# michiyasunaga/qagnn

Measured on AMD Instinct MI355X. Metric: QA-subgraphs/sec (batch x num_choice) fwd+bwd, higher is better.
Workload: dtype f32; 1 GPU; configs[1]: CSQA-shaped batch 64 questions x 5 choices = 320 subgraphs per GPU, n=200 node slots, 400..2000 edges/subgraph, 38 relations (run_qagnn__csqa.sh), 5-layer GAT d=200 H=4, QAGNN decoder fwd+bwd (LM encoder excluded: random sent_vecs), dropout 0.2, train-mode BN; subgraphs_per_gpu=320, nodes=64000, edges=396800, edges_with_self_loops=460800, graph_input=load-time int32 blobs (qagnn_graph_from_blobs), 13.3 B/edge on the wire, parallelism=single

## Files before the change

### include/qagnn_hip_tn.h

```cpp
#ifndef QAGNN_HIP_TN_H
#define QAGNN_HIP_TN_H

#include "qagnn_hip.h"

#ifdef __cplusplus
extern "C" {
#endif

int qagnn_gemm_tn_graph_f32(const float* A1, int32_t lda1, int32_t Ka1, const float* A2, int32_t lda2, int32_t Ka2, const float* B, int32_t ldb,
                            float* C, int32_t ldc, int32_t R, int32_t No, const uint32_t* amax_a1, const uint32_t* amax_a2,
                            const uint32_t* amax_b, int32_t pieces, const qagnn_graph* g, float* workspace, qagnn_stream_t stream);
int qagnn_gemm_tn_route_query(int32_t R, int32_t Ka1, int32_t Ka2, int32_t No, int32_t* h_out );
int qagnn_tn_work_table(const qagnn_graph* g, int32_t S, int32_t chunk_tiles, int32_t* out, qagnn_stream_t stream);
int qagnn_tn_live_tiles(int32_t on);

#ifdef __cplusplus
}
#endif
#endif
```

### qagnn_amd/_lib.py

```python
import ctypes as C
import functools
import os

import torch

_HERE = os.path.dirname(os.path.abspath(__file__))
LIB_PATH = os.environ.get('QAGNN_LIB') or os.path.join(_HERE, 'libqagnn_hip.so')

EXPORTS = ['qagnn_last_error', 'qagnn_abi_version', 'qagnn_graph_storage_elems', 'qagnn_graph_prep', 'qagnn_graph_prep_blocked',
           'qagnn_graph_from_blobs', 'qagnn_radam_step_f32', 'qagnn_node_prep_f32', 'qagnn_seed_epoch_advance', 'qagnn_seed_epoch_set',
           'qagnn_gemm_nn_f32', 'qagnn_gemm_nn_split_f32', 'qagnn_gemm_nn_pack_bytes', 'qagnn_gemm_nn_ws_bytes', 'qagnn_gemm_nn_split_ws_f32', 'qagnn_gemm_nn_prepack_bytes', 'qagnn_gemm_nn_prepack_f32',
           'qagnn_gemm_nn_prepack_clear', 'qagnn_gemm_tn_workspace_elems', 'qagnn_gemm_tn_f32', 'qagnn_gemm_tn2_f32', 'qagnn_gemm_tn_colsum_f32',
           'qagnn_colreduce_workspace_elems', 'qagnn_colreduce_f32', 'qagnn_bn_finalize_f32', 'qagnn_bn_stats_finalize_f32', 'qagnn_bn_relu_bwd_f32',
           'qagnn_gelu_dropout_fwd_f32', 'qagnn_gelu_dropout_bwd_f32', 'qagnn_sin_basis_f32',
           'qagnn_bn_relu_bwd_colsum_f32',
           'qagnn_pool_attn_fwd_f32', 'qagnn_pool_attn_bwd_f32', 'qagnn_head_post_fwd_f32', 'qagnn_head_post_bwd_f32', 'qagnn_add_row0_f32', 'qagnn_gather_multi_f32', 'qagnn_gather_multi_sum_f32',
           'qagnn_edge_attn_fwd_f32', 'qagnn_edge_attn_bwd_f32',
           'qagnn_hop_fwd_workspace_elems', 'qagnn_hop_bwd_workspace_elems', 'qagnn_hop_fwd_f32', 'qagnn_hop_bwd_f32',
           'qagnn_stack_fwd_f32', 'qagnn_stack_bwd_f32', 'qagnn_absmax_f32', 'qagnn_zero_words', 'qagnn_gemm_tn_h2_f32', 'qagnn_gelu_dropout_fwd_amax_f32', 'qagnn_gelu_dropout_amax_scratch_elems',
           'qagnn_timing_enable', 'qagnn_timing_read', 'qagnn_gemm_tn_h1_f32', 'qagnn_gelu_dropout_bwd_amax_f32', 'qagnn_packed_min_rows',
           'qagnn_radam_step_scaled_f32', 'qagnn_grad_norm_workspace_elems', 'qagnn_grad_norm_f32', 'qagnn_scale_multi_f32', 'qagnn_graph_prep_cap',
           'qagnn_store_gather', 'qagnn_graph_from_store']
EXPORTS_TN = ['qagnn_gemm_tn_graph_f32', 'qagnn_gemm_tn_route_query', 'qagnn_tn_work_table', 'qagnn_tn_live_tiles']
EXPORTS_INFER = ['qagnn_infer_version', 'qagnn_bn_relu_absmax_scratch_elems', 'qagnn_bn_relu_absmax_f32', 'qagnn_stack_infer_f32',
                 'qagnn_choice_eval_f32']
EXPORTS_LOSS = ['qagnn_loss_version', 'qagnn_choice_loss_f32', 'qagnn_choice_loss_bwd_f32']
LOSS_KINDS = {'cross_entropy': 0, 'margin_rank': 1}
LOSS_THREADS = 256

CLS_SLICES = 4
ABI_VERSION = 25

_i32, _i64, _f32, _u64, _vp = C.c_int32, C.c_int64, C.c_float, C.c_uint64, C.c_void_p


class qagnn_graph(C.Structure):
    _fields_ = ([(n, _i32) for n in ('N', 'E', 'Ep', 'R', 'T', 'C')] +
                [(n, _vp) for n in ('rowptr_s', 'tgt_s', 'src_s', 'cls_s', 'eid_s', 'rowptr_t', 'src_t', 'tgt_t', 'cls_t', 'pos_t',
                                    'cls_count', 'src_c', 'tgt_c', 'pos_c', 'chunk_cls', 'chunk_beg',
                                    'chunk_len', 'n_chunks', 'chunkptr')] +
                [('max_chunks', _i32), ('err', _vp), ('block_n', _i32), ('n_groups', _i32)])


class qagnn_store(C.Structure):
    _fields_ = ([(n, _vp) for n in ('blobs', 'blob_off', 'concept_ids', 'node_type', 'node_scores', 'adj_len')] +
                [('S', _i32), ('n', _i32), ('W', _i64)])


GATHER_MAX = 160


class qagnn_gather_tabs(C.Structure):
    _fields_ = [('p', _vp * GATHER_MAX), ('n', _i32)]


class qagnn_pack_desc(C.Structure):
    _fields_ = [('B1n', _vp), ('ldn1', _i32), ('K1', _i32), ('B2n', _vp), ('ldn2', _i32), ('K2', _i32), ('No', _i32), ('pieces', _i32)]


class qagnn_gemm_nn_args(C.Structure):
    _fields_ = [('A1', _vp), ('lda1', _i32), ('K1', _i32), ('B1', _vp), ('ldb1', _i32),
                ('A2', _vp), ('lda2', _i32), ('K2', _i32), ('B2', _vp), ('ldb2', _i32),
                ('C', _vp), ('ldc', _i32), ('M', _i32), ('No', _i32),
                ('bias', _vp), ('rowtab', _vp), ('ldt', _i32), ('rowidx', _vp),
                ('a_scale', _vp), ('a_shift', _vp), ('accumulate', _i32), ('a_rowidx', _vp), ('xcd_remap', _i32), ('colstat_part', _vp),
                ('a_amax1', _vp), ('a_amax2', _vp), ('a_rows', _i64), ('pieces', _i32)]


class qagnn_hop_args(C.Structure):
    _fields_ = ([('g', C.POINTER(qagnn_graph))] + [(n, _i32) for n in ('N', 'DP', 'SP', 'HP', 'T')] + [('qscale', _f32)] +
                [(n, _vp) for n in ('X', 'S', 'ntype', 'Wx_t', 'Wx', 'Ws_t', 'Ws', 'TT', 'EkEm', 'W1t', 'W1', 'b1', 'gamma', 'beta',
                                    'W2t', 'W2', 'b2')] +
                [('batch_stats', _i32), ('eps', _f32), ('run_mean_p', _vp), ('run_var_p', _vp), ('run_mean', _vp), ('run_var', _vp),
                 ('num_batches_tracked', _vp), ('dense_pos', _vp), ('d', _i32), ('momentum', _f32),
                 ('apply_act', _i32), ('p_drop', _f32), ('seed', _u64)] +
                [(n, _vp) for n in ('KMQ', 'a', 'alpha', 'aggr', 'h1', 'out', 'y', 'stats', 'dy', 'dX', 'dS')] +
                [('accumulate_dS', _i32), ('accumulate_dX', _i32)] +
                [(n, _vp) for n in ('dWx_t', 'dWs_t', 'dTT', 'dEkEm', 'dW1t', 'db1', 'dbn', 'dW2t', 'db2', 'ws')] +
                [('ws_elems', _i64), ('gemm_split', _i32), ('ones_col', _i32), ('tab_col', _i32), ('side_stream', _vp), ('amax', _vp), ('x_amax', _vp), ('s_amax', _vp)])


HOP_AMAX_WORDS = 16


def load_library(path=LIB_PATH):
    if not os.path.exists(path):
        raise OSError(f'{path} not found: build it with `python -m qagnn_amd.build` (hipcc, gfx950)')
    lib = C.CDLL(path)
    lib.qagnn_last_error.restype = C.c_char_p
    lib.qagnn_abi_version.restype = _i32
    lib.qagnn_graph_storage_elems.restype = _i64
    lib.qagnn_graph_storage_elems.argtypes = [_i32, _i32, _i32, _i32]
    lib.qagnn_graph_prep.argtypes = [C.POINTER(qagnn_graph), _vp, _vp, _vp, _vp, _i32, _i32, _i32, _i32, _vp]
    lib.qagnn_graph_prep_blocked.argtypes = [C.POINTER(qagnn_graph), _vp, _vp, _vp, _vp, _i32, _i32, _i32, _i32, _i32, _vp]
    lib.qagnn_graph_prep_cap.argtypes = [C.POINTER(qagnn_graph), _vp, _vp, _i64, _vp, _vp, _i32, _i32, _vp, _i32, _i32, _i32, _vp]
    lib.qagnn_graph_from_blobs.argtypes = [C.POINTER(qagnn_graph), _vp, _vp, _vp, _vp, _vp, _i32, _i32, _i32, _i32, _i32, _vp]
    lib.qagnn_store_gather.argtypes = [C.POINTER(qagnn_store), _vp, _i32, _vp, _vp, _vp, _vp, _vp, _vp, _vp]
    lib.qagnn_graph_from_store.argtypes = [C.POINTER(qagnn_graph), _vp, C.POINTER(qagnn_store), _vp, _vp, _vp, _i32, _i32, _i32, _i32, _vp]
    lib.qagnn_node_prep_f32.argtypes = [_vp, _vp, _vp, _vp, _i32, _i32, _vp, _vp, _vp, _i64, _vp, _vp]
    lib.qagnn_seed_epoch_advance.argtypes = [_u64, _vp]
    lib.qagnn_seed_epoch_set.argtypes = [_u64, _vp]
    lib.qagnn_radam_step_f32.argtypes = [_i32, _vp, _vp, _vp, _vp, _vp] + [C.c_double] * 6 + [_i32, _vp]
    lib.qagnn_radam_step_scaled_f32.argtypes = [_i32, _vp, _vp, _vp, _vp, _vp] + [C.c_double] * 6 + [_i32, _vp, _vp]
    lib.qagnn_grad_norm_workspace_elems.restype = _i64
    lib.qagnn_grad_norm_workspace_elems.argtypes = [_i32, _vp]
    lib.qagnn_grad_norm_f32.argtypes = [_i32, _vp, _vp, C.c_double, _vp, _vp, _vp]
    lib.qagnn_scale_multi_f32.argtypes = [_i32, _vp, _vp, _vp, _vp]
    lib.qagnn_gemm_nn_f32.argtypes = [C.POINTER(qagnn_gemm_nn_args), _vp]
    lib.qagnn_gemm_nn_split_f32.argtypes = [C.POINTER(qagnn_gemm_nn_args), _vp, _i32, _vp, _i32, _vp]
    lib.qagnn_gemm_nn_pack_bytes.restype = _i64
    lib.qagnn_gemm_nn_pack_bytes.argtypes = [_i32, _i32, _i32]
    lib.qagnn_gemm_nn_split_ws_f32.argtypes = [C.POINTER(qagnn_gemm_nn_args), _vp, _i32, _vp, _i32, _vp, _i64, _vp]
    lib.qagnn_gemm_nn_ws_bytes.restype = _i64
    lib.qagnn_gemm_nn_ws_bytes.argtypes = [C.POINTER(qagnn_gemm_nn_args), _vp, _i32, _vp, _i32]
    lib.qagnn_gemm_nn_prepack_bytes.restype = _i64
    lib.qagnn_gemm_nn_prepack_bytes.argtypes = [C.POINTER(qagnn_pack_desc), _i32]
    lib.qagnn_gemm_nn_prepack_f32.argtypes = [C.POINTER(qagnn_pack_desc), _i32, _vp, _i64, _i64, _vp]
    lib.qagnn_gemm_nn_prepack_clear.argtypes = [_i64]
    lib.qagnn_gemm_tn_workspace_elems.restype = _i64
    lib.qagnn_gemm_tn_workspace_elems.argtypes = [_i32, _i32, _i32]
    lib.qagnn_gemm_tn_f32.argtypes = [_vp, _i32, _vp, _i32, _vp, _i32, _i32, _i32, _i32, _vp, _vp, _vp, _i32, _vp, _vp]
    lib.qagnn_gemm_tn2_f32.argtypes = [_vp, _i32, _i32, _vp, _i32, _i32, _vp, _i32, _vp, _i32, _i32, _i32, _vp, _vp]
    lib.qagnn_gemm_tn_h2_f32.argtypes = [_vp, _i32, _i32, _vp, _i32, _i32, _vp, _i32, _vp, _i32, _i32, _i32, _vp, _vp, _vp, _vp, _vp, _vp, _vp]
    lib.qagnn_gemm_tn_h1_f32.argtypes = lib.qagnn_gemm_tn_h2_f32.argtypes
    lib.qagnn_gemm_tn_graph_f32.argtypes = [_vp, _i32, _i32, _vp, _i32, _i32, _vp, _i32, _vp, _i32, _i32, _i32, _vp, _vp, _vp, _i32,
                                            C.POINTER(qagnn_graph), _vp, _vp]
    lib.qagnn_gemm_tn_route_query.argtypes = [_i32, _i32, _i32, _i32, _vp]
    lib.qagnn_tn_work_table.argtypes = [C.POINTER(qagnn_graph), _i32, _i32, _vp, _vp]
    lib.qagnn_tn_live_tiles.argtypes = [_i32]
    lib.qagnn_absmax_f32.argtypes = [_vp, _i64, _vp, _vp]
    lib.qagnn_zero_words.argtypes = [_vp, _i64, _vp]
    lib.qagnn_timing_enable.argtypes = [_i32]
    lib.qagnn_timing_read.argtypes = [_vp, _vp]
    lib.qagnn_packed_min_rows.restype = _i64
    lib.qagnn_packed_min_rows.argtypes = [_i64]
    lib.qagnn_gemm_tn_colsum_f32.argtypes = [_vp, _i32, _vp, _i32, _vp, _i32, _i32, _i32, _i32, _vp, _vp, _vp, _i32, _vp, _vp, _i32,
                                             _vp, _vp]
    lib.qagnn_colreduce_workspace_elems.restype = _i64
    lib.qagnn_colreduce_workspace_elems.argtypes = [_i32, _i32, _i32]
    lib.qagnn_colreduce_f32.argtypes = [_i32, _vp, _i32, _vp, _i32, _i32, _i32, _vp, _i32, _vp, _vp, _vp, _vp, _vp, _f32, _vp, _vp, _vp]
    lib.qagnn_bn_finalize_f32.argtypes = [_vp, _vp, _vp, _vp, _f32, _vp, _vp, _vp, _i32, _vp, _vp, _vp, _vp, _i32, _f32, _f32, _i32, _vp]
    lib.qagnn_bn_stats_finalize_f32.argtypes = [_vp, _i32, _i32, _i32, _vp, _vp, _f32, _vp, _vp, _vp, _vp, _vp, _i32, _f32, _f32, _i32, _vp]
    lib.qagnn_bn_relu_bwd_f32.argtypes = [_vp, _vp, _vp, _i32, _i32, _i32, _vp, _vp, _vp, _vp, _vp, _vp, _vp, _f32, _vp, _vp]
    lib.qagnn_gelu_dropout_fwd_f32.argtypes = [_vp, _vp, _i64, _f32, _u64, _vp]
    lib.qagnn_gelu_dropout_bwd_f32.argtypes = [_vp, _vp, _vp, _i64, _f32, _u64, _vp]
    lib.qagnn_gelu_dropout_fwd_amax_f32.argtypes = [_vp, _vp, _i64, _f32, _u64, _vp, _vp, _vp]
    lib.qagnn_gelu_dropout_bwd_amax_f32.argtypes = [_vp, _vp, _vp, _i64, _f32, _u64, _vp, _vp, _vp]
    lib.qagnn_gelu_dropout_amax_scratch_elems.restype = _i64
    lib.qagnn_gelu_dropout_amax_scratch_elems.argtypes = [_i64]
    lib.qagnn_sin_basis_f32.argtypes = [_vp, _vp, _vp, _i32, _i32, _i32, _vp]
    lib.qagnn_bn_relu_bwd_colsum_f32.argtypes = [_vp, _vp, _vp, _i32, _i32, _i32, _vp, _vp, _vp, _vp, _vp, _vp, _vp, _f32, _vp, _vp, _vp, _vp]
    lib.qagnn_pool_attn_fwd_f32.argtypes = [_vp, _vp, _vp, _i32, _vp, _i32, _i32, _i32, _i32, _f32, _f32, _u64, _vp, _vp, _vp, _vp]
    lib.qagnn_pool_attn_bwd_f32.argtypes = [_vp, _vp, _i32, _i32, _i32, _i32, _i32, _f32, _f32, _u64, _vp, _vp, _vp, _vp, _vp, _i32, _vp, _vp, _vp]
    lib.qagnn_head_post_fwd_f32.argtypes = [_vp, _vp, _vp, _vp, _vp, _vp, _i64, _vp, _vp, _i32, _i32, _i32, _i32, _i32, _i32, _i32, _f32, _f32, _u64, _u64,
                                            _vp, _vp, _vp, _vp]
    lib.qagnn_head_post_bwd_f32.argtypes = [_vp, _vp, _vp, _vp, _vp, _vp, _vp, _i64, _vp, _i32, _i32, _i32, _i32, _i32, _i32, _i32, _f32, _f32, _u64, _u64,
                                            _vp, _vp, _vp, _vp, _vp, _vp, _i32, _vp]
    lib.qagnn_add_row0_f32.argtypes = [_vp, _i64, _vp, _i32, _i32, _vp]
    lib.qagnn_gather_multi_f32.argtypes = [C.POINTER(qagnn_gather_tabs), _vp, _vp, _vp, _i32, _vp]
    lib.qagnn_gather_multi_sum_f32.argtypes = [C.POINTER(qagnn_gather_tabs), _vp, _vp, _i32, _i32, _vp, _vp]
    lib.qagnn_edge_attn_fwd_f32.argtypes = [C.POINTER(qagnn_graph), _vp, _i32, _vp, _i32, _i32, _f32, _vp, _vp, _vp, _vp, _i32, _vp]
    lib.qagnn_edge_attn_bwd_f32.argtypes = [C.POINTER(qagnn_graph), _vp, _i32, _vp, _i32, _i32, _f32, _vp, _vp, _vp, _i32,
                                            _vp, _vp, _vp, _vp, _vp, _vp]
    lib.qagnn_hop_fwd_workspace_elems.restype = _i64
    lib.qagnn_hop_fwd_workspace_elems.argtypes = [_i32, _i32, _i32]
    lib.qagnn_hop_bwd_workspace_elems.restype = _i64
    lib.qagnn_hop_bwd_workspace_elems.argtypes = [_i32, _i32, _i32, _i32, _i32]
    lib.qagnn_hop_fwd_f32.argtypes = [C.POINTER(qagnn_hop_args), _vp]
    lib.qagnn_hop_bwd_f32.argtypes = [C.POINTER(qagnn_hop_args), _vp]
    lib.qagnn_stack_fwd_f32.argtypes = [C.POINTER(qagnn_hop_args), _i32, _vp]
    lib.qagnn_stack_bwd_f32.argtypes = [C.POINTER(qagnn_hop_args), _i32, _vp]
    lib.qagnn_infer_version.argtypes = []
    lib.qagnn_bn_relu_absmax_scratch_elems.restype = _i64
    lib.qagnn_bn_relu_absmax_scratch_elems.argtypes = [_i32, _i32]
    lib.qagnn_bn_relu_absmax_f32.argtypes = [_vp, _i32, _i32, _i32, _vp, _vp, _vp, _vp, _vp]
    lib.qagnn_stack_infer_f32.argtypes = [C.POINTER(qagnn_hop_args), _i32, _vp]
    lib.qagnn_choice_eval_f32.argtypes = [_vp, _i64, _vp, _i32, _i32, _vp, _vp, _vp]
    lib.qagnn_loss_version.argtypes = []
    lib.qagnn_choice_loss_f32.argtypes = [_vp, _i64, _vp, _i32, _i32, _i32, _f32, _vp, _vp, _vp, _i64, _vp, _vp, _vp]
    lib.qagnn_choice_loss_bwd_f32.argtypes = [_vp, _i64, _vp, _vp, _i64, _i32, _i32, _vp]
    for name in EXPORTS + EXPORTS_TN + EXPORTS_INFER + EXPORTS_LOSS:
        fn = getattr(lib, name)
        if fn.restype is C.c_int and name not in ('qagnn_abi_version',):
            fn.restype = _i32
    return lib


def _ptr(t):
    return None if t is None else t.data_ptr()


def choice_loss_bound(kind, nc, Q, max_abs=1.0, margin=0.0, weight=1.0, threads=LOSS_THREADS):
    import math
    u, v = 2.0 ** -24, 2.0 ** -53
    M, L, w = max(1.0, float(max_abs)), math.log(nc), abs(float(weight))
    S = -(-Q // threads) + math.log2(threads) + nc
    if LOSS_KINDS[kind] == 0:
        return w * M * (u * (nc + 8 + 5 * L) + v * S * (2 + L)), w / Q * u * (nc + 8 + L)
    return w * M * (3 * u + v * S) * (2 + abs(float(margin)) / M), w / Q * 2 * u


def _running_fields(running):
    if running is None:
        return None, None, None, None, 0, 0.0, 1.0
    rm, rv, nbt, pos, mom, unb = running
    assert rm.is_contiguous() and rv.is_contiguous() and pos.dtype == torch.long and (nbt is None or nbt.dtype == torch.long)
    return rm.data_ptr(), rv.data_ptr(), _ptr(nbt), pos.data_ptr(), rm.numel(), float(mom), float(unb)


def _chk2d(t, name, dtype=torch.float32):
    assert t.is_cuda and t.dtype == dtype and t.dim() == 2 and t.is_contiguous(), \
        f'{name}: need a contiguous 2-D {dtype} device tensor, got {tuple(t.shape)} {t.dtype} {t.device}'
# ... 426 lines not shown
                n2, ld2 = B2n.data_ptr(), _ld(B2n)
            ws_bytes = self.lib.qagnn_gemm_nn_ws_bytes(C.byref(a), B1n.data_ptr(), ld1, n2, ld2) if M >= self.PACK_MIN_M else 0
            if ws_bytes > 0:
                ws = torch.empty(ws_bytes, dtype=torch.uint8, device=A1.device)
                self._check(self.lib.qagnn_gemm_nn_split_ws_f32(C.byref(a), B1n.data_ptr(), ld1, n2, ld2, ws.data_ptr(), ws_bytes, self._stream()),
                            'qagnn_gemm_nn_split_ws_f32')
            else:
                self._check(self.lib.qagnn_gemm_nn_split_f32(C.byref(a), B1n.data_ptr(), ld1, n2, ld2, self._stream()), 'qagnn_gemm_nn_split_f32')
            return (out, part) if colstats else out
        assert K1 % 16 == 0 and (A2 is None or A2.size(1) % 16 == 0), 'the fp32-MFMA kernel needs K to be a multiple of 16'
        self._check(self.lib.qagnn_gemm_nn_f32(C.byref(a), self._stream()), 'qagnn_gemm_nn_f32')
        return out

    def _tn_out_ws(self, R, Ka, No, out, dev):
        if out is None:
            out = torch.empty((Ka, No), dtype=torch.float32, device=dev)
        else:
            _chkp(out, 'out')
            assert out.shape == (Ka, No)
        return out, torch.empty(self.lib.qagnn_gemm_tn_workspace_elems(R, Ka, No), dtype=torch.float32, device=dev)

    def gemm_tn(self, A, B, a_scale=None, a_shift=None, out=None, accumulate=False, a_rowidx=None, colsum_groups=0,
                b_rowidx=None):
        _chkp(A, 'A'), _chkp(B, 'B')
        Ka = A.size(1)
        R, No = B.shape
        assert (A.size(0) == R) if a_rowidx is None else (a_rowidx.numel() == R and a_rowidx.dtype == torch.long)
        assert out is not None or not accumulate
        out, ws = self._tn_out_ws(R, Ka, No, out, A.device)
        bsum = None
        if colsum_groups:
            assert b_rowidx is None or (b_rowidx.dtype == torch.long and b_rowidx.numel() == R and b_rowidx.is_contiguous())
            bsum = torch.empty((colsum_groups, No), dtype=torch.float32, device=A.device)
        rc = self.lib.qagnn_gemm_tn_colsum_f32(A.data_ptr(), _ld(A), B.data_ptr(), _ld(B), out.data_ptr(), _ld(out), R, Ka, No, _ptr(a_scale),
                                               _ptr(a_shift), _ptr(a_rowidx), 1 if accumulate else 0, _ptr(bsum), _ptr(b_rowidx),
                                               colsum_groups, ws.data_ptr(), self._stream())
        self._check(rc, 'qagnn_gemm_tn_colsum_f32')
        return (out, bsum) if colsum_groups else out

    def absmax(self, x, out=None):
        assert x.is_contiguous() and x.dtype == torch.float32 and x.numel() % 4 == 0
        if out is None:
            out = torch.empty(4, dtype=torch.int32, device=x.device)
            self._check(self.lib.qagnn_zero_words(out.data_ptr(), 4, self._stream()), 'qagnn_zero_words')
        self._check(self.lib.qagnn_absmax_f32(x.data_ptr(), x.numel(), out.data_ptr(), self._stream()), 'qagnn_absmax_f32')
        return out

    def gemm_tn_h2(self, A1, B, amax_a1, amax_b, A2=None, amax_a2=None, a_scale=None, a_shift=None, out=None):
        _chkp(A1, 'A1'), _chkp(B, 'B')
        if A2 is not None:
            _chkp(A2, 'A2')
        Ka1, Ka2 = A1.size(1), (A2.size(1) if A2 is not None else 0)
        R, No = B.shape
        out, ws = self._tn_out_ws(R, Ka1 + Ka2, No, out, B.device)
        fn = self.lib.qagnn_gemm_tn_h1_f32 if self.gemm_split == 3 else self.lib.qagnn_gemm_tn_h2_f32
        rc = fn(A1.data_ptr(), _ld(A1), Ka1, _ptr(A2), _ld(A2) if A2 is not None else 0, Ka2, B.data_ptr(), _ld(B), out.data_ptr(), _ld(out), R, No, _ptr(a_scale),
                                           _ptr(a_shift), amax_a1.data_ptr(), _ptr(amax_a2), amax_b.data_ptr(), ws.data_ptr(), self._stream())
        self._check(rc, 'qagnn_gemm_tn_h2_f32')
        return out

    def gemm_tn_graph(self, A1, A2, B, graph=None, pieces=3, amax=None, out=None):
        _chkp(A1, 'A1'), _chkp(A2, 'A2'), _chkp(B, 'B')
        Ka1, Ka2 = A1.size(1), A2.size(1)
        R, No = B.shape
        assert A1.size(0) == R and A2.size(0) == R and (pieces == 3 or amax is not None)
        out, ws = self._tn_out_ws(R, Ka1 + Ka2, No, out, B.device)
        am = [None, None, None] if amax is None else [t.data_ptr() for t in amax]
        rc = self.lib.qagnn_gemm_tn_graph_f32(A1.data_ptr(), _ld(A1), Ka1, A2.data_ptr(), _ld(A2), Ka2, B.data_ptr(), _ld(B), out.data_ptr(), _ld(out),
                                              R, No, am[0], am[1], am[2], pieces, C.byref(graph.c) if graph is not None else None, ws.data_ptr(),
                                              self._stream())
        self._check(rc, 'qagnn_gemm_tn_graph_f32')
        return out

    def tn_route_query(self, R, Ka1, Ka2, No):
        out = (_i32 * 4)()
        self._check(self.lib.qagnn_gemm_tn_route_query(R, Ka1, Ka2, No, C.cast(out, _vp)), 'qagnn_gemm_tn_route_query')
        return tuple(out)

    def tn_work_table(self, graph, S, chunk_tiles):
        out = torch.empty(4 + 5 * S, dtype=torch.int32, device=graph.storage.device)
        self._check(self.lib.qagnn_tn_work_table(C.byref(graph.c), S, chunk_tiles, out.data_ptr(), self._stream()), 'qagnn_tn_work_table')
        return out

    def tn_live_tiles(self, on):
        return int(self.lib.qagnn_tn_live_tiles(int(on)))

    def gemm_tn2(self, A1, A2, B, out=None):
        _chkp(A1, 'A1'), _chkp(A2, 'A2'), _chkp(B, 'B')
        Ka1, Ka2 = A1.size(1), A2.size(1)
        R, No = B.shape
        assert A1.size(0) == R and A2.size(0) == R
        out, ws = self._tn_out_ws(R, Ka1 + Ka2, No, out, B.device)
        rc = self.lib.qagnn_gemm_tn2_f32(A1.data_ptr(), _ld(A1), Ka1, A2.data_ptr(), _ld(A2), Ka2, B.data_ptr(), _ld(B), out.data_ptr(), _ld(out), R, No,
                                         ws.data_ptr(), self._stream())
        self._check(rc, 'qagnn_gemm_tn2_f32')
        return out

    def _colreduce(self, mode, X, X2, rowidx, groups, mean, invstd, scale, shift, nout, out_scale=1.0, roww=None, out=None):
        _chkp(X, 'X')
        R, Cc = X.shape
        if out is None:
            out = torch.empty((nout, Cc), dtype=torch.float32, device=X.device)
        else:
            assert out.shape == (nout, Cc) and out.is_contiguous() and out.dtype == torch.float32
        ws = torch.empty(self.lib.qagnn_colreduce_workspace_elems(R, Cc, groups), dtype=torch.float32, device=X.device)
        rc = self.lib.qagnn_colreduce_f32(mode, X.data_ptr(), _ld(X), _ptr(X2), _ld(X2) if X2 is not None else Cc, R, Cc, _ptr(rowidx), groups, _ptr(mean),
                                          _ptr(invstd), _ptr(scale), _ptr(shift), _ptr(roww), float(out_scale), out.data_ptr(), ws.data_ptr(), self._stream())
        self._check(rc, 'qagnn_colreduce_f32')
        return out

    def colsum(self, X, rowidx=None, groups=1, scale=1.0, roww=None, out=None):
        return self._colreduce(0, X, None, rowidx, groups, None, None, None, None, groups, scale, roww, out=out)

    def colvar_sum(self, X, mean, scale=1.0, roww=None):
        return self._colreduce(1, X, None, None, 1, mean, None, None, None, 1, scale, roww)[0]

    def bn_finalize(self, mean, var, gamma, beta, eps, running=None, ones_col=-1):
        Cc = mean.numel()
        out = torch.empty((3, Cc), dtype=torch.float32, device=mean.device)
        rc = self.lib.qagnn_bn_finalize_f32(mean.data_ptr(), var.data_ptr(), gamma.data_ptr(), beta.data_ptr(), float(eps),
                                            out[0].data_ptr(), out[1].data_ptr(), out[2].data_ptr(), Cc, *_running_fields(running),
                                            int(ones_col), self._stream())
        self._check(rc, 'qagnn_bn_finalize_f32')
        return out[0], out[1], out[2]

    def bn_stats_finalize(self, part, rows, gamma, beta, eps, running=None, ones_col=-1):
        nt, _, Cc = part.shape
        assert part.is_contiguous() and nt == -(-rows // self.STAT_TILE)
        stats = torch.empty((5, Cc), dtype=torch.float32, device=part.device)
        rc = self.lib.qagnn_bn_stats_finalize_f32(part.data_ptr(), nt, int(rows), Cc, gamma.data_ptr(), beta.data_ptr(), float(eps), stats.data_ptr(),
                                                  *_running_fields(running), int(ones_col), self._stream())
        self._check(rc, 'qagnn_bn_stats_finalize_f32')
        return stats

    def bn_bwd_reduce(self, dR, H, mean, invstd, scale, shift):
        _chkp(H, 'H')
        assert H.shape == dR.shape
        return self._colreduce(2, dR, H, None, 1, mean, invstd, scale, shift, 2)

    @staticmethod
    def _bn_bwd_operands(dR, H, dH):
        _chkp(dR, 'dR'), _chkp(H, 'H')
        if dH is None:
            dH = torch.empty(H.shape, dtype=torch.float32, device=H.device)
        _chkp(dH, 'dH')
        assert dR.shape == H.shape == dH.shape and _ld(dR) == _ld(H) == _ld(dH), \
            f'bn_relu_bwd: dR, H and dH share one row pitch, got {_ld(dR)}, {_ld(H)}, {_ld(dH)}'
        return dH, _ld(H)

    def bn_relu_bwd(self, dR, H, mean, invstd, scale, shift, gamma, red, inv_rows, roww=None, dH=None):
        assert red.is_contiguous() and red.shape == (2, H.size(1))
        dH, ld = self._bn_bwd_operands(dR, H, dH)
        R, Cc = H.shape
        rc = self.lib.qagnn_bn_relu_bwd_f32(dR.data_ptr(), H.data_ptr(), dH.data_ptr(), ld, R, Cc, mean.data_ptr(),
                                            invstd.data_ptr(), scale.data_ptr(), shift.data_ptr(), gamma.data_ptr(),
                                            red[0].data_ptr(), red[1].data_ptr(), float(inv_rows), _ptr(roww), self._stream())
        self._check(rc, 'qagnn_bn_relu_bwd_f32')
        return dH

    POOL_LIMITS = (4, 256, 1024)

    def pool_attn_fwd(self, u, cvec, K, mask, inv_temp, p, seed):
        B, NH, Cc = u.shape
        n = K.size(1)
        assert u.is_contiguous() and cvec.is_contiguous() and mask.is_contiguous() and mask.dtype == torch.bool
        _chkp3(K, 'K')
# ... 473 lines not shown
```

### qagnn_amd/csrc/common.h

```cpp
#pragma once
#include <hip/hip_runtime.h>
#include <stdint.h>
#include <stdio.h>

#include <type_traits>

#include "../../include/qagnn_hip.h"
#include "../../include/qagnn_hip_tn.h"
#include "../../include/qagnn_hip_infer.h"

namespace qagnn {

void set_error(const char* fmt, ...);

struct NnProduct {
  const qagnn_gemm_nn_args* a;
  bool split;
  const float* B1n; int ldn1; const float* B2n; int ldn2;
  void* ws; int64_t ws_bytes;
};
enum class NnFamily { FP32, SPLIT, NN2 };
enum class NnB { IN_KERNEL, PACK, IMAGE };
struct NnRoute {
  NnFamily family;
  int nt, np, wv;
  bool affine, flat, stats;
  NnB b; const void* image;
  int64_t ws_bytes;
  int ntiles, grid;
};
inline int num_cus() {
  static int n = [] {
    int dev = 0, v = 0;
    if (hipGetDevice(&dev) != hipSuccess || hipDeviceGetAttribute(&v, hipDeviceAttributeMultiprocessorCount, dev) != hipSuccess || v <= 0) v = 256;
    return v;
  }();
  return n;
}
static inline int cdiv(int64_t a, int64_t b) { return (int)((a + b - 1) / b); }
inline void nn_grid(NnRoute& r, int M, int No, int rows_per_tile, int per_cu) {
  r.ntiles = cdiv(No, r.nt * 16) * cdiv(M, rows_per_tile);
  const int cap = (num_cus() * per_cu) & ~7;
  r.grid = r.ntiles < cap ? r.ntiles : cap;
}
NnRoute nn_route(const NnProduct& p);
bool nn_rows_packed(int64_t M);
int gemm_nn(const NnProduct& p, hipStream_t stream);
int launch_nn(const NnRoute& r, const qagnn_gemm_nn_args& a, hipStream_t stream);
int launch_nn_split(const NnRoute& r, const qagnn_gemm_nn_args& a, const float* B1n, int ldn1, const float* B2n, int ldn2, hipStream_t stream);
int launch_nn2(const NnRoute& r, const qagnn_gemm_nn_args& a, const float* B1n, int ldn1, const float* B2n, int ldn2, hipStream_t stream);
int launch_pack_b(int np, const qagnn_gemm_nn_args& a, const float* B1n, int ldn1, const float* B2n, int ldn2, void* ws, hipStream_t stream);
namespace nn2 { int walk_tiles(int K1, int K2); }
int64_t nn2_pack_bytes(int No, int K1, int K2, int np);
const void* nn2_prepack_lookup(const float* B1n, int ldn1, int K1, const float* B2n, int ldn2, int K2, int No, int np);

struct TnProduct {
  const float* A1; int lda1, Ka1;
  const float* A2; int lda2, Ka2; bool two;
  const float* B; int ldb;
  float* C; int ldc, R, No;
  const float* a_scale; const float* a_shift; const int64_t* a_rowidx; int accumulate;
  float* bsum; const int64_t* b_rowidx; int groups;
  const uint32_t* amax[3]; int np;
  float* ws;
  const qagnn_graph* g;
};
inline TnProduct tn_product(const float* A1, int lda1, int Ka1, const float* A2, int lda2, int Ka2, const float* B, int ldb, float* C, int ldc, int R,
                            int No, const float* a_scale, const float* a_shift, float* ws, const uint32_t* amax_a1 = nullptr,
                            const uint32_t* amax_a2 = nullptr, const uint32_t* amax_b = nullptr, int np = 3) {
  TnProduct p = {};
  p.A1 = A1; p.lda1 = lda1; p.Ka1 = Ka1;
  if (A2 && Ka2 > 0) { p.A2 = A2; p.lda2 = lda2; p.Ka2 = Ka2; p.two = true; }
  p.B = B; p.ldb = ldb; p.C = C; p.ldc = ldc; p.R = R; p.No = No; p.a_scale = a_scale; p.a_shift = a_shift; p.ws = ws;
  p.amax[0] = amax_a1; p.amax[1] = amax_a2; p.amax[2] = amax_b; p.np = np;
  return p;
}
enum class TnFamily { RUNTIME, STRIP, SPLIT, WS, PAIR };
struct TnRoute {
  TnFamily family;
  int kt, nt, waves, np;
  bool affine, gather, colsum;
  int chunk_rows, nchunks;
  bool sum_by4;
  bool live;
  dim3 grid;
  int64_t ws_elems;
};
TnRoute tn_route(const TnProduct& p);
int gemm_tn(const TnProduct& p, hipStream_t stream);
int launch_tn(const TnRoute& r, const TnProduct& p, float* Pcs, hipStream_t stream);
int launch_tn_strip(const TnRoute& r, const TnProduct& p, float* Pcs, hipStream_t stream);
int launch_tn_split(const TnRoute& r, const TnProduct& p, hipStream_t stream);
int launch_tn_ws(const TnRoute& r, const TnProduct& p, hipStream_t stream);
int launch_sum_chunks(const float* P, float* C, int ldc, int rows, int No, int nchunks, int accumulate, bool by4, hipStream_t stream);

constexpr int TN_LIST_CAP = 1024;
constexpr int TN_LIVE_BC = 208;
struct TnLive { const int* list; const int* n_live; int T, S, chunk_tiles; };
struct TnWork { int cK, cM, lenM, qK, rK; };
struct TnSlot { int cb, list, beg, cnt, pslot; };
__host__ __device__ inline TnWork tn_work(int S, int T, int L, int chunk_tiles) {
  TnWork w;
  L = L < 0 ? 0 : (L > T ? T : L);
  if (L >= T) {
    w.cK = S / 3; w.cM = S - 2 * w.cK; w.lenM = chunk_tiles; w.qK = -1; w.rK = 0;
    return w;
  }
  const long long den = (long long)T + 2ll * L;
  int c = (int)((2ll * S * L + den) / (2 * den));
  const int hi = (S - 1) / 2;
  c = c < 1 ? 1 : (c > hi ? hi : c);
  w.cK = c; w.cM = S - 2 * c; w.lenM = (T + w.cM - 1) / w.cM; w.qK = L / c; w.rK = L % c;
  return w;
}
__host__ __device__ inline TnSlot tn_slot(const TnWork& w, int S, int T, int u) {
  auto start = [&](int j) { return 2 * j + (int)((long long)j * w.cM / w.cK); };
  int j = (int)((long long)u * w.cK / S);
  while (j > 0 && start(j) > u) --j;
  while (j + 1 < w.cK && start(j + 1) <= u) ++j;
  const int off = u - start(j);
  TnSlot s;
  auto range = [&](int i) { s.list = 0; s.beg = i * w.lenM < T ? i * w.lenM : T; s.cnt = T - s.beg < w.lenM ? T - s.beg : w.lenM; };
  if (off < 2) {
    s.cb = off == 0 ? 0 : 2;
    s.pslot = off == 0 ? j : w.cK + j;
    if (w.qK < 0) range(j);
    else { s.list = 1; s.beg = j * w.qK + (j < w.rK ? j : w.rK); s.cnt = w.qK + (j < w.rK ? 1 : 0); }
  } else {
    const int m = (int)((long long)j * w.cM / w.cK) + off - 2;
    s.cb = 1;
    s.pslot = 2 * w.cK + m;
    range(m);
  }
  return s;
}
int launch_sum_chunks_live(const float* P, float* C, int ldc, int rows, const TnLive& lv, int accumulate, hipStream_t stream);
bool tn_live_enabled();
struct LiveTiles { int n_tiles; int32_t *n_live, *live, *list; };
inline LiveTiles live_tiles_of(const qagnn_graph* g) {
  const int T = (int)(((int64_t)g->N + 31) / 32), T4 = (T + 3) & ~3;
  int32_t* const p = g->err + 16;
  return LiveTiles{T, p, p + 4, p + 4 + T4};
}

int launch_gelu_dropout(const float* X, const float* dY, float* out, int64_t n, float p, uint64_t seed, uint32_t* amax, float* amax_part,
                        hipStream_t stream);
int64_t gelu_amax_scratch_elems(int64_t n);
int launch_bn_relu_bwd_colsum(const float* dR, const float* Hh, float* dH, int ld, int R, int Cc, const float* mean, const float* invstd,
                              const float* scale, const float* shift, const float* gamma, const float* sum_dy, const float* sum_dy_hhat,
                              float inv_rows, const float* roww, float* colsum, float* workspace, uint32_t* amax, hipStream_t stream);
int launch_bn_stats_finalize(const float* part, int n_tiles, int R, int Cc, const float* gamma, const float* beta, float eps, float* stats,
                             float* run_mean, float* run_var, int64_t* nbt, int d, float momentum, float unbias, int ones_col, uint32_t* amax_bound,
                             hipStream_t stream);

int launch_edge_attn_fwd(const qagnn_graph* g, const float* KMQ, int32_t ldk, const float* EkEm, int32_t lde, int32_t HP, float qscale,
                         float* score, float* a, float* alpha, float* aggr, int32_t lda, float* amax_part , hipStream_t stream);
int launch_edge_attn_bwd(const qagnn_graph* g, const float* KMQ, int32_t ldk, const float* EkEm, int32_t lde, int32_t HP, float qscale,
                         const float* a, const float* alpha, const float* G, int32_t ldg, float* dKMQ, float* dEkEm, float* ga, float* rs,
                         float* cls_part, float* amax_part , uint32_t* amax_slot, hipStream_t stream);
int launch_amax_reduce(const float* part, int64_t n, uint32_t* slot, hipStream_t stream);
int launch_bn_relu_absmax(const float* H, int ldh, int R, int Cc, const float* scale, const float* shift, uint32_t* slot, float* part, hipStream_t stream);

struct TimedScope {
  int kind;
  hipStream_t s;
  hipEvent_t e0, e1;
  bool counted;
  TimedScope(int kind, hipStream_t s);
  ~TimedScope();
  TimedScope(const TimedScope&) = delete;
  TimedScope& operator=(const TimedScope&) = delete;
};

#define QAGNN_REQUIRE(cond, code, ...) \
  do {                                 \
    if (!(cond)) {                     \
      qagnn::set_error(__VA_ARGS__);   \
      return (code);                   \
    }                                  \
  } while (0)

#define QAGNN_LAUNCH_CHECK(name)                                               \
  do {                                                                         \
    hipError_t e__ = hipGetLastError();                                        \
    if (e__ != hipSuccess) {                                                   \
      qagnn::set_error("%s launch failed: %s", name, hipGetErrorString(e__));  \
      return QAGNN_EHIP;                                                       \
    }                                                                          \
  } while (0)

#ifndef QAGNN_NN_OCC
#define QAGNN_NN_OCC 2
#endif

template <int V0, int... Vs, class F>
inline int dispatch_int(int v, F&& f) {
  if constexpr (sizeof...(Vs) == 0) return f(std::integral_constant<int, V0>{});
  else return v == V0 ? f(std::integral_constant<int, V0>{}) : dispatch_int<Vs...>(v, f);
}
template <class F>
inline int dispatch_bool(bool v, F&& f) { return v ? f(std::true_type{}) : f(std::false_type{}); }

template <auto KERNEL>
inline int raise_lds_limit(int bytes, const char* name) {
  static bool raised[64] = {};
  int dev = 0;
  if (hipGetDevice(&dev) != hipSuccess) dev = 0;
  if (bytes <= 64 * 1024 || raised[dev & 63]) return QAGNN_OK;
  hipError_t e = hipFuncSetAttribute((const void*)KERNEL, hipFuncAttributeMaxDynamicSharedMemorySize, bytes);
  if (e != hipSuccess) { set_error("%s: cannot raise the dynamic LDS limit: %s", name, hipGetErrorString(e)); return QAGNN_EHIP; }
  raised[dev & 63] = true;
  return QAGNN_OK;
}

static inline bool aligned16(const void* p) { return (reinterpret_cast<uintptr_t>(p) & 15u) == 0; }

__device__ __forceinline__ int xcd_remap(int b, int nblocks) {
  const int q = nblocks >> 3, r = nblocks & 7;
  const int xcd = b & 7, slot = b >> 3;
  const int base = xcd < r ? xcd * (q + 1) : r * (q + 1) + (xcd - r) * q;
  return base + slot;
}

__host__ __device__ __forceinline__ int edge_xcd_cap(int N) {
  const int per = (((N + 3) >> 2) + 7) >> 3;
  return (per * 5 + 3) >> 2;
}
// ... 136 lines not shown
```

### qagnn_amd/csrc/elementwise.hip

```cpp
#include "common.h"

namespace qagnn {

constexpr int CR_WR_BIG = 32, CR_WR_SMALL = 8;
static inline int cr_wr(int R) { return R < 32768 ? CR_WR_SMALL : CR_WR_BIG; }

template <int MODE, int CR_WR>
__global__ __launch_bounds__(256) void k_colreduce(const float* __restrict__ X, int ldx, const float* __restrict__ X2, int ldx2,
                                                   int R, int Cc, const int64_t* __restrict__ rowidx, int groups,
                                                   const float* __restrict__ mean, const float* __restrict__ invstd,
                                                   const float* __restrict__ scale, const float* __restrict__ shift,
                                                   const float* __restrict__ roww, float* __restrict__ part) {
  constexpr int NOUT = MODE == 0 ? 4 : (MODE == 2 ? 2 : 1);
  __shared__ __attribute__((aligned(16))) float red[4][NOUT][256];
  const int lane = threadIdx.x & 63, w = threadIdx.x >> 6;
  const int col = blockIdx.x * 256 + lane * 4;
  const bool act = col < Cc;
  constexpr int CR_ROWS = 4 * CR_WR;
  const int r0 = blockIdx.y * CR_ROWS + w * CR_WR;
  float4 acc[NOUT];
#pragma unroll
  for (int o = 0; o < NOUT; ++o) acc[o] = make_float4(0.f, 0.f, 0.f, 0.f);
  float4 mu = make_float4(0.f, 0.f, 0.f, 0.f), is = mu, sc = mu, sh = mu;
  if (act && MODE >= 1) mu = ld4(mean + col);
  if (act && MODE == 2) { is = ld4(invstd + col); sc = ld4(scale + col); sh = ld4(shift + col); }
  if (act) {
    const int rend = min(R, r0 + CR_WR);
    for (int rb = r0; rb < rend; rb += 8) {
      float4 xs[8], hs[8];
#pragma unroll
      for (int u = 0; u < 8; ++u) {
        const int r = min(rb + u, rend - 1);
        xs[u] = ld4(X + (int64_t)r * ldx + col);
        if (MODE == 2) hs[u] = ld4(X2 + (int64_t)r * ldx2 + col);
      }
#pragma unroll
      for (int u = 0; u < 8; ++u) {
        const int r = rb + u;
        if (r >= rend) break;
        float4 x = xs[u];
        const float wr = (MODE != 2 && roww) ? roww[r] : 1.f;
        if (MODE == 0) {
          x = make_float4(x.x * wr, x.y * wr, x.z * wr, x.w * wr);
          const int g = rowidx ? (int)rowidx[r] : 0;
          if (g == 0) acc[0] = add4(acc[0], x);
          else if (g == 1) acc[1] = add4(acc[1], x);
          else if (g == 2) acc[2] = add4(acc[2], x);
          else acc[3] = add4(acc[3], x);
        } else if (MODE == 1) {
          const float4 d = make_float4(x.x - mu.x, x.y - mu.y, x.z - mu.z, x.w - mu.w);
          acc[0] = make_float4(fmaf(d.x * wr, d.x, acc[0].x), fmaf(d.y * wr, d.y, acc[0].y), fmaf(d.z * wr, d.z, acc[0].z),
                               fmaf(d.w * wr, d.w, acc[0].w));
        } else {
          const float4 h = hs[u];
          float4 dy;
          dy.x = fmaf(h.x, sc.x, sh.x) <= 0.f ? 0.f : x.x;
          dy.y = fmaf(h.y, sc.y, sh.y) <= 0.f ? 0.f : x.y;
          dy.z = fmaf(h.z, sc.z, sh.z) <= 0.f ? 0.f : x.z;
          dy.w = fmaf(h.w, sc.w, sh.w) <= 0.f ? 0.f : x.w;
          acc[0] = add4(acc[0], dy);
          acc[1].x = fmaf(dy.x, (h.x - mu.x) * is.x, acc[1].x);
          acc[1].y = fmaf(dy.y, (h.y - mu.y) * is.y, acc[1].y);
          acc[1].z = fmaf(dy.z, (h.z - mu.z) * is.z, acc[1].z);
          acc[1].w = fmaf(dy.w, (h.w - mu.w) * is.w, acc[1].w);
        }
      }
    }
  }
#pragma unroll
  for (int o = 0; o < NOUT; ++o) st4(&red[w][o][lane * 4], acc[o]);
  __syncthreads();
  const int nout = MODE == 0 ? groups : NOUT;
  for (int i = threadIdx.x; i < nout * 256; i += 256) {
    const int o = i >> 8, c = i & 255;
    if (blockIdx.x * 256 + c < Cc) {
      const float s = (red[0][o][c] + red[1][o][c]) + (red[2][o][c] + red[3][o][c]);
      part[((int64_t)blockIdx.y * nout + o) * Cc + blockIdx.x * 256 + c] = s;
    }
  }
}

constexpr int CF_Q = 16;
__global__ __launch_bounds__(64 * CF_Q) void k_colreduce_final(const float* __restrict__ part, float* __restrict__ out, int nchunks,
                                                               int tot, float out_scale) {
  __shared__ float red[CF_Q][64];
  const int lane = threadIdx.x & 63, q = threadIdx.x >> 6;
  const int o = blockIdx.x * 64 + lane;
  float s0 = 0.f, s1 = 0.f;
  if (o < tot) {
    int c = q;
#pragma unroll 4
    for (; c + CF_Q < nchunks; c += 2 * CF_Q) {
      s0 += part[(int64_t)c * tot + o];
      s1 += part[(int64_t)(c + CF_Q) * tot + o];
    }
    if (c < nchunks) s0 += part[(int64_t)c * tot + o];
  }
  red[q][lane] = s0 + s1;
  __syncthreads();
  if (q == 0 && o < tot) {
    float s = red[0][lane];
#pragma unroll
    for (int k = 1; k < CF_Q; ++k) s += red[k][lane];
    out[o] = s * out_scale;
  }
}


__global__ void k_bn_relu_bwd(const float* __restrict__ dR, const float* __restrict__ Hh, float* __restrict__ dH, int ld, int R,
                              int Cc, const float* __restrict__ mean, const float* __restrict__ invstd,
                              const float* __restrict__ scale, const float* __restrict__ shift, const float* __restrict__ gamma,
                              const float* __restrict__ sum_dy, const float* __restrict__ sum_dy_hhat, float inv_rows,
                              const float* __restrict__ roww) {
  const int c4n = Cc >> 2;
  const int64_t i = (int64_t)blockIdx.x * blockDim.x + threadIdx.x;
  if (i >= (int64_t)R * c4n) return;
  const int r = (int)(i / c4n), col = (int)(i % c4n) * 4;
  if (roww) inv_rows = roww[r];
  const int64_t off = (int64_t)r * ld + col;
  const float4 g = ld4(dR + off), h = ld4(Hh + off);
  const float4 mu = ld4(mean + col), is = ld4(invstd + col), sc = ld4(scale + col), sh = ld4(shift + col);
  const float4 ga = ld4(gamma + col), k1 = ld4(sum_dy + col), k2 = ld4(sum_dy_hhat + col);
  float4 o;
#define ONE(f)                                              \
  {                                                         \
// ... 207 lines not shown
        acc = add4(acc, o);
        am = fmaxf(am, absmax4(o));
      }
    }
  }
  st4(&red[w][lane * 4], acc);
  __syncthreads();
  const int c = threadIdx.x;
  if (blockIdx.x * 256 + c < Cc)
    part[(int64_t)blockIdx.y * Cc + blockIdx.x * 256 + c] = (red[0][c] + red[1][c]) + (red[2][c] + red[3][c]);
  if (amax) {
    __shared__ float ared[16];
    block_amax_merge(am, amax, ared);
  }
}

__device__ unsigned long long g_seed_epoch = 0;
__global__ void k_seed_epoch(unsigned long long* w, unsigned long long v, int add) { *w = add ? *w + v : v; }

const unsigned long long* seed_epoch_ptr() {
  static const unsigned long long* cache[64] = {};
  int dev = 0;
  if (hipGetDevice(&dev) != hipSuccess) dev = 0;
  const unsigned long long*& p = cache[dev & 63];
  if (!p) {
    void* a = nullptr;
    if (hipGetSymbolAddress(&a, HIP_SYMBOL(g_seed_epoch)) != hipSuccess) return nullptr;
    p = static_cast<const unsigned long long*>(a);
  }
  return p;
}

__global__ void k_sin_basis(const float* __restrict__ score, const float* __restrict__ js, float* __restrict__ out, int ldo, int R,
                            int J) {
  const int64_t i = (int64_t)blockIdx.x * blockDim.x + threadIdx.x;
  if (i >= (int64_t)R * ldo) return;
  const int r = (int)(i / ldo), j = (int)(i % ldo);
  out[i] = j < J ? sinf(js[j] * score[r]) : 0.f;
}

}

using namespace qagnn;

extern "C" int64_t qagnn_colreduce_workspace_elems(int32_t R, int32_t Cc, int32_t groups) {
  return (int64_t)cdiv(R, 4 * cr_wr(R)) * (groups < 2 ? 2 : groups) * Cc;
}

extern "C" int qagnn_colreduce_f32(int32_t mode, const float* X, int32_t ldx, const float* X2, int32_t ldx2, int32_t R, int32_t Cc,
                                   const int64_t* rowidx, int32_t groups, const float* mean, const float* invstd,
                                   const float* scale, const float* shift, const float* roww, float out_scale, float* out, float* workspace, qagnn_stream_t stream_) {
  hipStream_t stream = (hipStream_t)stream_;
  QAGNN_REQUIRE(X && out && workspace, QAGNN_EINVAL, "colreduce: null pointer");
  QAGNN_REQUIRE(R > 0 && Cc > 0 && Cc % 4 == 0 && ldx % 4 == 0 && aligned16(X), QAGNN_EINVAL, "colreduce: bad sizes/alignment");
  QAGNN_REQUIRE(mode >= 0 && mode <= 2, QAGNN_EINVAL, "colreduce: bad mode %d", mode);
  QAGNN_REQUIRE(ldx >= Cc && (mode != 2 || ldx2 >= Cc), QAGNN_EINVAL, "colreduce: ldx=%d / ldx2=%d below Cc=%d", ldx, ldx2, Cc);
  const bool small = cr_wr(R) == CR_WR_SMALL;
  dim3 grid(cdiv(Cc, 256), cdiv(R, 4 * cr_wr(R)));
  int nout;
  if (mode == 0) {
    QAGNN_REQUIRE(groups >= 1 && groups <= 4 && (groups == 1 || rowidx), QAGNN_EINVAL, "colreduce: groups=%d (1..4)", groups);
    nout = groups;
    if (small) k_colreduce<0, CR_WR_SMALL><<<grid, 256, 0, stream>>>(X, ldx, X2, ldx2, R, Cc, rowidx, groups, mean, invstd, scale, shift, roww, workspace);
    else k_colreduce<0, CR_WR_BIG><<<grid, 256, 0, stream>>>(X, ldx, X2, ldx2, R, Cc, rowidx, groups, mean, invstd, scale, shift, roww, workspace);
  } else if (mode == 1) {
    QAGNN_REQUIRE(mean && aligned16(mean), QAGNN_EINVAL, "colreduce: mode 1 needs mean");
    nout = 1;
    if (small) k_colreduce<1, CR_WR_SMALL><<<grid, 256, 0, stream>>>(X, ldx, X2, ldx2, R, Cc, rowidx, groups, mean, invstd, scale, shift, roww, workspace);
    else k_colreduce<1, CR_WR_BIG><<<grid, 256, 0, stream>>>(X, ldx, X2, ldx2, R, Cc, rowidx, groups, mean, invstd, scale, shift, roww, workspace);
  } else {
    QAGNN_REQUIRE(X2 && mean && invstd && scale && shift && ldx2 % 4 == 0 && aligned16(X2), QAGNN_EINVAL,
                  "colreduce: mode 2 needs X2, mean, invstd, scale, shift");
    nout = 2;
    if (small) k_colreduce<2, CR_WR_SMALL><<<grid, 256, 0, stream>>>(X, ldx, X2, ldx2, R, Cc, rowidx, groups, mean, invstd, scale, shift, roww, workspace);
    else k_colreduce<2, CR_WR_BIG><<<grid, 256, 0, stream>>>(X, ldx, X2, ldx2, R, Cc, rowidx, groups, mean, invstd, scale, shift, roww, workspace);
  }
  QAGNN_LAUNCH_CHECK("k_colreduce");
  const int tot = nout * Cc;
  k_colreduce_final<<<cdiv(tot, 64), 64 * CF_Q, 0, stream>>>(workspace, out, grid.y, tot, out_scale);
  QAGNN_LAUNCH_CHECK("k_colreduce_final");
  return QAGNN_OK;
}

extern "C" int qagnn_bn_relu_bwd_f32(const float* dR, const float* Hh, float* dH, int32_t ld, int32_t R, int32_t Cc,
                                     const float* mean, const float* invstd, const float* scale, const float* shift,
                                     const float* gamma, const float* sum_dy, const float* sum_dy_hhat, float inv_rows,
                                     const float* roww, qagnn_stream_t stream_) {
  hipStream_t stream = (hipStream_t)stream_;
  QAGNN_REQUIRE(dR && Hh && dH && mean && invstd && scale && shift && gamma && sum_dy && sum_dy_hhat, QAGNN_EINVAL,
                "bn_relu_bwd: null pointer");
  QAGNN_REQUIRE(R > 0 && Cc > 0 && Cc % 4 == 0 && ld % 4 == 0, QAGNN_EINVAL, "bn_relu_bwd: bad sizes");
  QAGNN_REQUIRE(ld >= Cc, QAGNN_EINVAL, "bn_relu_bwd: ld=%d below Cc=%d", ld, Cc);
  const int64_t tot = (int64_t)R * (Cc / 4);
  k_bn_relu_bwd<<<cdiv(tot, 256), 256, 0, stream>>>(dR, Hh, dH, ld, R, Cc, mean, invstd, scale, shift, gamma, sum_dy, sum_dy_hhat,
                                                    inv_rows, roww);
  QAGNN_LAUNCH_CHECK("k_bn_relu_bwd");
  return QAGNN_OK;
}

extern "C" int qagnn_bn_finalize_f32(const float* mean, const float* var, const float* gamma, const float* beta, float eps, float* invstd,
                                     float* scale, float* shift, int32_t Cc, float* run_mean, float* run_var, int64_t* num_batches_tracked,
                                     const int64_t* dense_pos, int32_t d, float momentum, float unbias, int32_t ones_col,
                                     qagnn_stream_t stream_) {
  hipStream_t stream = (hipStream_t)stream_;
  QAGNN_REQUIRE(mean && var && gamma && beta && invstd && scale && shift && Cc > 0, QAGNN_EINVAL, "bn_finalize: null pointer");
  QAGNN_REQUIRE(!run_mean || (run_var && dense_pos && d > 0 && d <= Cc), QAGNN_EINVAL, "bn_finalize: running-stat arguments");
  k_bn_finalize<<<cdiv(Cc, 256), 256, 0, stream>>>(mean, var, gamma, beta, eps, invstd, scale, shift, Cc, run_mean, run_var,
                                                   num_batches_tracked, dense_pos, d, momentum, unbias, ones_col);
  QAGNN_LAUNCH_CHECK("k_bn_finalize");
  return QAGNN_OK;
}

namespace qagnn {
int launch_bn_stats_finalize(const float* part, int n_tiles, int R, int Cc, const float* gamma, const float* beta, float eps, float* stats,
                             float* run_mean, float* run_var, int64_t* nbt, int d, float momentum, float unbias, int ones_col, uint32_t* amax_bound,
                             hipStream_t stream) {
  k_bn_stats_finalize<<<cdiv(Cc, BF_COLS), BF_COLS * BF_PARTS, 0, stream>>>(part, n_tiles, R, Cc, gamma, beta, eps, stats, run_mean, run_var, nbt, d,
                                                                            momentum, unbias, ones_col, amax_bound);
  QAGNN_LAUNCH_CHECK("k_bn_stats_finalize");
  return QAGNN_OK;
}
}

extern "C" int qagnn_bn_stats_finalize_f32(const float* part, int32_t n_tiles, int32_t R, int32_t Cc, const float* gamma, const float* beta,
                                           float eps, float* stats, float* run_mean, float* run_var, int64_t* num_batches_tracked,
                                           const int64_t* dense_pos, int32_t d, float momentum, float unbias, int32_t ones_col,
                                           qagnn_stream_t stream_) {
  hipStream_t stream = (hipStream_t)stream_;
  QAGNN_REQUIRE(part && gamma && beta && stats && R > 0 && Cc > 0 && n_tiles == cdiv(R, ST_TILE), QAGNN_EINVAL,
                "bn_stats_finalize: bad arguments (R=%d needs %d tiles of %d rows, got %d)", R, cdiv(R, ST_TILE), ST_TILE, n_tiles);
  QAGNN_REQUIRE(!run_mean || (run_var && d > 0 && d % 4 == 0 && Cc % 4 == 0 && d <= Cc), QAGNN_EINVAL, "bn_stats_finalize: running-stat arguments");
  (void)dense_pos;
  return launch_bn_stats_finalize(part, n_tiles, R, Cc, gamma, beta, eps, stats, run_mean, run_var, num_batches_tracked, d, momentum, unbias, ones_col,
                                  nullptr, stream);
}

__global__ __launch_bounds__(256) void k_gather_multi(qagnn_gather_tabs t, const int* __restrict__ tid, const int* __restrict__ off,
                                                     float* __restrict__ out, int total) {
  __shared__ const float* ps[QAGNN_GATHER_MAX];
  for (int i = threadIdx.x; i < t.n; i += blockDim.x) ps[i] = t.p[i];
  __syncthreads();
  const int i = blockIdx.x * blockDim.x + threadIdx.x;
  if (i >= total) return;
  const int k = tid[i];
  out[i] = k >= 0 ? ps[k][off[i]] : 0.f;
}

__global__ __launch_bounds__(256) void k_gather_multi_sum(qagnn_gather_tabs t, const int* __restrict__ tid, const int* __restrict__ off, int K, int S,
                                                         float* __restrict__ out) {
  __shared__ const float* ps[QAGNN_GATHER_MAX];
  for (int i = threadIdx.x; i < t.n; i += blockDim.x) ps[i] = t.p[i];
  __syncthreads();
  const int s = blockIdx.x * blockDim.x + threadIdx.x;
  if (s >= S) return;
  float acc = 0.f;
  for (int k = 0; k < K; ++k) {
    const int g = tid[(int64_t)k * S + s];
    const float* p = g >= 0 ? ps[g] : nullptr;
    const float v = p != nullptr ? p[off[(int64_t)k * S + s]] : 0.f;
    acc = k == 0 ? v : acc + v;
  }
  out[s] = acc;
}

extern "C" int qagnn_gather_multi_f32(const qagnn_gather_tabs* t, const int32_t* tid, const int32_t* off, float* out, int32_t total,
                                      qagnn_stream_t stream_) {
// ... 194 lines not shown
```

### qagnn_amd/csrc/gemm.hip

```cpp
#include <stdlib.h>

#include "gemm_device.h"

namespace qagnn {

typedef float f32x4 __attribute__((ext_vector_type(4)));

constexpr int BK = 16;
constexpr int NN_BM = 128;
constexpr int PA_NN = BK + 4;

__host__ __device__ constexpr int pitch_b(int bn) { return (bn % 32 == 16) ? bn : bn + 16; }

template <int V> struct ic { static constexpr int value = V; };

template <int NM>
__device__ __forceinline__ void sched_ktile_pipeline() {
  constexpr int DS = 0x100, MFMA = 0x008, NR = (NM + 1) / 2 + 1;
#pragma unroll
  for (int r = 0; r < NR; ++r) __builtin_amdgcn_sched_group_barrier(DS, 1, 0);
#pragma unroll
  for (int kk = 0; kk < 3; ++kk) {
#pragma unroll
    for (int t = 0; t < NR; ++t) {
// ... 380 lines not shown
        const int g = groups > 1 ? grp_s[cur][kq] : 0;
        if (g == 0) cs[0] += v;
        else if (g == 1) cs[1] += v;
        else if (g == 2) cs[2] += v;
        else cs[3] += v;
      }
    }
    if (more) lstore(ic<cur ^ 1>{});
    __syncthreads();
  };

  if (nkt > 0) {
    gload(0);
    lstore(ic<0>{});
  }
  __syncthreads();
  for (int kt = 0; kt < nkt; kt += 2) {
    ktile(ic<0>{}, kt);
    if (kt + 1 < nkt) ktile(ic<1>{}, kt + 1);
  }
  if (do_cs && n0 + tid < No) {
    float* pc = Pcs + (int64_t)chunk * groups * No + n0 + tid;
    pc[0] = cs[0];
    if (groups > 1) pc[No] = cs[1];
    if (groups > 2) pc[2 * No] = cs[2];
    if (groups > 3) pc[3 * No] = cs[3];
  }
  float* Pc = P + (int64_t)chunk * Ka * No;
#pragma unroll
  for (int r = 0; r < 4; ++r) {
    const int row = m0 + w * 16 + (lane >> 4) * 4 + r;
    if (row >= Ka) continue;
#pragma unroll
    for (int j = 0; j < NT; ++j) {
      const int col = n0 + j * 16 + (lane & 15);
      if (col < No) Pc[(int64_t)row * No + col] = acc[j][r];
    }
  }
}

__global__ void k_sum_chunks(const float* __restrict__ P, float* __restrict__ C, int ldc, int Ka, int No, int nchunks,
                             int accumulate) {
  const int64_t i = (int64_t)blockIdx.x * blockDim.x + threadIdx.x;
  if (i >= (int64_t)Ka * No) return;
  const int row = (int)(i / No), col = (int)(i % No);
  float s = 0.f;
#pragma unroll 8
  for (int c = 0; c < nchunks; ++c) s += P[(int64_t)c * Ka * No + i];
  float* d = C + (int64_t)row * ldc + col;
  *d = accumulate ? *d + s : s;
}

constexpr int SC_G = 16;
__global__ __launch_bounds__(SC_G * 64) void k_sum_chunks4(const float* __restrict__ P, float* __restrict__ C, int ldc, int Ka, int No,
                                                           int nchunks, int accumulate) {
  __shared__ float4 part[SC_G][64];
  const int lane = threadIdx.x & 63, g = threadIdx.x >> 6;
  const int64_t n4 = (int64_t)Ka * No / 4, i4 = (int64_t)blockIdx.x * 64 + lane;
  float4 s = make_float4(0.f, 0.f, 0.f, 0.f);
  if (i4 < n4) {
    const float4* src = reinterpret_cast<const float4*>(P) + i4;
    for (int c0 = g; c0 < nchunks; c0 += 4 * SC_G) {
      float4 v[4];
#pragma unroll
      for (int u = 0; u < 4; ++u) v[u] = src[(int64_t)min(c0 + u * SC_G, nchunks - 1) * n4];
#pragma unroll
      for (int u = 0; u < 4; ++u)
        if (c0 + u * SC_G < nchunks) s = add4(s, v[u]);
    }
  }
  part[g][lane] = s;
  __syncthreads();
  if (g == 0 && i4 < n4) {
    float4 t = part[0][lane];
#pragma unroll
    for (int k = 1; k < SC_G; ++k) t = add4(t, part[k][lane]);
    const int64_t e = i4 * 4;
    float* d = C + (e / No) * ldc + (e % No);
    if (accumulate) t = add4(t, ld4(d));
    st4(d, t);
  }
}

__global__ __launch_bounds__(SC_G * 64) void k_sum_chunks4_live(const float* __restrict__ P, float* __restrict__ C, int ldc, int Ka, TnLive lv,
                                                                int accumulate) {
  __shared__ float4 part[SC_G][64];
  constexpr int BC = TN_LIVE_BC, No = 3 * BC;
  const int lane = threadIdx.x & 63, g = threadIdx.x >> 6;
  const int64_t n4 = (int64_t)Ka * No / 4, i4 = (int64_t)blockIdx.x * 64 + lane;
  const TnWork w = tn_work(lv.S, lv.T, lv.n_live[0], lv.chunk_tiles);
  float4 s = make_float4(0.f, 0.f, 0.f, 0.f);
  if (i4 < n4) {
    const int64_t e = i4 * 4;
    const int row = (int)(e / No), col = (int)(e % No), cb = col / BC, lc = col - cb * BC;
    const int first = cb == 0 ? 0 : cb == 2 ? w.cK : 2 * w.cK, n = cb == 1 ? w.cM : w.cK;
    const int64_t t4 = (int64_t)Ka * BC / 4;
    const float4* src = reinterpret_cast<const float4*>(P) + (int64_t)first * t4 + ((int64_t)row * BC + lc) / 4;
    for (int c0 = g; c0 < n; c0 += 4 * SC_G) {
      float4 v[4];
#pragma unroll
      for (int u = 0; u < 4; ++u) v[u] = src[(int64_t)min(c0 + u * SC_G, n - 1) * t4];
#pragma unroll
      for (int u = 0; u < 4; ++u)
        if (c0 + u * SC_G < n) s = add4(s, v[u]);
    }
  }
  part[g][lane] = s;
  __syncthreads();
  if (g == 0 && i4 < n4) {
    float4 t = part[0][lane];
#pragma unroll
    for (int k = 1; k < SC_G; ++k) t = add4(t, part[k][lane]);
    const int64_t e = i4 * 4;
    float* d = C + (e / No) * ldc + (e % No);
    if (accumulate) t = add4(t, ld4(d));
    st4(d, t);
  }
}

int launch_nn(const NnRoute& r, const qagnn_gemm_nn_args& a, hipStream_t stream) {
  qagnn_gemm_nn_args b = a;
  b.xcd_remap = 1;
  return dispatch_int<13, 8, 7, 4, 2>(r.nt, [&](auto nt) {
    return dispatch_bool(r.affine, [&](auto aff) {
      k_gemm_nn<nt.value, aff.value, 8, 1><<<r.grid, 512, 0, stream>>>(b, r.ntiles);
      QAGNN_LAUNCH_CHECK("k_gemm_nn");
      return QAGNN_OK;
    });
  });
}

#define QAGNN_TN_ARGS p.A1, p.lda1, p.B, p.ldb, p.ws, p.R, p.Ka1, p.No, p.a_scale, p.a_shift, p.a_rowidx
int launch_tn(const TnRoute& r, const TnProduct& p, float* Pcs, hipStream_t stream) {
  return dispatch_int<13, 8, 7, 4, 2>(r.nt, [&](auto nt) {
    return dispatch_bool(r.affine, [&](auto aff) {
      const size_t lds = 2 * (size_t)(BK * pitch16(r.waves * 16) + BK * pitch_b(nt.value * 16) + BK) * sizeof(float);
      k_gemm_tn<nt.value, aff.value><<<r.grid, r.waves * 64, lds, stream>>>(QAGNN_TN_ARGS, Pcs, p.b_rowidx, p.groups, r.chunk_rows);
      QAGNN_LAUNCH_CHECK("k_gemm_tn");
      return QAGNN_OK;
    });
  });
}
int launch_tn_strip(const TnRoute& r, const TnProduct& p, float* Pcs, hipStream_t stream) {
  return dispatch_int<7, 13, 16>(r.waves, [&](auto nw) {
    return dispatch_bool(r.colsum, [&](auto cs) {
      return dispatch_bool(r.affine, [&](auto aff) {
        k_gemm_tn_strip<13, nw.value, aff.value, cs.value><<<r.grid, nw.value * 64, 0, stream>>>(QAGNN_TN_ARGS, r.chunk_rows, Pcs, p.b_rowidx, p.groups);
        QAGNN_LAUNCH_CHECK("k_gemm_tn_strip");
        return QAGNN_OK;
      });
    });
  });
}
#undef QAGNN_TN_ARGS

int launch_sum_chunks_live(const float* P, float* C, int ldc, int rows, const TnLive& lv, int accumulate, hipStream_t stream) {
  const int64_t tot = (int64_t)rows * 3 * TN_LIVE_BC;
  k_sum_chunks4_live<<<cdiv(tot / 4, 64), SC_G * 64, 0, stream>>>(P, C, ldc, rows, lv, accumulate);
  QAGNN_LAUNCH_CHECK("k_sum_chunks4_live");
  return QAGNN_OK;
}

int launch_sum_chunks(const float* P, float* C, int ldc, int rows, int No, int nchunks, int accumulate, bool by4, hipStream_t stream) {
  const int64_t tot = (int64_t)rows * No;
  if (by4) k_sum_chunks4<<<cdiv(tot / 4, 64), SC_G * 64, 0, stream>>>(P, C, ldc, rows, No, nchunks, accumulate);
  else k_sum_chunks<<<cdiv(tot, 256), 256, 0, stream>>>(P, C, ldc, rows, No, nchunks, accumulate);
  QAGNN_LAUNCH_CHECK("k_sum_chunks");
  return QAGNN_OK;
}

}
```

### qagnn_amd/csrc/gemm_dispatch.hip

```cpp
#include <stdlib.h>

#include <atomic>
#include <initializer_list>

#include "common.h"

namespace qagnn {

static int pick_nt(int No) {
  const int cands[5] = {13, 7, 8, 4, 2};
  for (int c : cands)
    if (No % (c * 16) == 0) return c;
  int best = 4;
  int64_t best_cost = INT64_MAX;
  for (int c : cands) {
    const int64_t cost = (int64_t)cdiv(No, c * 16) * c * 16;
    if (cost < best_cost) { best_cost = cost; best = c; }
  }
  return best;
}

static std::atomic<int64_t> g_pack_min_m{8192};
bool nn_rows_packed(int64_t M) { return M >= g_pack_min_m.load(std::memory_order_relaxed); }

// ... 69 lines not shown
  QAGNN_REQUIRE(!a.rowtab || a.rowidx, QAGNN_EINVAL, "gemm_nn: rowtab without rowidx");
  QAGNN_REQUIRE(a.ldc % 4 == 0 && aligned16(a.C) && (!a.bias || aligned16(a.bias)) && (!a.rowtab || (aligned16(a.rowtab) && a.ldt % 4 == 0)),
                QAGNN_EINVAL, "gemm_nn: C / bias / rowtab must be 16-byte aligned with pitches multiple of 4");
  QAGNN_REQUIRE(!a.a_scale || (a.a_shift && aligned16(a.a_scale) && aligned16(a.a_shift)), QAGNN_EINVAL,
                "gemm_nn: a_scale/a_shift must both be given and 16-byte aligned");
  QAGNN_REQUIRE(a.lda1 >= a.K1 && (a.K2 == 0 || a.lda2 >= a.K2), QAGNN_EINVAL, "gemm_nn: lda1=%d / lda2=%d below K1=%d / K2=%d", a.lda1, a.lda2,
                a.K1, a.K2);
  QAGNN_REQUIRE(p.split || (ldb1 >= a.No && (a.K2 == 0 || ldb2 >= a.No)), QAGNN_EINVAL, "gemm_nn: ldb1=%d / ldb2=%d below No=%d", ldb1, ldb2, a.No);
  QAGNN_REQUIRE(a.ldc >= a.No && (!a.rowtab || a.ldt >= a.No), QAGNN_EINVAL, "gemm_nn: ldc=%d / ldt=%d below No=%d", a.ldc, a.ldt, a.No);
  if (p.split && a.colstat_part) {
    const int64_t lim = (int64_t)0x7FFFFFFF;
    QAGNN_REQUIRE(cdiv(a.No, 16) == 13 && !a.a_scale && !a.a_rowidx && !a.rowtab && !a.accumulate && a.K2 == 0, QAGNN_EUNSUPPORTED,
                  "gemm_nn: column statistics need 193..208 output columns and a bias-only epilogue (No=%d)", a.No);
    QAGNN_REQUIRE((int64_t)a.M * a.lda1 * 4 < lim && (int64_t)a.No * ldb1 * 4 < lim, QAGNN_EUNSUPPORTED,
                  "gemm_nn: column statistics with operands of 2 GB and more");
  }
  return QAGNN_OK;
}

int gemm_nn(const NnProduct& p, hipStream_t stream) {
  TimedScope timed(0, stream);
  if (int rc = nn_validate(p)) return rc;
  const qagnn_gemm_nn_args& a = *p.a;
  const NnRoute r = nn_route(p);
  if (r.family == NnFamily::FP32) return launch_nn(r, a, stream);
  if (r.family == NnFamily::SPLIT) return launch_nn_split(r, a, p.B1n, p.ldn1, p.B2n, p.ldn2, stream);
  if (r.b == NnB::IN_KERNEL) return launch_nn2(r, a, p.B1n, p.ldn1, p.B2n, p.ldn2, stream);
  if (r.b == NnB::PACK) {
    QAGNN_REQUIRE(aligned16(p.ws), QAGNN_EINVAL, "gemm_nn: the pack workspace must be 16-byte aligned");
    if (int rc = launch_pack_b(r.np, a, p.B1n, p.ldn1, p.B2n, p.ldn2, p.ws, stream)) return rc;
  }
  return launch_nn2(r, a, static_cast<const float*>(r.b == NnB::PACK ? p.ws : r.image), cdiv(a.No, 16), nullptr, 0, stream);
}

static int tn_chunk_rows(int R, int blocks_per_chunk, int per_cu, int ktile, int lo) {
  const int target = num_cus() * per_cu / blocks_per_chunk;
  const int rows = cdiv(cdiv(R, target > 0 ? target : 1), ktile) * ktile, lo_k = cdiv(lo, ktile) * ktile;
  return rows > lo_k ? rows : lo_k;
}
static int tn_min_chunk(int R, bool split) { return R > 4096 ? 256 : split ? 32 : 64; }
static int64_t tn_ws_bound(int R, int Ka, int No) { return (int64_t)cdiv(R, tn_min_chunk(R, true)) * ((int64_t)Ka * No + 4 * (int64_t)No); }
constexpr int TN_WS_MIN_TILES = 28;

static int pick_tn_waves(int Ka) {
  int best = 4, best_waste = INT32_MAX;
  for (int nw = 16; nw >= 4; --nw) {
    const int bm = nw * 16, waste = cdiv(Ka, bm) * bm - Ka;
    if (waste < best_waste) { best_waste = waste; best = nw; }
  }
  return best;
}
static bool tn_split_ok(const TnProduct& p, int Ka, int lda) {
  static const int mode = getenv("QAGNN_GEMM_SPLIT") ? atoi(getenv("QAGNN_GEMM_SPLIT")) : 1;
  const bool gather = p.a_rowidx != nullptr;
  const int64_t big = (int64_t)p.R * ((lda > p.ldb && !gather) ? lda : p.ldb) * 4;
  if (gather && (Ka <= 112 || p.a_scale)) return false;
  return mode != 0 && Ka >= 64 && p.No >= 104 && p.R >= 1024 && big < (int64_t)0x7FFFFFFF;
}

static std::atomic<int> g_tn_live{1};
bool tn_live_enabled() { return g_tn_live.load(std::memory_order_relaxed) != 0; }
static bool tn_live_ok(const TnProduct& p) {
  return p.g && tn_live_enabled() && p.two && p.No == 3 * TN_LIVE_BC && p.g->N == p.R && p.g->err && !p.a_scale;
}

TnRoute tn_route(const TnProduct& p) {
  TnRoute r = {};
  r.np = 3;
  r.affine = p.a_scale != nullptr;
  r.gather = p.a_rowidx != nullptr;
  r.colsum = p.bsum != nullptr;
  r.sum_by4 = p.ldc % 4 == 0 && aligned16(p.C);
  const bool split = !r.colsum && tn_split_ok(p, p.Ka1, p.lda1) && (!p.two || (r.sum_by4 && tn_split_ok(p, p.Ka2, p.lda2)));
  const int lo = tn_min_chunk(p.R, split);
  int row_blocks;
  if (split) {
    if (r.sum_by4 && !r.gather && p.amax[0] && p.amax[2] && (!p.two || p.amax[1])) r.np = p.np;
    r.kt = (p.two || p.Ka1 <= 112) ? 7 : 13;
    r.nt = 20 - r.kt;
    row_blocks = cdiv(p.Ka1, r.kt * 16) + (p.two ? cdiv(p.Ka2, r.kt * 16) : 0);
    const int bpc = cdiv(p.No, r.nt * 16) * row_blocks;
    r.chunk_rows = tn_chunk_rows(p.R, bpc, 2, 32, lo);
    r.family = TnFamily::SPLIT;
    if (p.two) {
      const int rows1 = tn_chunk_rows(p.R, bpc, 1, 32, lo);
      if (rows1 >= 2 * TN_WS_MIN_TILES * 32) r.chunk_rows = rows1;
      if (r.chunk_rows >= TN_WS_MIN_TILES * 32) r.family = TnFamily::WS;
      if (r.family == TnFamily::WS && tn_live_ok(p)) {
        const int T = cdiv(p.R, 32), nch = cdiv(p.R, r.chunk_rows);
        r.live = nch >= 3 && 5 * (T / (3 * nch) + 1) <= TN_LIST_CAP && cdiv(T, nch - 2) <= TN_LIST_CAP;
      }
    }
  } else if (p.two) {
    r.family = TnFamily::PAIR;
    return r;
  } else {
    r.nt = pick_nt(p.No);
    r.waves = pick_tn_waves(p.Ka1);
    r.family = r.nt == 13 && (r.waves == 7 || r.waves == 13 || r.waves == 16) ? TnFamily::STRIP : TnFamily::RUNTIME;
    row_blocks = cdiv(p.Ka1, r.waves * 16);
    r.chunk_rows = tn_chunk_rows(p.R, cdiv(p.No, r.nt * 16) * row_blocks, r.waves <= 8 ? 2 : 1, 16, lo);
  }
  r.nchunks = cdiv(p.R, r.chunk_rows);
  r.grid = dim3(cdiv(p.No, r.nt * 16), row_blocks, r.nchunks);
  r.ws_elems = (int64_t)r.nchunks * ((int64_t)(p.Ka1 + p.Ka2) * p.No + (r.colsum ? (int64_t)p.groups * p.No : 0));
  return r;
}

static int tn_validate(const TnProduct& p) {
  QAGNN_REQUIRE(p.A1 && p.B && p.C && p.ws && (!p.two || p.A2), QAGNN_EINVAL, "gemm_tn: null pointer");
  QAGNN_REQUIRE(p.R > 0 && p.Ka1 > 0 && p.No > 0 && p.Ka1 % 4 == 0 && p.No % 4 == 0 && (!p.two || (p.Ka2 > 0 && p.Ka2 % 4 == 0)), QAGNN_EINVAL,
                "gemm_tn: bad sizes R=%d Ka1=%d Ka2=%d No=%d (Ka, No multiples of 4)", p.R, p.Ka1, p.Ka2, p.No);
  QAGNN_REQUIRE(p.lda1 % 4 == 0 && p.ldb % 4 == 0 && aligned16(p.A1) && aligned16(p.B) && (!p.two || (p.lda2 % 4 == 0 && aligned16(p.A2))),
                QAGNN_EINVAL, "gemm_tn: operands must be 16-byte aligned with pitches multiple of 4");
  QAGNN_REQUIRE(!p.a_scale || (!p.two && p.a_shift && aligned16(p.a_scale) && aligned16(p.a_shift)), QAGNN_EINVAL,
                "gemm_tn: a_scale/a_shift must both be given and 16-byte aligned (one-operand products only)");
  QAGNN_REQUIRE(p.lda1 >= p.Ka1 && (!p.two || p.lda2 >= p.Ka2) && p.ldb >= p.No && p.ldc >= p.No, QAGNN_EINVAL,
                "gemm_tn: a pitch below its width (lda1=%d Ka1=%d lda2=%d Ka2=%d ldb=%d ldc=%d No=%d)", p.lda1, p.Ka1, p.lda2, p.Ka2, p.ldb, p.ldc,
                p.No);
  QAGNN_REQUIRE(!p.bsum || (p.groups >= 1 && p.groups <= 4 && (p.groups == 1 || p.b_rowidx)), QAGNN_EINVAL, "gemm_tn: colsum groups=%d (1..4)",
                p.groups);
  return QAGNN_OK;
}

static int tn_run(const TnProduct& p, hipStream_t stream) {
  if (int rc = tn_validate(p)) return rc;
  const TnRoute r = tn_route(p);
  if (r.family == TnFamily::PAIR) {
    TnProduct q = p;
    q.two = false; q.A2 = nullptr; q.lda2 = q.Ka2 = 0;
    q.amax[0] = q.amax[1] = q.amax[2] = nullptr;
    if (int rc = tn_run(q, stream)) return rc;
    q.A1 = p.A2; q.lda1 = p.lda2; q.Ka1 = p.Ka2; q.C = p.C + (int64_t)p.Ka1 * p.ldc;
    return tn_run(q, stream);
  }
  const int Ka = p.Ka1 + p.Ka2;
  QAGNN_REQUIRE(r.ws_elems <= tn_ws_bound(p.R, Ka, p.No), QAGNN_EINVAL, "gemm_tn: the route outgrows qagnn_gemm_tn_workspace_elems()");
  float* Pcs = r.colsum ? p.ws + (int64_t)r.nchunks * Ka * p.No : nullptr;
  const int rc = r.family == TnFamily::WS      ? launch_tn_ws(r, p, stream)
                 : r.family == TnFamily::SPLIT ? launch_tn_split(r, p, stream)
                 : r.family == TnFamily::STRIP ? launch_tn_strip(r, p, Pcs, stream)
                                               : launch_tn(r, p, Pcs, stream);
  if (rc != QAGNN_OK) return rc;
  if (r.live) {
    const LiveTiles lt = live_tiles_of(p.g);
    return launch_sum_chunks_live(p.ws, p.C, p.ldc, Ka, TnLive{lt.list, lt.n_live, lt.n_tiles, 3 * r.nchunks, r.chunk_rows / 32}, p.accumulate, stream);
  }
  if (int rc2 = launch_sum_chunks(p.ws, p.C, p.ldc, Ka, p.No, r.nchunks, p.accumulate, r.sum_by4, stream)) return rc2;
  return r.colsum ? launch_sum_chunks(Pcs, p.bsum, p.No, p.groups, p.No, r.nchunks, 0, false, stream) : QAGNN_OK;
}

int gemm_tn(const TnProduct& p, hipStream_t stream) {
  TimedScope timed(1, stream);
  return tn_run(p, stream);
}

}

using namespace qagnn;

extern "C" int64_t qagnn_packed_min_rows(int64_t rows) { return rows < 0 ? g_pack_min_m.load() : g_pack_min_m.exchange(rows > 1 ? rows : 1); }

extern "C" int64_t qagnn_gemm_nn_pack_bytes(int32_t No, int32_t K1, int32_t K2) { return nn2_pack_bytes(No, K1, K2, 3) + 256; }

extern "C" int64_t qagnn_gemm_nn_ws_bytes(const qagnn_gemm_nn_args* a, const float* B1n, int32_t ldn1, const float* B2n, int32_t ldn2) {
  alignas(16) static char any_ws;
  return a && B1n ? nn_route(NnProduct{a, true, B1n, ldn1, B2n, ldn2, &any_ws, INT64_MAX}).ws_bytes : 0;
}

extern "C" int qagnn_gemm_nn_f32(const qagnn_gemm_nn_args* a, qagnn_stream_t stream) {
  return gemm_nn(NnProduct{a, false, nullptr, 0, nullptr, 0, nullptr, 0}, (hipStream_t)stream);
}

extern "C" int qagnn_gemm_nn_split_f32(const qagnn_gemm_nn_args* a, const float* B1n, int32_t ldn1, const float* B2n, int32_t ldn2,
                                       qagnn_stream_t stream) {
  return gemm_nn(NnProduct{a, true, B1n, ldn1, B2n, ldn2, nullptr, 0}, (hipStream_t)stream);
}

extern "C" int qagnn_gemm_nn_split_ws_f32(const qagnn_gemm_nn_args* a, const float* B1n, int32_t ldn1, const float* B2n, int32_t ldn2,
                                          void* ws, int64_t ws_bytes, qagnn_stream_t stream) {
  return gemm_nn(NnProduct{a, true, B1n, ldn1, B2n, ldn2, ws, ws_bytes}, (hipStream_t)stream);
}

extern "C" int64_t qagnn_gemm_tn_workspace_elems(int32_t R, int32_t Ka, int32_t No) { return tn_ws_bound(R, Ka, No); }

extern "C" int qagnn_gemm_tn_colsum_f32(const float* A, int32_t lda, const float* B, int32_t ldb, float* C, int32_t ldc, int32_t R,
                                        int32_t Ka, int32_t No, const float* a_scale, const float* a_shift, const int64_t* a_rowidx,
                                        int32_t accumulate, float* bsum, const int64_t* b_rowidx, int32_t groups, float* workspace,
                                        qagnn_stream_t stream) {
  TnProduct p = tn_product(A, lda, Ka, nullptr, 0, 0, B, ldb, C, ldc, R, No, a_scale, a_shift, workspace);
  p.a_rowidx = a_rowidx; p.accumulate = accumulate; p.bsum = bsum; p.b_rowidx = b_rowidx; p.groups = groups;
  return gemm_tn(p, (hipStream_t)stream);
}

extern "C" int qagnn_gemm_tn_f32(const float* A, int32_t lda, const float* B, int32_t ldb, float* C, int32_t ldc, int32_t R,
                                 int32_t Ka, int32_t No, const float* a_scale, const float* a_shift, const int64_t* a_rowidx,
                                 int32_t accumulate, float* workspace, qagnn_stream_t stream) {
  TnProduct p = tn_product(A, lda, Ka, nullptr, 0, 0, B, ldb, C, ldc, R, No, a_scale, a_shift, workspace);
  p.a_rowidx = a_rowidx; p.accumulate = accumulate;
  return gemm_tn(p, (hipStream_t)stream);
}

extern "C" int qagnn_gemm_tn2_f32(const float* A1, int32_t lda1, int32_t Ka1, const float* A2, int32_t lda2, int32_t Ka2, const float* B,
                                  int32_t ldb, float* C, int32_t ldc, int32_t R, int32_t No, float* workspace, qagnn_stream_t stream) {
  TnProduct p = tn_product(A1, lda1, Ka1, A2, lda2, Ka2, B, ldb, C, ldc, R, No, nullptr, nullptr, workspace);
  p.two = true;
  return gemm_tn(p, (hipStream_t)stream);
}

extern "C" int qagnn_gemm_tn_h2_f32(const float* A1, int32_t lda1, int32_t Ka1, const float* A2, int32_t lda2, int32_t Ka2, const float* B,
                                    int32_t ldb, float* C, int32_t ldc, int32_t R, int32_t No, const float* a_scale, const float* a_shift,
                                    const uint32_t* amax_a1, const uint32_t* amax_a2, const uint32_t* amax_b, float* workspace,
                                    qagnn_stream_t stream) {
  return gemm_tn(tn_product(A1, lda1, Ka1, A2, lda2, Ka2, B, ldb, C, ldc, R, No, a_scale, a_shift, workspace, amax_a1, amax_a2, amax_b, 2),
                 (hipStream_t)stream);
}

extern "C" int qagnn_gemm_tn_graph_f32(const float* A1, int32_t lda1, int32_t Ka1, const float* A2, int32_t lda2, int32_t Ka2, const float* B,
                                       int32_t ldb, float* C, int32_t ldc, int32_t R, int32_t No, const uint32_t* amax_a1, const uint32_t* amax_a2,
                                       const uint32_t* amax_b, int32_t pieces, const qagnn_graph* g, float* workspace, qagnn_stream_t stream) {
  QAGNN_REQUIRE(pieces >= 1 && pieces <= 3, QAGNN_EINVAL, "gemm_tn_graph: pieces=%d (1..3)", pieces);
  const bool h = pieces < 3;
  TnProduct p = tn_product(A1, lda1, Ka1, A2, lda2, Ka2, B, ldb, C, ldc, R, No, nullptr, nullptr, workspace, h ? amax_a1 : nullptr,
                           h ? amax_a2 : nullptr, h ? amax_b : nullptr, h ? pieces : 3);
  p.g = g;
  return gemm_tn(p, (hipStream_t)stream);
}

extern "C" int qagnn_gemm_tn_route_query(int32_t R, int32_t Ka1, int32_t Ka2, int32_t No, int32_t* h_out) {
  QAGNN_REQUIRE(h_out && R > 0 && Ka1 > 0 && Ka2 >= 0 && No > 0, QAGNN_EINVAL, "gemm_tn_route_query: bad arguments");
  alignas(16) static float any[4];
  qagnn_graph any_g = {};
  TnProduct p = tn_product(any, Ka1, Ka1, Ka2 > 0 ? any : nullptr, Ka2, Ka2, any, No, any, No, R, No, nullptr, nullptr, any);
  any_g.N = R;
  any_g.err = reinterpret_cast<int32_t*>(any);
  p.g = &any_g;
  const TnRoute r = tn_route(p);
  h_out[0] = (int)r.family; h_out[1] = r.chunk_rows; h_out[2] = r.nchunks; h_out[3] = r.live ? 1 : 0;
  return QAGNN_OK;
}

extern "C" int qagnn_tn_live_tiles(int32_t on) { return on < 0 ? g_tn_live.load() : g_tn_live.exchange(on ? 1 : 0); }

extern "C" int qagnn_gemm_tn_h1_f32(const float* A1, int32_t lda1, int32_t Ka1, const float* A2, int32_t lda2, int32_t Ka2, const float* B,
                                    int32_t ldb, float* C, int32_t ldc, int32_t R, int32_t No, const float* a_scale, const float* a_shift,
                                    const uint32_t* amax_a1, const uint32_t* amax_a2, const uint32_t* amax_b, float* workspace,
                                    qagnn_stream_t stream) {
  return gemm_tn(tn_product(A1, lda1, Ka1, A2, lda2, Ka2, B, ldb, C, ldc, R, No, a_scale, a_shift, workspace, amax_a1, amax_a2, amax_b, 1),
                 (hipStream_t)stream);
}
```

### qagnn_amd/csrc/gemm_split.hip

```cpp
#include <stdlib.h>

#include <type_traits>

#include "gemm_device.h"

namespace qagnn {

constexpr int SBK = 32, SBM = 128, SWAVES = 4, SRT = 2, STHR = SWAVES * 64;

__device__ __forceinline__ void store_split(uint16_t* __restrict__ img, int img_elems, int off, float4 v) {
  uint32_t a1, a2, a3, b1, b2, b3, c1, c2, c3, d1, d2, d3;
  split3(v.x, a1, a2, a3);
  split3(v.y, b1, b2, b3);
  split3(v.z, c1, c2, c3);
  split3(v.w, d1, d2, d3);
  *reinterpret_cast<uint2*>(img + off) = make_uint2(pack_hi(a1, b1), pack_hi(c1, d1));
  *reinterpret_cast<uint2*>(img + img_elems + off) = make_uint2(pack_hi(a2, b2), pack_hi(c2, d2));
  *reinterpret_cast<uint2*>(img + 2 * img_elems + off) = make_uint2(pack_hi(a3, b3), pack_hi(c3, d3));
}
__device__ __forceinline__ int swz(int row, int k) {
  const int g = (0x78 >> (((row >> 2) & 3) << 1)) & 3;
  return row * SBK + ((((k >> 3) ^ g) & 3) << 3) + (k & 7);
}

// ... 144 lines not shown
    for (int i = 0; i < SRT; ++i) {
      __syncthreads();
      QAGNN_NN_SLAB_FILL(acc[i], (lane >> 4) * 4)
      __syncthreads();
      if constexpr (STATS) {
        const float* const S0 = reinterpret_cast<const float*>(smem_raw);
        QAGNN_NN_SLAB_STATS(S0, i == 0, a.M - (m0 + (w * SRT + i) * 16), a.No)
      }
      QAGNN_NN_SLAB_STORE(m0 + (w * SRT + i) * 16, a.M, a.No)
    }
    if constexpr (STATS) QAGNN_NN_STATS_PUT(false, 1, a.M, a.No)
  }
}

int launch_nn_split(const NnRoute& r, const qagnn_gemm_nn_args& a, const float* B1n, int ldn1, const float* B2n, int ldn2, hipStream_t stream) {
  qagnn_gemm_nn_args b = a;
  b.xcd_remap = 1;
  return dispatch_int<13, 8, 7, 4, 2>(r.nt, [&](auto nt) {
    constexpr int NT = nt.value;
    if constexpr (NT != 8) {
      if (r.stats) {
        k_gemm_nn_split<NT, false, false, true><<<r.grid, STHR, 0, stream>>>(b, B1n, ldn1, B2n, ldn2, r.ntiles);
        QAGNN_LAUNCH_CHECK("k_gemm_nn_split<stats>");
        return QAGNN_OK;
      }
    }
    return dispatch_bool(r.flat, [&](auto flat) {
      return dispatch_bool(r.affine, [&](auto aff) {
        k_gemm_nn_split<NT, aff.value, flat.value><<<r.grid, STHR, 0, stream>>>(b, B1n, ldn1, B2n, ldn2, r.ntiles);
        QAGNN_LAUNCH_CHECK("k_gemm_nn_split");
        return QAGNN_OK;
      });
    });
  });
}


constexpr int TKR = 32, TCP = 40, TTHR = 256;

template <int NP>
__device__ __forceinline__ void store_col8(uint16_t* __restrict__ dst, int img_elems, const float (&x)[8], float s) {
  if constexpr (NP == 2) {
    uint32_t ph[4], pl[4];
#pragma unroll
    for (int e = 0; e < 8; e += 2) split2(x[e], x[e + 1], s, ph[e >> 1], pl[e >> 1]);
    *reinterpret_cast<uint4*>(dst) = make_uint4(ph[0], ph[1], ph[2], ph[3]);
    *reinterpret_cast<uint4*>(dst + img_elems) = make_uint4(pl[0], pl[1], pl[2], pl[3]);
    return;
  }
  if constexpr (NP == 1) {
    uint32_t ph[4];
#pragma unroll
    for (int e = 0; e < 8; e += 2) split1(x[e], x[e + 1], s, ph[e >> 1]);
    *reinterpret_cast<uint4*>(dst) = make_uint4(ph[0], ph[1], ph[2], ph[3]);
    return;
  }
  uint32_t h1[8], h2[8], h3[8];
#pragma unroll
  for (int i = 0; i < 8; ++i) split3(x[i], h1[i], h2[i], h3[i]);
  *reinterpret_cast<uint4*>(dst) = make_uint4(pack_hi(h1[0], h1[1]), pack_hi(h1[2], h1[3]), pack_hi(h1[4], h1[5]), pack_hi(h1[6], h1[7]));
  *reinterpret_cast<uint4*>(dst + img_elems) = make_uint4(pack_hi(h2[0], h2[1]), pack_hi(h2[2], h2[3]), pack_hi(h2[4], h2[5]), pack_hi(h2[6], h2[7]));
  *reinterpret_cast<uint4*>(dst + 2 * img_elems) = make_uint4(pack_hi(h3[0], h3[1]), pack_hi(h3[2], h3[3]), pack_hi(h3[4], h3[5]), pack_hi(h3[6], h3[7]));
}

template <bool AFF, int NP>
__device__ __forceinline__ void store_task(uint16_t* __restrict__ img, int img_elems, int off, const float4 (&r)[8], float s,
                                           float4 sc = make_float4(1.f, 1.f, 1.f, 1.f), float4 sh = make_float4(0.f, 0.f, 0.f, 0.f)) {
#pragma unroll
  for (int j = 0; j < 4; ++j) {
    float x[8];
#pragma unroll
    for (int i = 0; i < 8; ++i) {
      float v = j == 0 ? r[i].x : j == 1 ? r[i].y : j == 2 ? r[i].z : r[i].w;
      if (AFF) {
        const float s_ = j == 0 ? sc.x : j == 1 ? sc.y : j == 2 ? sc.z : sc.w, h = j == 0 ? sh.x : j == 1 ? sh.y : j == 2 ? sh.z : sh.w;
        v = floor_nan(fmaf(v, s_, h), 0.f);
      }
      x[i] = v;
    }
    store_col8<NP>(img + off + j * TCP, img_elems, x, s);
  }
}

template <int KT, int NT, bool AFFINE, bool GATHER, int NP = 3>
__global__ __launch_bounds__(TTHR) __attribute__((amdgpu_waves_per_eu(2, 2))) void k_gemm_tn_split(
    const float* __restrict__ A, int lda, const float* __restrict__ B, int ldb, float* __restrict__ P, int R, int Ka, int No,
    const float* __restrict__ a_scale, const float* __restrict__ a_shift, int chunk_rows, const int64_t* __restrict__ a_rowidx,
    const float* __restrict__ A2, int lda2, int Ka2, TnAmax amax) {
  extern __shared__ __attribute__((aligned(16))) unsigned char smem_tn[];
  constexpr int AC = KT * 16, BC = NT * 16, A_EL = AC * TCP, B_EL = BC * TCP;
  constexpr int MT = KT / 4, REM = KT % 4, RS = (REM * NT + 3) / 4;
  constexpr int A_TW = (AC + 63) / 64, B_TW = (BC + 63) / 64;
  constexpr bool A_MAJOR = A_TW >= B_TW;
  constexpr int MAJ_TW = A_MAJOR ? A_TW : B_TW, MIN_TW = A_MAJOR ? B_TW : A_TW;
  constexpr int MAJ_C = A_MAJOR ? AC : BC, MIN_C = A_MAJOR ? BC : AC, MAJ_EL = A_MAJOR ? A_EL : B_EL, MIN_EL = A_MAJOR ? B_EL : A_EL;
  static_assert(MAJ_TW <= 4 && MIN_TW <= 4, "task-waves per operand");
  static_assert(NP == 3 || !GATHER, "the gathered table goes through the exact split");
  uint16_t* const As = reinterpret_cast<uint16_t*>(smem_tn);
  uint16_t* const Bs = As + NP * A_EL;
  uint16_t* const Maj = A_MAJOR ? As : Bs;
  uint16_t* const Min = A_MAJOR ? Bs : As;
  const int tid = threadIdx.x, lane = tid & 63, w = __builtin_amdgcn_readfirstlane(tid >> 6);
  QAGNN_TN_BLOCK(false, TnLive{})
  const int r_beg = chunk * chunk_rows, r_end = min(R, r_beg + chunk_rows);
  const int ntile = (r_end - r_beg + TKR - 1) / TKR;

  static_assert(!GATHER || A_MAJOR, "the gathered operand is handled as the wide one");
  const __amdgpu_buffer_rsrc_t rsA = __builtin_amdgcn_make_buffer_rsrc(const_cast<float*>(A), 0, GATHER ? 0 : R * lda * 4, 0x00020000);
  const __amdgpu_buffer_rsrc_t rsB = __builtin_amdgcn_make_buffer_rsrc(const_cast<float*>(B), 0, R * ldb * 4, 0x00020000);
  const __amdgpu_buffer_rsrc_t rsMaj = A_MAJOR ? rsA : rsB, rsMin = A_MAJOR ? rsB : rsA;
  const int maj0 = A_MAJOR ? m0 : n0, min0 = A_MAJOR ? n0 : m0, majDim = A_MAJOR ? Ka : No, minDim = A_MAJOR ? No : Ka;
  const uint32_t ldMaj4 = (uint32_t)(A_MAJOR ? lda : ldb) * 4u, ldMin4 = (uint32_t)(A_MAJOR ? ldb : lda) * 4u;

  const int g = lane & 3;
  const int c4j = w * 16 + (lane >> 2);
  const bool maj_act = w < MAJ_TW && c4j * 4 < MAJ_C;
  const bool maj_in = maj_act && maj0 + c4j * 4 < majDim;
  uint32_t maj_voff = maj_in ? ((uint32_t)(r_beg + g * 8) * ldMaj4 + (uint32_t)(maj0 + c4j * 4) * 4u) : OOB;
  const int maj_off = c4j * 4 * TCP + ((g ^ ((c4j ^ (c4j >> 1)) & 1)) << 3);
  float4 scj = make_float4(1.f, 1.f, 1.f, 1.f), shj = make_float4(0.f, 0.f, 0.f, 0.f);
  if (AFFINE && A_MAJOR) {
    const int cc = min(maj0 + c4j * 4, Ka - 4);
    scj = ld4(a_scale + cc);
    shj = ld4(a_shift + cc);
  }

  f32x4s acc[MT > 0 ? MT : 1][NT], accr[RS > 0 ? RS : 1];
#pragma unroll
  for (int i = 0; i < MT; ++i)
#pragma unroll
    for (int j = 0; j < NT; ++j) acc[i][j] = (f32x4s){0.f, 0.f, 0.f, 0.f};
#pragma unroll
  for (int q = 0; q < RS; ++q) accr[q] = (f32x4s){0.f, 0.f, 0.f, 0.f};

  float4 rj[8], rn[8];
  int gi[GATHER ? 8 : 1];
  const float* const Acol = A + min(maj0 + c4j * 4, Ka - 4);
  auto gidx = [&](int t) {
    if constexpr (GATHER) {
      const int r0 = r_beg + t * TKR + g * 8;
#pragma unroll
      for (int i = 0; i < 8; ++i) {
        const int64_t v = a_rowidx[min(r0 + i, R - 1)];
        gi[i] = (maj_in && r0 + i < R && v >= 0) ? (int)v : -1;
      }
    }
  };
  auto gload = [&](int t) {
    if constexpr (GATHER) {
#pragma unroll
      for (int i = 0; i < 8; ++i) {
        const float4 v = ld4(Acol + (int64_t)max(gi[i], 0) * lda);
        rj[i] = gi[i] >= 0 ? v : make_float4(0.f, 0.f, 0.f, 0.f);
      }
    } else {
#pragma unroll
      for (int i = 0; i < 8; ++i) rj[i] = bload<float4>(rsMaj, maj_voff + (uint32_t)i * ldMaj4);
      maj_voff += maj_in ? (uint32_t)TKR * ldMaj4 : 0u;
    }
    const int mk = (w - t) & 3;
    if (mk < MIN_TW) {
      const int c4 = mk * 16 + (lane >> 2);
      const bool in = c4 * 4 < MIN_C && min0 + c4 * 4 < minDim;
      const uint32_t voff = in ? ((uint32_t)(r_beg + t * TKR + g * 8) * ldMin4 + (uint32_t)(min0 + c4 * 4) * 4u) : OOB;
#pragma unroll
      for (int i = 0; i < 8; ++i) rn[i] = bload<float4>(rsMin, voff + (uint32_t)i * ldMin4);
    }
  };
  auto lstore = [&](int t) {
    if (maj_act) store_task<AFFINE && A_MAJOR, NP>(Maj, MAJ_EL, maj_off, rj, A_MAJOR ? sa : sb, scj, shj);
    const int mk = (w - t) & 3;
    if (mk < MIN_TW) {
      const int c4 = mk * 16 + (lane >> 2);
      if (c4 * 4 < MIN_C) {
        const int off = c4 * 4 * TCP + ((g ^ ((c4 ^ (c4 >> 1)) & 1)) << 3);
        float4 sc = make_float4(1.f, 1.f, 1.f, 1.f), sh = make_float4(0.f, 0.f, 0.f, 0.f);
        if (AFFINE && !A_MAJOR) {
          const int cc = min(min0 + c4 * 4, Ka - 4);
          sc = ld4(a_scale + cc);
          sh = ld4(a_shift + cc);
        }
        store_task<AFFINE && !A_MAJOR, NP>(Min, MIN_EL, off, rn, A_MAJOR ? sb : sa, sc, sh);
      }
    }
  };

  const int rd_off = (lane & 15) * TCP + (((lane >> 4) ^ ((((lane & 15) >> 2) ^ ((lane & 15) >> 3)) & 1)) << 3);
#define QAGNN_SIX(C, AF, BF) C = mfma_pieces<NP>(AF, BF, C);

  gidx(0);
  gload(0);
  for (int t = 0; t < ntile; ++t) {
    __syncthreads();
    lstore(t);
    gidx(t + 1);
    __syncthreads();
    gload(t + 1);
    __builtin_amdgcn_s_setprio(1);
    u32x4s af[MT > 0 ? MT : 1][NP];
#pragma unroll
    for (int i = 0; i < MT; ++i)
#pragma unroll
      for (int p = 0; p < NP; ++p) af[i][p] = *reinterpret_cast<const u32x4s*>(As + p * A_EL + (w + 4 * i) * 16 * TCP + rd_off);
#pragma unroll
    for (int j = 0; j < NT; ++j) {
      u32x4s bf[NP];
#pragma unroll
      for (int p = 0; p < NP; ++p) bf[p] = *reinterpret_cast<const u32x4s*>(Bs + p * B_EL + j * 16 * TCP + rd_off);
#pragma unroll
      for (int i = 0; i < MT; ++i) {
        f32x4s c = acc[i][j];
        QAGNN_SIX(c, af[i], bf)
        acc[i][j] = c;
      }
    }
#pragma unroll
    for (int s = 0; s < RS; ++s) {
      const int q = w + 4 * s;
      if (q < REM * NT) {
        const int ir = q / NT, jr = q % NT;
        u32x4s ar[NP], br[NP];
#pragma unroll
        for (int p = 0; p < NP; ++p) {
          ar[p] = *reinterpret_cast<const u32x4s*>(As + p * A_EL + (4 * MT + ir) * 16 * TCP + rd_off);
          br[p] = *reinterpret_cast<const u32x4s*>(Bs + p * B_EL + jr * 16 * TCP + rd_off);
        }
        f32x4s c = accr[s];
        QAGNN_SIX(c, ar, br)
        accr[s] = c;
      }
    }
    __builtin_amdgcn_s_setprio(0);
  }
#undef QAGNN_SIX

  float* const Pc = P + (int64_t)chunk * ka_total * No;
  const float inv = NP <= 2 ? h2_inv_scale(fa, fb) : 1.f;
  auto put = [&](int strip, int j, const f32x4s& c) { QAGNN_TN_PUT(false, strip, j, c) };
#pragma unroll
  for (int i = 0; i < MT; ++i)
#pragma unroll
    for (int j = 0; j < NT; ++j) put(w + 4 * i, j, acc[i][j]);
#pragma unroll
  for (int s = 0; s < RS; ++s) {
    const int q = w + 4 * s;
    if (q < REM * NT) put(4 * MT + q / NT, q % NT, accr[s]);
  }
// ... 178 lines not shown
    else asm volatile("" : "+v"(F[0]));                                                  \
  }
#define QAGNN_TNW_SIX(C, AF, BF) C = mfma_pieces<NP>(AF, BF, C);

  QAGNN_TNW_BAR
  for (int t = 0; t < ntile4; ++t) {
    if (t >= ntile) {
      QAGNN_TNW_BAR
      continue;
    }
    const uint32_t cur = (uint32_t)((t & 1) * IMG_B);
    const uint32_t amaj = maj0 + cur, amin = min0 + cur;
    u32x4s mf[MT][NP], nf[3][NP];
    __builtin_amdgcn_s_setprio(1);
#pragma unroll
    for (int s_ = 0; s_ < MT; ++s_) QAGNN_TNW_FRAG(mf[s_], amaj, s_ * 4 * STRIP_B, MAJ_PIECE)
    QAGNN_TNW_FRAG(nf[0], amin, 0, MIN_PIECE)
    if constexpr (MINT > 1) QAGNN_TNW_FRAG(nf[1], amin, STRIP_B, MIN_PIECE)
#pragma unroll
    for (int n = 0; n < MINT; ++n) {
      u32x4s(&bfn)[NP] = nf[n % 3];
      if (n + 2 < MINT) {
        QAGNN_TNW_FRAG(nf[(n + 2) % 3], amin, (n + 2) * STRIP_B, MIN_PIECE)
        QAGNN_TNW_WAIT(bfn, 2);
      } else if (n + 1 < MINT) {
        QAGNN_TNW_WAIT(bfn, 1);
      } else {
        QAGNN_TNW_WAIT(bfn, 0);
      }
      if (n == 0) {
#pragma unroll
        for (int s_ = 0; s_ < MT; ++s_) QAGNN_TNW_TOUCH(mf[s_])
      }
#pragma unroll
      for (int s_ = 0; s_ < MT; ++s_) {
        f32x4s c = acc[s_][n];
        if constexpr (MAJ_A) { QAGNN_TNW_SIX(c, mf[s_], bfn) } else { QAGNN_TNW_SIX(c, bfn, mf[s_]) }
        acc[s_][n] = c;
      }
      __builtin_amdgcn_sched_barrier(0);
    }
#pragma unroll
    for (int s_ = 0; s_ < RS; ++s_) {
      if (ci + 4 * s_ < REM * MINT) {
        u32x4s ar[NP], br[NP];
        QAGNN_TNW_FRAG(ar, rem_maj[s_] + cur, 0, MAJ_PIECE)
        QAGNN_TNW_FRAG(br, rem_min[s_] + cur, 0, MIN_PIECE)
        QAGNN_TNW_WAIT(ar, 0);
        QAGNN_TNW_TOUCH(br)
        f32x4s c = accr[s_];
        if constexpr (MAJ_A) { QAGNN_TNW_SIX(c, ar, br) } else { QAGNN_TNW_SIX(c, br, ar) }
        accr[s_] = c;
      }
    }
    __builtin_amdgcn_s_setprio(0);
    QAGNN_TNW_BAR
  }
#undef QAGNN_TNW_FRAG
#undef QAGNN_TNW_WAIT
#undef QAGNN_TNW_TOUCH
#undef QAGNN_TNW_SIX
#undef QAGNN_TNW_BAR

  float* const Pc = LIVE ? P + (int64_t)min(max(slot.pslot, 0), lv.S - 1) * ka_total * BC : P + (int64_t)chunk * ka_total * No;
  const float inv = NP <= 2 ? h2_inv_scale(fa, fb) : 1.f;
  auto put = [&](int maj_strip, int min_tile, const f32x4s& c) { QAGNN_TN_PUT(LIVE, MAJ_A ? maj_strip : min_tile, MAJ_A ? min_tile : maj_strip, c) };
#pragma unroll
  for (int s_ = 0; s_ < MT; ++s_)
#pragma unroll
    for (int n = 0; n < MINT; ++n) put(ci + 4 * s_, n, acc[s_][n]);
#pragma unroll
  for (int s_ = 0; s_ < RS; ++s_) {
    const int q = ci + 4 * s_;
    if (q < REM * MINT) put(4 * MT + q / MINT, q % MINT, accr[s_]);
  }
}

#define QAGNN_TN_ARGS p.A1, p.lda1, p.B, p.ldb, p.ws, p.R, p.Ka1, p.No
static TnLive tn_live_args(const TnRoute& r, const TnProduct& p) {
  if (!r.live) return TnLive{nullptr, nullptr, 0, 0, 0};
  const LiveTiles lt = live_tiles_of(p.g);
  return TnLive{lt.list, lt.n_live, lt.n_tiles, 3 * r.nchunks, r.chunk_rows / TKR};
}
static TnAmax tn_amax(const TnRoute& r, const TnProduct& p) {
  return r.np == 3 ? TnAmax{nullptr, nullptr, nullptr} : TnAmax{p.amax[0], p.two ? p.amax[1] : nullptr, p.amax[2]};
}
template <int KT, int NT, int NP = 3, bool LIVE = false>
static int launch_tn_ws_i(const TnRoute& r, const TnProduct& p, hipStream_t stream) {
  static_assert(!LIVE || NT * 16 == TN_LIVE_BC, "the live-tile form is built for 208-column blocks");
  constexpr int lds = 2 * NP * (KT * 16 + NT * 16) * TCP * (int)sizeof(uint16_t) + 64 + (LIVE ? (TN_LIST_CAP + 8) * (int)sizeof(int) : 0);
  if (int rc = raise_lds_limit<k_gemm_tn_ws<KT, NT, NP, LIVE>>(lds, "k_gemm_tn_ws")) return rc;
  k_gemm_tn_ws<KT, NT, NP, LIVE><<<r.grid, WTHR, lds, stream>>>(QAGNN_TN_ARGS, r.chunk_rows, p.A2, p.lda2, p.Ka2, tn_amax(r, p), tn_live_args(r, p));
  QAGNN_LAUNCH_CHECK("k_gemm_tn_ws");
  return QAGNN_OK;
}
template <int KT, int NT, bool AFFINE, bool GATHER = false, int NP = 3>
static int launch_tn_split_i(const TnRoute& r, const TnProduct& p, hipStream_t stream) {
  constexpr int lds = NP * (KT * 16 + NT * 16) * TCP * (int)sizeof(uint16_t);
  if (int rc = raise_lds_limit<k_gemm_tn_split<KT, NT, AFFINE, GATHER, NP>>(lds, "k_gemm_tn_split")) return rc;
  k_gemm_tn_split<KT, NT, AFFINE, GATHER, NP><<<r.grid, TTHR, lds, stream>>>(QAGNN_TN_ARGS, p.a_scale, p.a_shift, r.chunk_rows, p.a_rowidx, p.A2, p.lda2, p.Ka2, tn_amax(r, p));
  QAGNN_LAUNCH_CHECK("k_gemm_tn_split");
  return QAGNN_OK;
}
#undef QAGNN_TN_ARGS

int launch_tn_ws(const TnRoute& r, const TnProduct& p, hipStream_t stream) {
  return dispatch_int<3, 2, 1>(r.np, [&](auto np) {
    return dispatch_bool(r.live, [&](auto live) { return launch_tn_ws_i<7, 13, np.value, live.value>(r, p, stream); });
  });
}
int launch_tn_split(const TnRoute& r, const TnProduct& p, hipStream_t stream) {
  if (r.gather) return launch_tn_split_i<13, 7, false, true>(r, p, stream);
  return dispatch_bool(r.kt == 7, [&](auto wide_b) {
    return dispatch_bool(r.affine, [&](auto aff) {
      return dispatch_int<3, 2, 1>(r.np, [&](auto np) {
        constexpr int KT = wide_b.value ? 7 : 13;
        return launch_tn_split_i<KT, 20 - KT, aff.value, false, np.value>(r, p, stream);
      });
    });
  });
}

}
```

### qagnn_amd/csrc/graph_prep.hip

```cpp
#include <stdarg.h>

#include <stdlib.h>

#include "common.h"

namespace qagnn {

static thread_local char g_err[512] = "";
void set_error(const char* fmt, ...) {
  va_list ap;
  va_start(ap, fmt);
  vsnprintf(g_err, sizeof(g_err), fmt, ap);
  va_end(ap);
}

__device__ __forceinline__ int true_edges(const int* __restrict__ E_dev, int E) {
  return E_dev ? min(max(*E_dev, 0), E) : E;
}

__global__ void k_decode_count(const int64_t* __restrict__ edge_index, int64_t ld_edge, const int64_t* __restrict__ edge_type,
                               const int64_t* __restrict__ node_type, int N, int E_cap, const int* __restrict__ E_dev, int R, int T,
                               int* __restrict__ es, int* __restrict__ et, int* __restrict__ ec, int* __restrict__ cnt_s,
                               int* __restrict__ cnt_t, int* __restrict__ err, int block_n) {
  const int e = blockIdx.x * blockDim.x + threadIdx.x;
// ... 368 lines not shown
}

__global__ __launch_bounds__(1024) void k_chunk_counts(const int* __restrict__ gc_cnt, int* __restrict__ nch, int n) {
  const int i = blockIdx.x * blockDim.x + threadIdx.x;
  if (i < n) nch[i] = (gc_cnt[i] + QAGNN_CLS_CHUNK - 1) / QAGNN_CLS_CHUNK;
}
__global__ __launch_bounds__(1024) void k_scan_pairs(const int* gc_cnt, int* gcptr, const int* nch, int* chunkptr, int n) {
  if (blockIdx.x == 0) block_exclusive_scan(gc_cnt, gcptr, n);
  else block_exclusive_scan(nch, chunkptr, n);
}
__global__ void k_chunk_fill(const int* __restrict__ gcptr, const int* __restrict__ chunkptr, int* __restrict__ chunk_cls,
                             int* __restrict__ chunk_beg, int* __restrict__ chunk_len, int* __restrict__ n_chunks, int C, int n) {
  const int i = blockIdx.x * blockDim.x + threadIdx.x;
  if (i == 0) *n_chunks = chunkptr[n];
  if (i >= n) return;
  const int b = gcptr[i], e = gcptr[i + 1];
  int k = chunkptr[i];
  for (int p = b; p < e; p += QAGNN_CLS_CHUNK, ++k) {
    chunk_cls[k] = i % C;
    chunk_beg[k] = p;
    chunk_len[k] = min(QAGNN_CLS_CHUNK, e - p);
  }
}

static inline void cls_groups(int Ep, int* nblk, int* gb, int* NG) {
  *nblk = cdiv(Ep, CLS_BLK);
  *gb = cdiv(*nblk, QAGNN_CLS_GROUPS) > 1 ? cdiv(*nblk, QAGNN_CLS_GROUPS) : 1;
  *NG = cdiv(*nblk, *gb);
}

static inline int64_t up4(int64_t x) { return (x + 3) & ~(int64_t)3; }

__global__ void k_xcd_partition(const int* __restrict__ rowptr_s, int N, int cap, int balance, int* __restrict__ base) {
  const int nbk = (N + 3) >> 2, lane = threadIdx.x;
  int cand = 0;
  if (lane >= 1 && lane <= 7) {
    if (balance) {
      const long long W = 4ll * rowptr_s[N] - 3ll * N, target = (W * lane + 7) / 8;
      int lo = 0, hi = nbk;
      while (lo < hi) {
        const int mid = (lo + hi) >> 1, nd = min(4 * mid, N);
        if (4ll * rowptr_s[nd] - 3ll * nd >= target) hi = mid; else lo = mid + 1;
      }
      cand = lo;
    } else {
      const int q = nbk >> 3, r = nbk & 7;
      cand = lane < r ? lane * (q + 1) : r * (q + 1) + (lane - r) * q;
    }
  }
  __shared__ int c[8];
  if (lane < 8) c[lane] = cand;
  __syncthreads();
  if (lane == 0) {
    int prev = 0;
    base[0] = 0;
    for (int k = 1; k < 8; ++k) {
      int b = c[k];
      b = min(b, prev + cap);
      b = max(b, nbk - (8 - k) * cap);
      b = max(b, prev);
      base[k] = b;
      prev = b;
    }
    base[8] = nbk;
  }
}

__global__ __launch_bounds__(1024) void k_live_tiles(const int* __restrict__ rowptr_s, const int* __restrict__ rowptr_t, int N, int T,
                                                     int* __restrict__ live, int* __restrict__ rank, int* __restrict__ list,
                                                     int* __restrict__ n_live) {
  for (int t = threadIdx.x; t < T; t += 1024) {
    const int r0 = t * 32, r1 = min(N, r0 + 32);
    live[t] = (rowptr_s[r1] - rowptr_s[r0] != r1 - r0 || rowptr_t[r1] - rowptr_t[r0] != r1 - r0) ? 1 : 0;
  }
  __syncthreads();
  block_exclusive_scan(live, rank, T);
  __syncthreads();
  const int L = rank[T];
  for (int t = threadIdx.x; t < T; t += 1024) {
    const int r = rank[t];
    list[live[t] ? r : L + (t - r)] = t;
  }
  if (threadIdx.x == 0) *n_live = L;
}

__global__ void k_tn_work_table(const int* __restrict__ n_live, int T, int S, int chunk_tiles, int* __restrict__ out) {
  const int u = blockIdx.x * blockDim.x + threadIdx.x;
  const int L = min(max(n_live[0], 0), T);
  const TnWork w = tn_work(S, T, L, chunk_tiles);
  if (u == 0) { out[0] = w.cK; out[1] = w.cM; out[2] = T; out[3] = L; }
  if (u >= S) return;
  const TnSlot s = tn_slot(w, S, T, u);
  int* o = out + 4 + 5 * u;
  o[0] = s.cb; o[1] = s.list; o[2] = s.beg; o[3] = s.cnt; o[4] = s.pslot;
}

__global__ void k_zero16(int4* __restrict__ p, int64_t n16) {
  for (int64_t i = (int64_t)blockIdx.x * blockDim.x + threadIdx.x; i < n16; i += (int64_t)gridDim.x * blockDim.x) p[i] = make_int4(0, 0, 0, 0);
}

}

using namespace qagnn;

static int xcd_partition(qagnn_graph* g, hipStream_t stream) {
  k_xcd_partition<<<1, 64, 0, stream>>>(g->rowptr_s, g->N, edge_xcd_cap(g->N), 1, g->err + 4);
  QAGNN_LAUNCH_CHECK("k_xcd_partition");
  return QAGNN_OK;
}

static int live_tiles(qagnn_graph* g, int32_t* rank, hipStream_t stream) {
  const LiveTiles lt = live_tiles_of(g);
  k_live_tiles<<<1, 1024, 0, stream>>>(g->rowptr_s, g->rowptr_t, g->N, lt.n_tiles, lt.live, rank, lt.list, lt.n_live);
  QAGNN_LAUNCH_CHECK("k_live_tiles");
  return QAGNN_OK;
}

static hipError_t zero_range(void* p, size_t bytes, hipStream_t stream) {
  if (bytes % 16 != 0 || !aligned16(p)) return hipErrorInvalidValue;
  const int64_t n16 = (int64_t)(bytes / 16);
  if (n16 == 0) return hipSuccess;
  int blocks = (int)((n16 + 255) / 256);
  if (blocks > 1024) blocks = 1024;
  k_zero16<<<blocks, 256, 0, stream>>>((int4*)p, n16);
  return hipGetLastError();
}

struct carved {
  int32_t *eid_t, *gc_cnt, *gcptr, *nch, *cnt_s, *cnt_t, *es, *et, *ec, *tmp_s, *tmp_t, *srcpos, *hist, *live_rank;
  int nblk, gb, NG, pairs;
};
static carved carve(qagnn_graph* g, int32_t* storage, int N, int E, int R, int T, int block_n) {
  carved cv;
  const int Ep = E + N, C = R * T * T + T;
  cls_groups(Ep, &cv.nblk, &cv.gb, &cv.NG);
  cv.pairs = cv.NG * C;
  const int maxch = Ep / QAGNN_CLS_CHUNK + cv.pairs + 1;
  int32_t* p = storage;
  auto take = [&](int64_t n) { int32_t* r = p; p += up4(n); return r; };
  g->N = N; g->E = E; g->Ep = Ep; g->R = R; g->T = T; g->C = C; g->max_chunks = maxch; g->block_n = block_n;
  g->n_groups = cv.NG;
  g->rowptr_s = take(N + 1); g->rowptr_t = take(N + 1);
  g->tgt_s = take(Ep); g->src_s = take(Ep); g->cls_s = take(Ep); g->eid_s = take(Ep);
  g->src_t = take(Ep); g->tgt_t = take(Ep); g->cls_t = take(Ep); g->pos_t = take(Ep);
  g->src_c = take(Ep); g->tgt_c = take(Ep); g->pos_c = take(Ep);
  cv.eid_t = take(Ep);
  cv.gc_cnt = take(cv.pairs + 1); cv.gcptr = take(cv.pairs + 1);
  g->chunkptr = take(cv.pairs + 1);
  cv.nch = take(cv.pairs + 1);
  g->cls_count = take(C);
  g->chunk_cls = take(maxch); g->chunk_beg = take(maxch); g->chunk_len = take(maxch);
  g->n_chunks = take(4); g->err = take(16);
  take(4 + 2 * up4(cdiv(N, 32)));
  cv.cnt_s = take(N); cv.cnt_t = take(N);
  cv.es = take(Ep); cv.et = take(Ep); cv.ec = take(Ep);
  cv.tmp_s = take(Ep); cv.tmp_t = take(Ep); cv.srcpos = take(Ep);
  cv.hist = take((int64_t)cv.nblk * C);
  cv.live_rank = take(cdiv(N, 32) + 1);
  return cv;
}

static int class_pass(qagnn_graph* g, int32_t* hist, int32_t* gc_cnt, int32_t* gcptr, int32_t* nch, int nblk, int gb, int NG, int pairs,
                      hipStream_t stream) {
  const int TB = 256, C = g->C;
  const int* Ep = g->rowptr_s + g->N;
  k_cls_hist<<<nblk, 256, C * sizeof(int), stream>>>(g->cls_s, hist, g->cls_count, Ep, C);
// ... 55 lines not shown
  const int64_t Ep64 = (int64_t)E + N, C64 = (int64_t)R * T * T + T;
  QAGNN_REQUIRE(Ep64 < (1ll << 30), QAGNN_EUNSUPPORTED, "%s: E+N=%lld too large", who, (long long)Ep64);
  QAGNN_REQUIRE(C64 <= 8192, QAGNN_EUNSUPPORTED, "%s: %lld edge classes > 8192", who, (long long)C64);
  const int Ep = (int)Ep64;
  carved cv = carve(g, storage, N, E, R, T, block_n);
  int32_t *cnt_s = cv.cnt_s, *cnt_t = cv.cnt_t, *es = cv.es, *et = cv.et, *ec = cv.ec, *tmp_s = cv.tmp_s, *tmp_t = cv.tmp_t;
  int32_t *srcpos = cv.srcpos, *eid_t = cv.eid_t, *hist = cv.hist, *gc_cnt = cv.gc_cnt, *gcptr = cv.gcptr, *nch = cv.nch;
  const int nblk = cv.nblk, gb = cv.gb, NG = cv.NG, pairs = cv.pairs;

  hipError_t he = zero_range(g->cls_count, (size_t)((char*)es - (char*)g->cls_count), stream);
  if (he != hipSuccess) { set_error("%s: k_zero16 failed: %s", who, hipGetErrorString(he)); return QAGNN_EHIP; }
  const int TB = 256;
  k_decode_count<<<cdiv(Ep, TB), TB, 0, stream>>>(edge_index, ld_edge, edge_type, node_type, N, E, E_dev, R, T, es, et, ec, cnt_s, cnt_t,
                                                   g->err, block_n);
  QAGNN_LAUNCH_CHECK("k_decode_count");
  k_scan3<<<2, 1024, 0, stream>>>(cnt_s, g->rowptr_s, N, cnt_t, g->rowptr_t, N, nullptr, nullptr, 0);
  QAGNN_LAUNCH_CHECK("k_scan3");
  k_fill<<<cdiv(Ep, TB), TB, 0, stream>>>(es, et, g->rowptr_s, g->rowptr_t, cnt_s, cnt_t, tmp_s, tmp_t, N, E, E_dev);
  QAGNN_LAUNCH_CHECK("k_fill");
  k_sort_segments<<<cdiv(2 * (int64_t)N, 4), 256, 0, stream>>>(g->rowptr_s, g->rowptr_t, tmp_s, tmp_t, g->eid_s, eid_t, srcpos, N);
  QAGNN_LAUNCH_CHECK("k_sort_segments");
  k_payload<<<cdiv(Ep, TB), TB, 0, stream>>>(es, et, ec, g->eid_s, eid_t, srcpos, g->tgt_s, g->src_s, g->cls_s, g->src_t,
                                              g->tgt_t, g->cls_t, g->pos_t, N, E, E_dev);
  QAGNN_LAUNCH_CHECK("k_payload");
  int rc = xcd_partition(g, stream);
  if (rc != QAGNN_OK) return rc;
  if ((rc = live_tiles(g, cv.live_rank, stream)) != QAGNN_OK) return rc;
  return class_pass(g, hist, gc_cnt, gcptr, nch, nblk, gb, NG, pairs, stream);
}

extern "C" int qagnn_graph_prep_blocked(qagnn_graph* g, int32_t* storage, const int64_t* edge_index, const int64_t* edge_type,
                                        const int64_t* node_type, int32_t N, int32_t E, int32_t R, int32_t T, int32_t block_n,
                                        qagnn_stream_t stream_) {
  return prep_sorted("graph_prep", g, storage, edge_index, E, edge_type, node_type, N, E, nullptr, R, T, block_n, (hipStream_t)stream_);
}

extern "C" int qagnn_graph_prep_cap(qagnn_graph* g, int32_t* storage, const int64_t* edge_index, int64_t ld_edge,
                                    const int64_t* edge_type, const int64_t* node_type, int32_t N, int32_t E_cap, const int32_t* E_dev,
                                    int32_t R, int32_t T, int32_t block_n, qagnn_stream_t stream_) {
  QAGNN_REQUIRE(E_dev, QAGNN_EINVAL, "graph_prep_cap: null edge-count pointer");
  return prep_sorted("graph_prep_cap", g, storage, edge_index, ld_edge, edge_type, node_type, N, E_cap, E_dev, R, T, block_n,
                     (hipStream_t)stream_);
}

template <class Blobs>
static int from_blobs(const char* who, qagnn_graph* g, int32_t* storage, const Blobs src, const int32_t* edge_off, const int64_t* node_type,
                      int32_t B, int32_t n, int32_t E, int32_t R, int32_t T, hipStream_t stream) {
  QAGNN_REQUIRE(B > 0 && n > 0 && E >= 0 && R > 0 && T > 0, QAGNN_EINVAL, "%s: bad sizes B=%d n=%d E=%d R=%d T=%d", who, B, n, E, R, T);
  QAGNN_REQUIRE(n < 65536 && (int64_t)R * T * T < 65536, QAGNN_EUNSUPPORTED, "%s: n=%d or R*T*T=%d does not fit the 16-bit blob fields", who, n, R * T * T);
  QAGNN_REQUIRE((size_t)(2 * (n + 1)) * sizeof(int) <= 64 * 1024, QAGNN_EUNSUPPORTED, "%s: n=%d node slots per sample exceed the LDS scan", who, n);
  QAGNN_REQUIRE(aligned16(storage), QAGNN_EINVAL, "%s: storage must be 16-byte aligned", who);
  const int64_t N64 = (int64_t)B * n, Ep64 = (int64_t)E + N64, C64 = (int64_t)R * T * T + T;
  QAGNN_REQUIRE(Ep64 < (1ll << 30), QAGNN_EUNSUPPORTED, "%s: E+N=%lld too large", who, (long long)Ep64);
  QAGNN_REQUIRE(C64 <= 8192, QAGNN_EUNSUPPORTED, "%s: %lld edge classes > 8192", who, (long long)C64);
  carved cv = carve(g, storage, (int)N64, E, R, T, n);
  hipError_t he = zero_range(g->cls_count, (size_t)((char*)cv.es - (char*)g->cls_count), stream);
  if (he != hipSuccess) { set_error("%s: k_zero16 failed: %s", who, hipGetErrorString(he)); return QAGNN_EHIP; }
  k_blob_assemble<Blobs><<<B, 256, (size_t)(2 * (n + 1)) * sizeof(int), stream>>>(src, edge_off, node_type, n, B, R, T, g->rowptr_s,
                                                                                  g->tgt_s, g->src_s, g->cls_s, g->eid_s, g->rowptr_t, g->src_t,
                                                                                  g->tgt_t, g->cls_t, g->pos_t, g->err);
  QAGNN_LAUNCH_CHECK("k_blob_assemble");
  int rc = xcd_partition(g, stream);
  if (rc != QAGNN_OK) return rc;
  if ((rc = live_tiles(g, cv.live_rank, stream)) != QAGNN_OK) return rc;
  return class_pass(g, cv.hist, cv.gc_cnt, cv.gcptr, cv.nch, cv.nblk, cv.gb, cv.NG, cv.pairs, stream);
}

extern "C" int qagnn_graph_from_blobs(qagnn_graph* g, int32_t* storage, const int32_t* blobs, const int32_t* blob_off,
                                      const int32_t* edge_off, const int64_t* node_type, int32_t B, int32_t n, int32_t E, int32_t R,
                                      int32_t T, qagnn_stream_t stream_) {
  QAGNN_REQUIRE(g && storage && blobs && blob_off && edge_off && node_type, QAGNN_EINVAL, "graph_from_blobs: null pointer");
  return from_blobs("graph_from_blobs", g, storage, packed_blobs{blobs, blob_off}, edge_off, node_type, B, n, E, R, T, (hipStream_t)stream_);
}

extern "C" int qagnn_tn_work_table(const qagnn_graph* g, int32_t S, int32_t chunk_tiles, int32_t* out, qagnn_stream_t stream_) {
  QAGNN_REQUIRE(g && out && g->err && g->N > 0, QAGNN_EINVAL, "tn_work_table: null pointer");
  const LiveTiles lt = live_tiles_of(g);
  QAGNN_REQUIRE(S >= 3 && S % 3 == 0 && chunk_tiles > 0, QAGNN_EINVAL, "tn_work_table: S=%d (a multiple of 3), chunk_tiles=%d", S, chunk_tiles);
  k_tn_work_table<<<cdiv(S, 256), 256, 0, (hipStream_t)stream_>>>(lt.n_live, lt.n_tiles, S, chunk_tiles, out);
  QAGNN_LAUNCH_CHECK("k_tn_work_table");
  return QAGNN_OK;
}

static int check_store(const char* who, const qagnn_store* st) {
  QAGNN_REQUIRE(st, QAGNN_EINVAL, "%s: null store", who);
  QAGNN_REQUIRE(st->blobs && st->blob_off && st->concept_ids && st->node_type && st->node_scores && st->adj_len, QAGNN_EINVAL,
                "%s: null pointer in the store", who);
  QAGNN_REQUIRE(st->S > 0 && st->n > 0 && st->W >= 0, QAGNN_EINVAL, "%s: bad store sizes S=%d n=%d W=%lld", who, st->S, st->n, (long long)st->W);
  return QAGNN_OK;
}

extern "C" int qagnn_store_gather(const qagnn_store* st, const int32_t* ids, int32_t B, int64_t* concept_ids_out, int64_t* node_type_out,
                                  float* node_scores_out, int64_t* adj_len_out, int32_t* edge_off_out, int32_t* err, qagnn_stream_t stream_) {
  int rc = check_store("store_gather", st);
  if (rc != QAGNN_OK) return rc;
  QAGNN_REQUIRE(ids && concept_ids_out && node_type_out && node_scores_out && adj_len_out && edge_off_out && err, QAGNN_EINVAL,
                "store_gather: null pointer");
  QAGNN_REQUIRE(B > 0 && B <= 32768, QAGNN_EINVAL, "store_gather: B=%d outside 1..32768", B);
  k_store_gather<<<B + 1, 256, 0, (hipStream_t)stream_>>>(st->blob_off, st->concept_ids, st->node_type, st->node_scores, st->adj_len, st->S,
                                                          st->n, ids, B, concept_ids_out, node_type_out, node_scores_out, adj_len_out,
                                                          edge_off_out, err);
  QAGNN_LAUNCH_CHECK("k_store_gather");
  return QAGNN_OK;
}

extern "C" int qagnn_graph_from_store(qagnn_graph* g, int32_t* storage, const qagnn_store* st, const int32_t* ids, const int32_t* edge_off,
                                      const int64_t* node_type, int32_t B, int32_t E, int32_t R, int32_t T, qagnn_stream_t stream_) {
  int rc = check_store("graph_from_store", st);
  if (rc != QAGNN_OK) return rc;
  QAGNN_REQUIRE(g && storage && ids && edge_off && node_type, QAGNN_EINVAL, "graph_from_store: null pointer");
  return from_blobs("graph_from_store", g, storage, store_blobs{st->blobs, st->blob_off, ids, st->S}, edge_off, node_type, B, st->n, E, R, T,
                    (hipStream_t)stream_);
}
```

### qagnn_amd/data_utils.py

```python
import os
import pickle

import numpy as np
import torch


def record_to_graph(rec, max_node_num):
    adj, concepts = rec['adj'], np.asarray(rec['concepts'])
    qm, am = np.asarray(rec['qmask'], dtype=bool), np.asarray(rec['amask'], dtype=bool)
    cid2score = rec['cid2score']
    n = int(max_node_num)
    if len(concepts) != len(set(concepts.tolist())):
        raise AssertionError('duplicate concept ids in a record')
    qam = qm | am
    if not (len(qam) > 0 and qam[0]):
        raise AssertionError('first concept must be a question/answer concept')
    if len(qam) > 1 and np.any(qam[1:] & ~qam[:-1]):
        raise AssertionError('question/answer concepts must precede all other concepts')

    num_concept = min(len(concepts), n - 1) + 1
    concept_ids = np.full(n, 1, dtype=np.int64)
    concept_ids[0] = 0
    concept_ids[1:num_concept] = concepts[:num_concept - 1].astype(np.int64) + 1
    node_scores = np.zeros(n, dtype=np.float32)
    if cid2score is not None:
        for j in range(num_concept):
            node_scores[j] = np.float32(cid2score[int(concept_ids[j]) - 1])
    node_type_ids = np.full(n, 2, dtype=np.int64)
    node_type_ids[0] = 3
    k_real = num_concept - 1
    sl = node_type_ids[1:num_concept]
    sl[qm[:k_real]] = 0
    sl[am[:k_real]] = 1

    n_node = adj.shape[1]
    half_n_rel = adj.shape[0] // n_node
    row = np.asarray(adj.row, dtype=np.int64)
    col = np.asarray(adj.col, dtype=np.int64)
    i = row // n_node + 2
    j = row % n_node + 1
    k = col + 1
    lim = min(len(qm), num_concept)
    qn = np.nonzero(qm[:lim])[0].astype(np.int64) + 1
    an = np.nonzero(am[:lim])[0].astype(np.int64) + 1
    half_n_rel += 2
    i = np.concatenate([i, np.zeros(len(qn), np.int64), np.ones(len(an), np.int64)])
    j = np.concatenate([j, np.zeros(len(qn) + len(an), np.int64)])
    k = np.concatenate([k, qn, an])
    keep = (j < n) & (k < n)
    i, j, k = i[keep], j[keep], k[keep]
    edge_type = np.concatenate([i, i + half_n_rel])
    edge_index = np.stack([np.concatenate([j, k]), np.concatenate([k, j])], axis=0)
    return len(concepts), num_concept, concept_ids, node_type_ids, node_scores, edge_index, edge_type, half_n_rel


def records_to_tensors(records, max_node_num, num_choice):
    n_samples = len(records)
    assert n_samples % num_choice == 0
    concept_ids = torch.empty((n_samples, max_node_num), dtype=torch.long)
    node_type_ids = torch.empty((n_samples, max_node_num), dtype=torch.long)
    node_scores = torch.empty((n_samples, max_node_num, 1), dtype=torch.float)
    adj_lengths = torch.empty((n_samples,), dtype=torch.long)
    adj_lengths_ori = torch.empty((n_samples,), dtype=torch.long)
    edge_index, edge_type = [], []
    half_n_rel = 0
    for idx, rec in enumerate(records):
        lo, nc, cid, nt, ns, ei, et, half_n_rel = record_to_graph(rec, max_node_num)
        adj_lengths_ori[idx], adj_lengths[idx] = lo, nc
        concept_ids[idx] = torch.from_numpy(cid)
        node_type_ids[idx] = torch.from_numpy(nt)
        node_scores[idx, :, 0] = torch.from_numpy(ns)
        edge_index.append(torch.from_numpy(ei))
        edge_type.append(torch.from_numpy(et))
    return adj_lengths_ori, concept_ids, node_type_ids, node_scores, adj_lengths, edge_index, edge_type, half_n_rel


def load_sparse_adj_data_with_contextnode(adj_pk_path, max_node_num, num_choice, args=None):
    cache_path = adj_pk_path + '.loaded_cache'
    if os.path.exists(cache_path):
        with open(cache_path, 'rb') as f:
            (adj_lengths_ori, concept_ids, node_type_ids, node_scores, adj_lengths,
             edge_index, edge_type, half_n_rel) = pickle.load(f)
    else:
        with open(adj_pk_path, 'rb') as fin:
            records = pickle.load(fin)
        (adj_lengths_ori, concept_ids, node_type_ids, node_scores, adj_lengths,
         edge_index, edge_type, half_n_rel) = records_to_tensors(records, max_node_num, num_choice)
        with open(cache_path, 'wb') as f:
            pickle.dump([adj_lengths_ori, concept_ids, node_type_ids, node_scores, adj_lengths,
                         edge_index, edge_type, half_n_rel], f)

    ori = adj_lengths_ori.float()
    mu = ori.mean().item()
    sigma = float(np.sqrt(((ori - mu) ** 2).mean().item()))
    print('| ori_adj_len: mu {:.2f} sigma {:.2f} | adj_len: {:.2f} | prune_rate: {:.2f} | qc_num: {:.2f} | ac_num: {:.2f} |'.format(
        mu, sigma, adj_lengths.float().mean().item(), (adj_lengths_ori > adj_lengths).float().mean().item(),
        (node_type_ids == 0).float().sum(1).mean().item(), (node_type_ids == 1).float().sum(1).mean().item()))

    edge_index = [list(edge_index[q:q + num_choice]) for q in range(0, len(edge_index), num_choice)]
    edge_type = [list(edge_type[q:q + num_choice]) for q in range(0, len(edge_type), num_choice)]
    concept_ids, node_type_ids, node_scores, adj_lengths = [
        x.view(-1, num_choice, *x.size()[1:]) for x in (concept_ids, node_type_ids, node_scores, adj_lengths)]
    return concept_ids, node_type_ids, node_scores, adj_lengths, (edge_index, edge_type)

# ... 507 lines not shown
```

### qagnn_amd/modeling_qagnn.py

```python
import math

import torch
import torch.nn as nn
import torch.nn.functional as F

from . import ops
from .layers import GELU, MLP, CustomizedEmbedding, MultiheadAttPoolLayer, gelu


def make_one_hot(labels, C):
    return F.one_hot(labels, C).to(torch.float32)


def _fp32_region(fn):
    import functools

    @functools.wraps(fn)
    def wrapped(self, *args, **kwargs):
        dev_type = 'cuda' if torch.cuda.is_available() else 'cpu'
        if not torch.is_autocast_enabled(dev_type):
            return fn(self, *args, **kwargs)
        cast = lambda t: t.float() if torch.is_tensor(t) and t.is_floating_point() else t
        with torch.autocast(dev_type, enabled=False):
            return fn(self, *[cast(a) for a in args], **{k: cast(v) for k, v in kwargs.items()})
    return wrapped


_LAYOUTS = {}


def head_layout(d, device):
    key = (d, str(device))
    if key not in _LAYOUTS:
        _LAYOUTS[key] = ops.HeadLayout(d, device)
    return _LAYOUTS[key]


def _pad2(W, L):
    Wt = L.pad(L.pad(W).t())
    return Wt, Wt.t().contiguous()


_CLASS_FEATS = {}


def bn_momentum(bn):
    if bn.momentum is None:
        raise NotImplementedError('BatchNorm1d(momentum=None) (cumulative average) is not implemented by the HIP path')
    return bn.momentum


def bn_running(bn, L, rows, training):
    if not (training and bn.track_running_stats):
        return None
    R = float(rows)
    return (bn.running_mean, bn.running_var, bn.num_batches_tracked, L.dense_pos, bn_momentum(bn), R / max(R - 1.0, 1.0))


def edge_class_features(n_etype, n_ntype, device, dtype=torch.float32):
    key = (n_etype, n_ntype, str(device), dtype)
    if key not in _CLASS_FEATS:
        _CLASS_FEATS[key] = _edge_class_features(n_etype, n_ntype, device).to(dtype)
    return _CLASS_FEATS[key]


MAX_NTYPE, MAX_EDGE_CLASSES = 4, 8192


def check_type_counts(n_ntype, n_etype):
    if not 1 <= n_ntype <= MAX_NTYPE:
        raise NotImplementedError(f'n_ntype={n_ntype}: the hop kernels handle 1..{MAX_NTYPE} node types (the reference value is 4)')
    if n_etype < 1 or n_etype * n_ntype * n_ntype + n_ntype > MAX_EDGE_CLASSES:
        raise NotImplementedError(f'n_etype={n_etype}, n_ntype={n_ntype}: {n_etype * n_ntype * n_ntype + n_ntype} edge classes; '
                                  f'the graph preparation handles 2..{MAX_EDGE_CLASSES}')


def _edge_class_features(n_etype, n_ntype, device):
    R, T = n_etype, n_ntype
    C = R * T * T + T
    c = torch.arange(C, device=device)
    is_self = c >= R * T * T
    et = torch.where(is_self, torch.full_like(c, R), c // (T * T))
    hd = torch.where(is_self, c - R * T * T, (c // T) % T)
    tl = torch.where(is_self, c - R * T * T, c % T)
    feat = torch.zeros(C, R + 1 + 2 * T, device=device)
    ar = torch.arange(C, device=device)
    feat[ar, et] = 1
    feat[ar, R + 1 + hd] = 1
    feat[ar, R + 1 + T + tl] = 1
# ... 294 lines not shown
                ekem = ops.split_cols(ops.linear_nn(tab_p, We_t_all, We_all, bias=be_all), self.k)
                TT = ops.split_cols(torch.addmm(bias_all, temb, Wtype_all), self.k)
            accS, accX = (ops.GradAcc(), ops.GradAcc()) if self.k > 0 else (None, None)
            if stack_native:
                prms, runnings = [], []
                for l, (layer, pk) in enumerate(zip(self.gnn_layers, per_layer)):
                    bn = layer.mlp[1]
                    Wx_t, Wx, Ws_t, Ws = pk[:4]
                    W1t, W1p, b1, gam, bet, W2t, W2p, b2, rm_p, rv_p = pk[8:]
                    prms.append((Wx_t, Wx, Ws_t, Ws, TT[l], ekem[l], W1t, W1p, b1, gam, bet, W2t, W2p, b2, rm_p, rv_p))
                    runnings.append(bn_running(bn, L, Hp.size(0), self.training))
                if infer:
                    Xp = ops.stack_infer(Hp, S, ntype, graph, L.HP, 1.0 / math.sqrt(self.gnn_layers[0].dim_per_head), prms, bn0.eps,
                                         tab_col=(self._tab_col, L.ones_col))
                else:
                    Xp = ops.gat_stack(Hp, S, ntype, graph, L.HP, 1.0 / math.sqrt(self.gnn_layers[0].dim_per_head), prms,
                                       self.training or not bn0.track_running_stats, bn0.eps, self.dropout_rate if self.training else 0.0,
                                       runnings, accX=accX, tab_col=(self._tab_col, L.ones_col))
                per_layer = []
            for l, (layer, pk) in enumerate(zip(self.gnn_layers, per_layer)):
                Xp, _ = layer.hop(Xp, None, graph, None, L, apply_act=True, p_drop=self.dropout_rate, typed=(temb, ntype, S),
                                  packed=pk, tables=(TT[l], ekem[l]), acc=(accX if l == 0 else None, True, accS, l == 0),
                                  tab_col=self._tab_col)
            Y = ops.linear_nn(Hp, Vh_t, Vh, Xp, Vx_t, Vx, bias=bVh + bVx, acc=(accX, False, None, False))
        out = ops.gelu_dropout(Y, self.dropout_rate, self.training)
        if padded_output:
            return out.view(bs, n, L.DP)
        return L.unpad(out).view(bs, n, d)


class QAGNN(nn.Module):

    def __init__(self, args, k, n_ntype, n_etype, sent_dim, n_concept, concept_dim, concept_in_dim, n_attention_head,
                 fc_dim, n_fc_layer, p_emb, p_gnn, p_fc, pretrained_concept_emb=None, freeze_ent_emb=True, init_range=0.02):
        super().__init__()
        self.init_range = init_range
        self.concept_emb = CustomizedEmbedding(concept_num=n_concept, concept_out_dim=concept_dim, use_contextualized=False,
                                               concept_in_dim=concept_in_dim, pretrained_concept_emb=pretrained_concept_emb,
                                               freeze_ent_emb=freeze_ent_emb)
        self.svec2nvec = nn.Linear(sent_dim, concept_dim)
        self.concept_dim = concept_dim
        self.activation = GELU()
        self.gnn = QAGNN_Message_Passing(args, k=k, n_ntype=n_ntype, n_etype=n_etype, input_size=concept_dim,
                                         hidden_size=concept_dim, output_size=concept_dim, dropout=p_gnn)
        self.pooler = MultiheadAttPoolLayer(n_attention_head, sent_dim, concept_dim)
        self.fc = MLP(concept_dim + sent_dim + concept_dim, fc_dim, 1, n_fc_layer, p_fc, layer_norm=True)
        self.dropout_e = nn.Dropout(p_emb)
        self.dropout_fc = nn.Dropout(p_fc)
        self._input_plan = None
        if init_range > 0:
            self.apply(self._init_weights)

    def _init_weights(self, module):
        if isinstance(module, (nn.Linear, nn.Embedding)):
            module.weight.data.normal_(mean=0.0, std=self.init_range)
            if hasattr(module, 'bias') and module.bias is not None:
                module.bias.data.zero_()
        elif isinstance(module, nn.LayerNorm):
            module.bias.data.zero_()
            module.weight.data.fill_(1.0)

    def forward(self, sent_vecs, concept_ids, node_type_ids, node_scores, adj_lengths, adj, emb_data=None, cache_output=False):
        if concept_ids is None and node_type_ids is None and node_scores is None and adj_lengths is None:
            concept_ids, node_type_ids, node_scores, adj_lengths = adj.fields()
        dev = node_type_ids.device
        n = node_type_ids.size(1)
        ce = self.concept_emb
        fused_input = (emb_data is None and not ce.use_contextualized and hasattr(ce, 'cpt_transform') and ce.scale == 1.0
                       and not ce.emb.weight.requires_grad and ce.emb.weight.size(1) % 16 == 0)
        graph, join_graph = None, None
        node_type_ids = node_type_ids.contiguous()
        if fused_input and self.gnn.k > 0:
            graph, join_graph = ops.graph_prep_async(adj, node_type_ids.reshape(-1), self.gnn.n_etype, self.gnn.n_ntype, n)
        node_scores, mask, ridx = ops.kernels().node_prep(node_scores.contiguous(), adj_lengths.contiguous(), node_type_ids,
                                                          concept_ids.contiguous(), table_rows=ce.emb.weight.size(0) if fused_input else 0)
        node_scores = node_scores.unsqueeze(2)
        if fused_input:
            L = head_layout(self.concept_dim, dev)
            if self._input_plan is None:
                self._input_plan = ops.GatherPlan()
            Wc_t, Wc, bc = self._input_plan((ce.cpt_transform.weight, ce.cpt_transform.bias),
                                            lambda ids: [L.pad(ids[0].t()), L.pad(ids[0].t()).t().contiguous(), L.pad(ids[1])])
            gnn_input = ops.concept_input(ce.emb.weight, ridx, Wc_t, bc, L.pad(self.svec2nvec(sent_vecs)), n,
                                          self.dropout_e.p, self.training, Wc=Wc)
        else:
            gnn_input0 = self.activation(self.svec2nvec(sent_vecs)).unsqueeze(1)
            gnn_input1 = self.concept_emb(concept_ids[:, 1:] - 1, emb_data).to(dev)
            gnn_input = self.dropout_e(torch.cat([gnn_input0, gnn_input1], dim=1))

        Lh = head_layout(self.concept_dim, dev)
        if join_graph is not None:
            join_graph()
        gnn_output = self.gnn(gnn_input, adj, node_type_ids, node_scores, graph=graph, padded_input=fused_input, padded_output=True)
        pl, fc = self.pooler, self.fc
        if (fc.num_layers == 0 and fc.output_size == 1 and gnn_output.is_contiguous() and gnn_output.size(2) == Lh.DP
                and ops.head_supported(pl.n_head, pl.d_v, Lh.DP, n)):
            lin = fc.layers[0]
            logits, pool_attn = pl(sent_vecs, gnn_output, mask, layout=Lh, head=(sent_vecs, lin.weight, lin.bias, self.concept_dim, self.dropout_fc.p))
            if cache_output:
                self.concept_ids, self.adj, self.pool_attn = concept_ids, adj, pool_attn
            return logits, pool_attn
        Z_vecs = Lh.unpad(gnn_output[:, 0])
        graph_vecs, pool_attn = self.pooler(sent_vecs, gnn_output, mask, layout=Lh)
        if cache_output:
            self.concept_ids, self.adj, self.pool_attn = concept_ids, adj, pool_attn
        concat = self.dropout_fc(torch.cat((graph_vecs, sent_vecs, Z_vecs), 1))
        return self.fc(concat), pool_attn


def batch_graph(edge_index_init, edge_type_init, n_nodes):
    from .data_utils import batch_graph as _bg
    return _bg(edge_index_init, edge_type_init, n_nodes)


class LM_QAGNN(nn.Module):

    def __init__(self, args, model_name, k, n_ntype, n_etype, n_concept, concept_dim, concept_in_dim, n_attention_head,
                 fc_dim, n_fc_layer, p_emb, p_gnn, p_fc, pretrained_concept_emb=None, freeze_ent_emb=True, init_range=0.0,
                 encoder_config={}, encoder=None):
        super().__init__()
        if encoder is None:
            from modeling.modeling_encoder import TextEncoder
            encoder = TextEncoder(model_name, **encoder_config)
        self.encoder = encoder
        self.decoder = QAGNN(args, k, n_ntype, n_etype, self.encoder.sent_dim, n_concept, concept_dim, concept_in_dim,
                             n_attention_head, fc_dim, n_fc_layer, p_emb, p_gnn, p_fc,
                             pretrained_concept_emb=pretrained_concept_emb, freeze_ent_emb=freeze_ent_emb, init_range=init_range)

    def forward(self, *inputs, layer_id=-1, cache_output=False, detail=False):
        bs, nc = inputs[0].size(0), inputs[0].size(1)
        edge_index_orig, edge_type_orig = inputs[-2:]
        flat = [x.reshape(bs * nc, *x.shape[2:]) for x in inputs[:-2]]
        *lm_inputs, concept_ids, node_type_ids, node_scores, adj_lengths = flat
        dev = node_type_ids.device
        from .data_utils import GRAPH_HOLDERS
        if isinstance(edge_index_orig, GRAPH_HOLDERS):
            adj = edge_index_orig
        else:
            edge_index = [g for row in edge_index_orig for g in row]
            edge_type = [g for row in edge_type_orig for g in row]
            edge_index, edge_type = batch_graph(edge_index, edge_type, concept_ids.size(1))
            adj = (edge_index.to(dev), edge_type.to(dev))
        sent_vecs, all_hidden_states = self.encoder(*lm_inputs, layer_id=layer_id)
        logits, attn = self.decoder(sent_vecs.to(dev), concept_ids, node_type_ids, node_scores, adj_lengths, adj,
                                    emb_data=None, cache_output=cache_output)
        logits = logits.view(bs, nc)
        if not detail:
            return logits, attn
        if hasattr(edge_index_orig, 'nested_lists'):
            edge_index_orig, edge_type_orig = edge_index_orig.nested_lists()
        return logits, attn, concept_ids.view(bs, nc, -1), node_type_ids.view(bs, nc, -1), edge_index_orig, edge_type_orig

    batch_graph = staticmethod(batch_graph)
```

### qagnn_amd/ops.py

```python
import math
import os
import struct
import weakref

import torch
from torch.amp import custom_bwd, custom_fwd

_fwd = custom_fwd(device_type='cuda', cast_inputs=torch.float32)
_bwd = custom_bwd(device_type='cuda')

_K = None


def kernels():
    global _K
    if _K is None:
        from ._lib import HipKernels
        _K = HipKernels()
    return _K


def set_kernels(k):
    global _K
    old, _K = _K, k
# ... 853 lines not shown
    def backward(ctx, dlogits, _dattn_unused):
        u, K3, attn, attn_d, z, out, asum, BDv, bv, sent, w1 = ctx.saved_tensors
        inv_temp, p_attn, seed_attn, d, p_pool, p_fc, seed_pool, seed_fc, w_shape = ctx.cfg
        Kn = kernels()
        B, NO = out.shape
        Ds, n = sent.size(1), attn.size(2)
        L = NO + Ds + d
        dz, dattn, dout, dsent, dZ, part = Kn.head_post_bwd(dlogits.reshape(-1).contiguous(), out, asum, BDv, bv, sent, K3, d, w1, p_pool, p_fc,
                                                            seed_pool, seed_fc, n, ctx.needs_input_grad[9])
        cols = Kn.colsum(part)[0]
        dBDv = torch.mm(z.reshape(B, -1).t(), dout) if ctx.needs_input_grad[7] else None
        dK, du, dc = Kn.pool_attn_bwd(u, K3, inv_temp, p_attn, seed_attn, attn, attn_d, dz, dattn)
        Kn.add_row0(dK, dZ)
        return (du, dc, dK, None, None, None, None, dBDv, cols[L:L + NO], dsent, cols[:L].reshape(w_shape), cols[L + NO:L + NO + 1],
                None, None, None, None, None)


def head_supported(nh, dv, width, n):
    K = kernels()
    lim = getattr(K, 'HEAD_LIMITS', None)
    return (lim is not None and H_HEADS == 4 and nh <= lim[0] and nh * dv <= lim[1] and width <= lim[2] and width % 4 == 0
            and pool_attention_supported(nh, width, n))


def head(u, cvec, K3, mask, inv_temp, p_attn, BDv, bv, sent, w_fc, b_fc, d, p_pool, p_fc, training):
    p_attn, p_pool, p_fc = (float(p_attn), float(p_pool), float(p_fc)) if training else (0.0, 0.0, 0.0)
    return HeadFn.apply(u, cvec, K3, mask, inv_temp, p_attn, next_seed() if p_attn > 0 else 0, BDv, bv, sent, w_fc, b_fc, int(d),
                        p_pool, p_fc, next_seed() if p_pool > 0 else 0, next_seed() if p_fc > 0 else 0)


def pool_attention_supported(nh, width, n):
    lim = getattr(kernels(), 'POOL_LIMITS', None)
    return lim is not None and nh <= lim[0] and width <= lim[1] and width % 4 == 0 and n <= lim[2]


def table_amax(K, table):
    if not (getattr(K, 'gemm_split', 1) >= 2 and getattr(K, 'name', '') == 'hip') or table.requires_grad or table.numel() % 4 != 0 \
            or table.data_ptr() % 16 != 0 or not table.is_contiguous():
        return None
    w = amax_lookup(table)
    if w is None:
        if table.is_cuda and torch.cuda.is_current_stream_capturing():
            return None
        e = _AMAX_NOTES.get(id(table))
        w = K.absmax(table.detach().view(-1))
        if e is not None and e[0]() is table and e[2].shape == w.shape and e[2].device == w.device:
            w = e[2].copy_(w)
        amax_note(table, w)
    if _table_words[0] is not None and not any(t is table for t, _ in _table_words[0]):
        _table_words[0].append((table, w))
    return w


_table_words = [None]


class table_words:

    def __init__(self, sink):
        self.sink = sink

    def __enter__(self):
        self.old, _table_words[0] = _table_words[0], self.sink
        return self.sink

    def __exit__(self, *exc):
        _table_words[0] = self.old
        return False


def refresh_table_words(pairs):
    for table, word in pairs:
        if amax_lookup(table) is word:
            continue
        w = table_amax(kernels(), table)
        if w is not None and w is not word:
            word.copy_(w)


class ConceptInputFn(torch.autograd.Function):

    @staticmethod
    @_fwd
    def forward(ctx, emb_w, rowidx, Wc_t, bc, ctx_pre, n, p, seed, Wc=None):
        K = kernels()
        tam = table_amax(K, emb_w) if rowidx.numel() >= pack_min_rows(K) else None
        pre = K.gemm_nn(emb_w, Wc_t, bias=bc, a_rowidx=rowidx, B1n=Wc if Wc is not None else Wc_t.t().contiguous(),
                        **(dict(a_amax1=tam) if tam is not None else {}))
        B = ctx_pre.size(0)
        pre.view(B, n, -1)[:, 0] = ctx_pre
        ctx.save_for_backward(emb_w, rowidx, pre)
        ctx.cfg = (n, p, seed)
        if _wants_amax(K, pre):
            Hp, word = K.gelu_dropout_fwd(pre, p, seed, amax=True)
            return amax_note(Hp, word)
        return K.gelu_dropout_fwd(pre, p, seed)

    @staticmethod
    @_bwd
    def backward(ctx, dHp):
        K = kernels()
        emb_w, rowidx, pre = ctx.saved_tensors
        n, p, seed = ctx.cfg
        dpre = K.gelu_dropout_bwd(pre, dHp.contiguous(), p, seed)
        dctx = dpre.view(-1, n, dpre.size(1))[:, 0].contiguous()
        dWc_t, cs = K.gemm_tn(emb_w, dpre, a_rowidx=rowidx), K.colsum(dpre)
        dbc = cs[0] - dctx.sum(0)
        return None, None, dWc_t, dbc, dctx, None, None, None, None


def concept_input(emb_w, rowidx, Wc_t, bc, ctx_pre, n, p, training, Wc=None):
    p = float(p) if training else 0.0
    return ConceptInputFn.apply(emb_w, rowidx, Wc_t, bc, ctx_pre, n, p, next_seed() if p > 0 else 0, Wc)


QSCALE = lambda dh: 1.0 / math.sqrt(dh)


LOSS_KINDS = ('cross_entropy', 'margin_rank')


class ChoiceLossFn(torch.autograd.Function):

    @staticmethod
    def forward(ctx, logits, labels, K, kind, margin, weight, stats):
        loss, g = K.choice_loss(logits, labels, kind, margin, weight, stats)
        ctx.K = K
        ctx.save_for_backward(g)
        return loss.view(())

    @staticmethod
    @torch.autograd.function.once_differentiable
    def backward(ctx, dloss):
        (g,) = ctx.saved_tensors
        return ctx.K.choice_loss_bwd(g, dloss.reshape(1).contiguous()), None, None, None, None, None, None


_WEIGHT_WORDS = {}


def _weight_word(weight, device):
    key = (device, float(weight))
    word = _WEIGHT_WORDS.get(key)
    if word is None:
        if len(_WEIGHT_WORDS) >= 256:
            _WEIGHT_WORDS.clear()
        word = _WEIGHT_WORDS[key] = torch.full((1,), float(weight), dtype=torch.float32, device=device)
    return word


def _loss_provider(logits):
    K = _K
    if K is None:
        if not logits.is_cuda:
            return None
        K = kernels()
    if logits.dtype != torch.float32 or logits.dim() != 2 or not hasattr(K, 'choice_loss'):
        return None
    if not logits.is_cuda and getattr(K, 'name', 'hip') == 'hip':
        return None
    return K


def choice_loss_torch(logits, labels, kind='cross_entropy', margin=0.1, weight=None, stats=None):
    Q, nc = logits.shape
    valid = (labels >= 0) & (labels < nc)
    lab = labels.clamp(0, nc - 1).unsqueeze(1)
    xl = logits.gather(1, lab)
    if kind == 'cross_entropy':
        rows = torch.logsumexp(logits, dim=1) - xl.squeeze(1)
        total, denom = torch.where(valid, rows, torch.zeros_like(rows)).sum(), Q
    else:
        hinge = (-(xl - logits) + margin).clamp_min(0)
        pairs = (torch.arange(nc, device=logits.device).unsqueeze(0) != lab) & valid.unsqueeze(1)
        total, denom = torch.where(pairs, hinge, torch.zeros_like(hinge)).sum(), Q * (nc - 1)
    loss = total / denom
    if weight is not None:
        loss = loss * weight.reshape(()).to(loss.dtype)
    if stats is not None:
        with torch.no_grad():
            stats += torch.stack([loss.detach().float().double(), torch.ones((), dtype=torch.float64, device=loss.device)])
    return loss


def choice_loss(logits, labels, kind='cross_entropy', margin=0.1, weight=None, stats=None):
    if kind not in LOSS_KINDS:
        raise ValueError(f'unknown loss {kind!r}: one of {LOSS_KINDS}')
    assert logits.dim() == 2 and labels.dim() == 1 and labels.size(0) == logits.size(0), 'logits [Q, nc], labels [Q]'
    if kind == 'margin_rank' and logits.size(1) < 2:
        raise ValueError('margin_rank needs at least two choices')
    if weight is not None and not isinstance(weight, torch.Tensor):
        weight = _weight_word(weight, logits.device)
    margin = struct.unpack('f', struct.pack('f', float(margin)))[0]
    K = _loss_provider(logits)
    if K is None:
        return choice_loss_torch(logits, labels, kind, margin, weight, stats)
# ... 4 lines not shown
```

Measured before the change: 45110 QA-subgraphs/s.

## Skip all-pad row tiles in concept-input weight-gradient GEMM via rank-1 pad correction

In the concept-input backward, rows whose gathered embedding index is the pad concept are grouped into 32-row tiles. Tiles made entirely of pad rows are left out of the gathered TN GEMM, and their contribution is restored as a rank-1 update: the pad embedding row times the column sum of dpre over those tiles. That column sum is produced by an extended colsum kernel alongside the ordinary bias sum. The aim is to avoid redundant gather-GEMM work on padded node slots, at the cost of an extra single-block tile-classification kernel and added routing complexity.

```diff
diff --git a/include/qagnn_hip_tn.h b/include/qagnn_hip_tn.h
--- a/include/qagnn_hip_tn.h
+++ b/include/qagnn_hip_tn.h
@@ -14,6 +14,15 @@
 int qagnn_tn_work_table(const qagnn_graph* g, int32_t S, int32_t chunk_tiles, int32_t* out, qagnn_stream_t stream);
 int qagnn_tn_live_tiles(int32_t on);
 
+int64_t qagnn_pad_tiles_elems(int32_t R);
+int qagnn_pad_tiles(const int64_t* a_rowidx, int32_t R, int64_t pad_row, int32_t* tiles, qagnn_stream_t stream);
+int qagnn_colsum_pad_f32(const float* X, int32_t ldx, int32_t R, int32_t Cc, const int32_t* tiles, float* out, float* workspace,
+                         qagnn_stream_t stream);
+int qagnn_gemm_tn_pad_f32(const float* A, int32_t lda, const float* B, int32_t ldb, float* C, int32_t ldc, int32_t R, int32_t Ka, int32_t No,
+                          const int64_t* a_rowidx, int32_t accumulate, int64_t pad_row, const int32_t* tiles, const float* pad_sum,
+                          float* workspace, qagnn_stream_t stream);
+int qagnn_gemm_tn_pad_route_query(int32_t R, int32_t Ka, int32_t No, int32_t* h_out );
+
 #ifdef __cplusplus
 }
 #endif
diff --git a/qagnn_amd/_lib.py b/qagnn_amd/_lib.py
--- a/qagnn_amd/_lib.py
+++ b/qagnn_amd/_lib.py
@@ -21,7 +21,8 @@
            'qagnn_timing_enable', 'qagnn_timing_read', 'qagnn_gemm_tn_h1_f32', 'qagnn_gelu_dropout_bwd_amax_f32', 'qagnn_packed_min_rows',
            'qagnn_radam_step_scaled_f32', 'qagnn_grad_norm_workspace_elems', 'qagnn_grad_norm_f32', 'qagnn_scale_multi_f32', 'qagnn_graph_prep_cap',
            'qagnn_store_gather', 'qagnn_graph_from_store']
-EXPORTS_TN = ['qagnn_gemm_tn_graph_f32', 'qagnn_gemm_tn_route_query', 'qagnn_tn_work_table', 'qagnn_tn_live_tiles']
+EXPORTS_TN = ['qagnn_gemm_tn_graph_f32', 'qagnn_gemm_tn_route_query', 'qagnn_tn_work_table', 'qagnn_tn_live_tiles',
+              'qagnn_pad_tiles_elems', 'qagnn_pad_tiles', 'qagnn_colsum_pad_f32', 'qagnn_gemm_tn_pad_f32', 'qagnn_gemm_tn_pad_route_query']
 EXPORTS_INFER = ['qagnn_infer_version', 'qagnn_bn_relu_absmax_scratch_elems', 'qagnn_bn_relu_absmax_f32', 'qagnn_stack_infer_f32',
                  'qagnn_choice_eval_f32']
 EXPORTS_LOSS = ['qagnn_loss_version', 'qagnn_choice_loss_f32', 'qagnn_choice_loss_bwd_f32']
@@ -128,6 +129,12 @@
     lib.qagnn_gemm_tn_route_query.argtypes = [_i32, _i32, _i32, _i32, _vp]
     lib.qagnn_tn_work_table.argtypes = [C.POINTER(qagnn_graph), _i32, _i32, _vp, _vp]
     lib.qagnn_tn_live_tiles.argtypes = [_i32]
+    lib.qagnn_pad_tiles_elems.restype = _i64
+    lib.qagnn_pad_tiles_elems.argtypes = [_i32]
+    lib.qagnn_pad_tiles.argtypes = [_vp, _i32, _i64, _vp, _vp]
+    lib.qagnn_colsum_pad_f32.argtypes = [_vp, _i32, _i32, _i32, _vp, _vp, _vp, _vp]
+    lib.qagnn_gemm_tn_pad_f32.argtypes = [_vp, _i32, _vp, _i32, _vp, _i32, _i32, _i32, _i32, _vp, _i32, _i64, _vp, _vp, _vp, _vp]
+    lib.qagnn_gemm_tn_pad_route_query.argtypes = [_i32, _i32, _i32, _vp]
     lib.qagnn_absmax_f32.argtypes = [_vp, _i64, _vp, _vp]
     lib.qagnn_zero_words.argtypes = [_vp, _i64, _vp]
     lib.qagnn_timing_enable.argtypes = [_i32]
@@ -720,6 +727,44 @@
         self._check(self.lib.qagnn_tn_work_table(C.byref(graph.c), S, chunk_tiles, out.data_ptr(), self._stream()), 'qagnn_tn_work_table')
         return out
 
+    def pad_tiles(self, a_rowidx, pad_row):
+        assert a_rowidx.dtype == torch.long and a_rowidx.is_contiguous() and a_rowidx.is_cuda and pad_row >= 0
+        R = a_rowidx.numel()
+        tiles = torch.empty(self.lib.qagnn_pad_tiles_elems(R), dtype=torch.int32, device=a_rowidx.device)
+        self._check(self.lib.qagnn_pad_tiles(a_rowidx.data_ptr(), R, int(pad_row), tiles.data_ptr(), self._stream()), 'qagnn_pad_tiles')
+        return tiles
+
+    def pad_tiles_views(self, tiles, R):
+        T = (R + 31) // 32
+        T4 = (T + 3) & ~3
+        return tiles[:1], tiles[4:4 + T], tiles[4 + T4:4 + T4 + T]
+
+    def colsum_pad(self, X, tiles):
+        _chkp(X, 'X')
+        R, Cc = X.shape
+        out = torch.empty((2, Cc), dtype=torch.float32, device=X.device)
+        ws = torch.empty(self.lib.qagnn_colreduce_workspace_elems(R, Cc, 2), dtype=torch.float32, device=X.device)
+        self._check(self.lib.qagnn_colsum_pad_f32(X.data_ptr(), _ld(X), R, Cc, tiles.data_ptr(), out.data_ptr(), ws.data_ptr(), self._stream()),
+                    'qagnn_colsum_pad_f32')
+        return out
+
+    def gemm_tn_pad(self, A, B, a_rowidx, pad_row, tiles, pad_sum, out=None, accumulate=False):
+        _chkp(A, 'A'), _chkp(B, 'B')
+        Ka = A.size(1)
+        R, No = B.shape
+        assert a_rowidx.numel() == R and a_rowidx.dtype == torch.long and pad_sum.numel() == No and pad_sum.is_contiguous()
+        assert out is not None or not accumulate
+        out, ws = self._tn_out_ws(R, Ka, No, out, A.device)
+        rc = self.lib.qagnn_gemm_tn_pad_f32(A.data_ptr(), _ld(A), B.data_ptr(), _ld(B), out.data_ptr(), _ld(out), R, Ka, No, a_rowidx.data_ptr(),
+                                            1 if accumulate else 0, int(pad_row), tiles.data_ptr(), pad_sum.data_ptr(), ws.data_ptr(), self._stream())
+        self._check(rc, 'qagnn_gemm_tn_pad_f32')
+        return out
+
+    def tn_pad_route_query(self, R, Ka, No):
+        out = (_i32 * 4)()
+        self._check(self.lib.qagnn_gemm_tn_pad_route_query(R, Ka, No, C.cast(out, _vp)), 'qagnn_gemm_tn_pad_route_query')
+        return tuple(out)
+
     def tn_live_tiles(self, on):
         return int(self.lib.qagnn_tn_live_tiles(int(on)))
 
diff --git a/qagnn_amd/csrc/common.h b/qagnn_amd/csrc/common.h
--- a/qagnn_amd/csrc/common.h
+++ b/qagnn_amd/csrc/common.h
@@ -64,6 +64,7 @@
   const uint32_t* amax[3]; int np;
   float* ws;
   const qagnn_graph* g;
+  int64_t pad_row; const int32_t* pad_tiles; const float* pad_sum;
 };
 inline TnProduct tn_product(const float* A1, int lda1, int Ka1, const float* A2, int lda2, int Ka2, const float* B, int ldb, float* C, int ldc, int R,
                             int No, const float* a_scale, const float* a_shift, float* ws, const uint32_t* amax_a1 = nullptr,
@@ -73,6 +74,7 @@
   if (A2 && Ka2 > 0) { p.A2 = A2; p.lda2 = lda2; p.Ka2 = Ka2; p.two = true; }
   p.B = B; p.ldb = ldb; p.C = C; p.ldc = ldc; p.R = R; p.No = No; p.a_scale = a_scale; p.a_shift = a_shift; p.ws = ws;
   p.amax[0] = amax_a1; p.amax[1] = amax_a2; p.amax[2] = amax_b; p.np = np;
+  p.pad_row = -1;
   return p;
 }
 enum class TnFamily { RUNTIME, STRIP, SPLIT, WS, PAIR };
@@ -83,6 +85,7 @@
   int chunk_rows, nchunks;
   bool sum_by4;
   bool live;
+  bool pad;
   dim3 grid;
   int64_t ws_elems;
 };
@@ -143,6 +146,29 @@
   return LiveTiles{T, p, p + 4, p + 4 + T4};
 }
 
+struct TnPad { const int* list; const int* n_ord; const int* ord; int T, chunk_tiles; };
+struct PadTiles { int n_tiles; int32_t *n_ord, *ord, *list, *rank; };
+inline int pad_tiles_count(int R) { return (int)(((int64_t)R + 31) / 32); }
+inline int64_t pad_tiles_elems(int R) { const int64_t T4 = (pad_tiles_count(R) + 3) & ~3; return 4 + 3 * T4 + 4; }
+inline PadTiles pad_tiles_of(int32_t* p, int R) {
+  const int T = pad_tiles_count(R), T4 = (T + 3) & ~3;
+  return PadTiles{T, p, p + 4, p + 4 + T4, p + 4 + 2 * T4};
+}
+struct TnPadSlot { int list, beg, cnt; };
+__host__ __device__ inline TnPadSlot tn_pad_slot(int S, int T, int O, int chunk_tiles, int j) {
+  TnPadSlot s;
+  O = O < 0 ? 0 : (O > T ? T : O);
+  if (O >= T) {
+    s.list = 0; s.beg = j * chunk_tiles < T ? j * chunk_tiles : T; s.cnt = T - s.beg < chunk_tiles ? T - s.beg : chunk_tiles;
+  } else {
+    const int q = O / S, r = O % S;
+    s.list = 1; s.beg = j * q + (j < r ? j : r); s.cnt = q + (j < r ? 1 : 0);
+  }
+  return s;
+}
+int launch_sum_chunks_pad(const float* P, float* C, int ldc, int rows, int No, int nchunks, int accumulate, const float* pad_vec,
+                          const float* pad_sum, const TnPad& pd, hipStream_t stream);
+
 int launch_gelu_dropout(const float* X, const float* dY, float* out, int64_t n, float p, uint64_t seed, uint32_t* amax, float* amax_part,
                         hipStream_t stream);
 int64_t gelu_amax_scratch_elems(int64_t n);
diff --git a/qagnn_amd/csrc/elementwise.hip b/qagnn_amd/csrc/elementwise.hip
--- a/qagnn_amd/csrc/elementwise.hip
+++ b/qagnn_amd/csrc/elementwise.hip
@@ -10,8 +10,9 @@
                                                    int R, int Cc, const int64_t* __restrict__ rowidx, int groups,
                                                    const float* __restrict__ mean, const float* __restrict__ invstd,
                                                    const float* __restrict__ scale, const float* __restrict__ shift,
-                                                   const float* __restrict__ roww, float* __restrict__ part) {
-  constexpr int NOUT = MODE == 0 ? 4 : (MODE == 2 ? 2 : 1);
+                                                   const float* __restrict__ roww, float* __restrict__ part,
+                                                   const int* __restrict__ tile_ord = nullptr) {
+  constexpr int NOUT = MODE == 0 ? 4 : (MODE >= 2 ? 2 : 1);
   __shared__ __attribute__((aligned(16))) float red[4][NOUT][256];
   const int lane = threadIdx.x & 63, w = threadIdx.x >> 6;
   const int col = blockIdx.x * 256 + lane * 4;
@@ -22,8 +23,11 @@
 #pragma unroll
   for (int o = 0; o < NOUT; ++o) acc[o] = make_float4(0.f, 0.f, 0.f, 0.f);
   float4 mu = make_float4(0.f, 0.f, 0.f, 0.f), is = mu, sc = mu, sh = mu;
-  if (act && MODE >= 1) mu = ld4(mean + col);
+  if (act && (MODE == 1 || MODE == 2)) mu = ld4(mean + col);
   if (act && MODE == 2) { is = ld4(invstd + col); sc = ld4(scale + col); sh = ld4(shift + col); }
+  static_assert(32 % CR_WR == 0, "a wave's rows lie inside one k-tile");
+  bool uni = false;
+  if (MODE == 3 && r0 < R) uni = tile_ord[r0 >> 5] == 0;
   if (act) {
     const int rend = min(R, r0 + CR_WR);
     for (int rb = r0; rb < rend; rb += 8) {
@@ -39,8 +43,11 @@
         const int r = rb + u;
         if (r >= rend) break;
         float4 x = xs[u];
-        const float wr = (MODE != 2 && roww) ? roww[r] : 1.f;
-        if (MODE == 0) {
+        const float wr = (MODE <= 1 && roww) ? roww[r] : 1.f;
+        if (MODE == 3) {
+          acc[0] = add4(acc[0], x);
+          if (uni) acc[1] = add4(acc[1], x);
+        } else if (MODE == 0) {
           x = make_float4(x.x * wr, x.y * wr, x.z * wr, x.w * wr);
           const int g = rowidx ? (int)rowidx[r] : 0;
           if (g == 0) acc[0] = add4(acc[0], x);
@@ -414,6 +421,23 @@
   return QAGNN_OK;
 }
 
+extern "C" int qagnn_colsum_pad_f32(const float* X, int32_t ldx, int32_t R, int32_t Cc, const int32_t* tiles, float* out, float* workspace,
+                                    qagnn_stream_t stream_) {
+  hipStream_t stream = (hipStream_t)stream_;
+  QAGNN_REQUIRE(X && out && workspace && tiles, QAGNN_EINVAL, "colsum_pad: null pointer");
+  QAGNN_REQUIRE(R > 0 && Cc > 0 && Cc % 4 == 0 && ldx % 4 == 0 && ldx >= Cc && aligned16(X), QAGNN_EINVAL, "colsum_pad: bad sizes/alignment");
+  const PadTiles pt = pad_tiles_of(const_cast<int32_t*>(tiles), R);
+  dim3 grid(cdiv(Cc, 256), cdiv(R, 4 * cr_wr(R)));
+  if (cr_wr(R) == CR_WR_SMALL)
+    k_colreduce<3, CR_WR_SMALL><<<grid, 256, 0, stream>>>(X, ldx, nullptr, 0, R, Cc, nullptr, 2, nullptr, nullptr, nullptr, nullptr, nullptr, workspace, pt.ord);
+  else
+    k_colreduce<3, CR_WR_BIG><<<grid, 256, 0, stream>>>(X, ldx, nullptr, 0, R, Cc, nullptr, 2, nullptr, nullptr, nullptr, nullptr, nullptr, workspace, pt.ord);
+  QAGNN_LAUNCH_CHECK("k_colreduce");
+  k_colreduce_final<<<cdiv(2 * Cc, 64), 64 * CF_Q, 0, stream>>>(workspace, out, grid.y, 2 * Cc, 1.0f);
+  QAGNN_LAUNCH_CHECK("k_colreduce_final");
+  return QAGNN_OK;
+}
+
 extern "C" int qagnn_bn_relu_bwd_f32(const float* dR, const float* Hh, float* dH, int32_t ld, int32_t R, int32_t Cc,
                                      const float* mean, const float* invstd, const float* scale, const float* shift,
                                      const float* gamma, const float* sum_dy, const float* sum_dy_hhat, float inv_rows,
diff --git a/qagnn_amd/csrc/gemm.hip b/qagnn_amd/csrc/gemm.hip
--- a/qagnn_amd/csrc/gemm.hip
+++ b/qagnn_amd/csrc/gemm.hip
@@ -486,6 +486,39 @@
   }
 }
 
+__global__ __launch_bounds__(SC_G * 64) void k_sum_chunks4_pad(const float* __restrict__ P, float* __restrict__ C, int ldc, int Ka, int No,
+                                                               int nchunks, int accumulate, const float* __restrict__ pad_vec,
+                                                               const float* __restrict__ pad_sum, TnPad pd) {
+  __shared__ float4 part[SC_G][64];
+  const int lane = threadIdx.x & 63, g = threadIdx.x >> 6;
+  const int64_t n4 = (int64_t)Ka * No / 4, i4 = (int64_t)blockIdx.x * 64 + lane;
+  float4 s = make_float4(0.f, 0.f, 0.f, 0.f);
+  if (i4 < n4) {
+    const float4* src = reinterpret_cast<const float4*>(P) + i4;
+    for (int c0 = g; c0 < nchunks; c0 += 4 * SC_G) {
+      float4 v[4];
+#pragma unroll
+      for (int u = 0; u < 4; ++u) v[u] = src[(int64_t)min(c0 + u * SC_G, nchunks - 1) * n4];
+#pragma unroll
+      for (int u = 0; u < 4; ++u)
+        if (c0 + u * SC_G < nchunks) s = add4(s, v[u]);
+    }
+  }
+  part[g][lane] = s;
+  __syncthreads();
+  if (g == 0 && i4 < n4) {
+    float4 t = part[0][lane];
+#pragma unroll
+    for (int k = 1; k < SC_G; ++k) t = add4(t, part[k][lane]);
+    const int64_t e = i4 * 4;
+    const int row = (int)(e / No), col = (int)(e % No);
+    if (pd.n_ord[0] < pd.T) t = fma4(pad_vec[row], ld4(pad_sum + col), t);
+    float* d = C + (int64_t)row * ldc + col;
+    if (accumulate) t = add4(t, ld4(d));
+    st4(d, t);
+  }
+}
+
 __global__ __launch_bounds__(SC_G * 64) void k_sum_chunks4_live(const float* __restrict__ P, float* __restrict__ C, int ldc, int Ka, TnLive lv,
                                                                 int accumulate) {
   __shared__ float4 part[SC_G][64];
@@ -565,6 +598,14 @@
   return QAGNN_OK;
 }
 
+int launch_sum_chunks_pad(const float* P, float* C, int ldc, int rows, int No, int nchunks, int accumulate, const float* pad_vec,
+                          const float* pad_sum, const TnPad& pd, hipStream_t stream) {
+  const int64_t tot = (int64_t)rows * No;
+  k_sum_chunks4_pad<<<cdiv(tot / 4, 64), SC_G * 64, 0, stream>>>(P, C, ldc, rows, No, nchunks, accumulate, pad_vec, pad_sum, pd);
+  QAGNN_LAUNCH_CHECK("k_sum_chunks4_pad");
+  return QAGNN_OK;
+}
+
 int launch_sum_chunks(const float* P, float* C, int ldc, int rows, int No, int nchunks, int accumulate, bool by4, hipStream_t stream) {
   const int64_t tot = (int64_t)rows * No;
   if (by4) k_sum_chunks4<<<cdiv(tot / 4, 64), SC_G * 64, 0, stream>>>(P, C, ldc, rows, No, nchunks, accumulate);
diff --git a/qagnn_amd/csrc/gemm_dispatch.hip b/qagnn_amd/csrc/gemm_dispatch.hip
--- a/qagnn_amd/csrc/gemm_dispatch.hip
+++ b/qagnn_amd/csrc/gemm_dispatch.hip
@@ -175,6 +175,7 @@
     const int bpc = cdiv(p.No, r.nt * 16) * row_blocks;
     r.chunk_rows = tn_chunk_rows(p.R, bpc, 2, 32, lo);
     r.family = TnFamily::SPLIT;
+    r.pad = r.gather && p.pad_row >= 0 && p.pad_tiles && p.pad_sum && r.sum_by4;
     if (p.two) {
       const int rows1 = tn_chunk_rows(p.R, bpc, 1, 32, lo);
       if (rows1 >= 2 * TN_WS_MIN_TILES * 32) r.chunk_rows = rows1;
@@ -213,6 +214,8 @@
                 p.No);
   QAGNN_REQUIRE(!p.bsum || (p.groups >= 1 && p.groups <= 4 && (p.groups == 1 || p.b_rowidx)), QAGNN_EINVAL, "gemm_tn: colsum groups=%d (1..4)",
                 p.groups);
+  QAGNN_REQUIRE(p.pad_row < 0 || (p.a_rowidx && p.pad_tiles && p.pad_sum && aligned16(p.pad_sum) && !p.two && !p.bsum), QAGNN_EINVAL,
+                "gemm_tn: a pad row needs a_rowidx, the tile list of qagnn_pad_tiles and a 16-byte aligned column sum (one operand, no colsum)");
   return QAGNN_OK;
 }
 
@@ -239,6 +242,11 @@
     const LiveTiles lt = live_tiles_of(p.g);
     return launch_sum_chunks_live(p.ws, p.C, p.ldc, Ka, TnLive{lt.list, lt.n_live, lt.n_tiles, 3 * r.nchunks, r.chunk_rows / 32}, p.accumulate, stream);
   }
+  if (r.pad) {
+    const PadTiles pt = pad_tiles_of(const_cast<int32_t*>(p.pad_tiles), p.R);
+    return launch_sum_chunks_pad(p.ws, p.C, p.ldc, Ka, p.No, r.nchunks, p.accumulate, p.A1 + p.pad_row * p.lda1, p.pad_sum,
+                                 TnPad{pt.list, pt.n_ord, pt.ord, pt.n_tiles, r.chunk_rows / 32}, stream);
+  }
   if (int rc2 = launch_sum_chunks(p.ws, p.C, p.ldc, Ka, p.No, r.nchunks, p.accumulate, r.sum_by4, stream)) return rc2;
   return r.colsum ? launch_sum_chunks(Pcs, p.bsum, p.No, p.groups, p.No, r.nchunks, 0, false, stream) : QAGNN_OK;
 }
@@ -333,6 +341,25 @@
   return QAGNN_OK;
 }
 
+extern "C" int qagnn_gemm_tn_pad_f32(const float* A, int32_t lda, const float* B, int32_t ldb, float* C, int32_t ldc, int32_t R, int32_t Ka,
+                                     int32_t No, const int64_t* a_rowidx, int32_t accumulate, int64_t pad_row, const int32_t* tiles,
+                                     const float* pad_sum, float* workspace, qagnn_stream_t stream) {
+  QAGNN_REQUIRE(pad_row >= 0, QAGNN_EINVAL, "gemm_tn_pad: pad_row=%lld (a table row)", (long long)pad_row);
+  TnProduct p = tn_product(A, lda, Ka, nullptr, 0, 0, B, ldb, C, ldc, R, No, nullptr, nullptr, workspace);
+  p.a_rowidx = a_rowidx; p.accumulate = accumulate; p.pad_row = pad_row; p.pad_tiles = tiles; p.pad_sum = pad_sum;
+  return gemm_tn(p, (hipStream_t)stream);
+}
+
+extern "C" int qagnn_gemm_tn_pad_route_query(int32_t R, int32_t Ka, int32_t No, int32_t* h_out) {
+  QAGNN_REQUIRE(h_out && R > 0 && Ka > 0 && No > 0, QAGNN_EINVAL, "gemm_tn_pad_route_query: bad arguments");
+  alignas(16) static float any[4];
+  TnProduct p = tn_product(any, Ka, Ka, nullptr, 0, 0, any, No, any, No, R, No, nullptr, nullptr, any);
+  p.a_rowidx = reinterpret_cast<const int64_t*>(any); p.pad_row = 0; p.pad_tiles = reinterpret_cast<const int32_t*>(any); p.pad_sum = any;
+  const TnRoute r = tn_route(p);
+  h_out[0] = (int)r.family; h_out[1] = r.chunk_rows; h_out[2] = r.nchunks; h_out[3] = r.pad ? 1 : 0;
+  return QAGNN_OK;
+}
+
 extern "C" int qagnn_tn_live_tiles(int32_t on) { return on < 0 ? g_tn_live.load() : g_tn_live.exchange(on ? 1 : 0); }
 
 extern "C" int qagnn_gemm_tn_h1_f32(const float* A1, int32_t lda1, int32_t Ka1, const float* A2, int32_t lda2, int32_t Ka2, const float* B,
diff --git a/qagnn_amd/csrc/gemm_split.hip b/qagnn_amd/csrc/gemm_split.hip
--- a/qagnn_amd/csrc/gemm_split.hip
+++ b/qagnn_amd/csrc/gemm_split.hip
@@ -250,11 +250,11 @@
   }
 }
 
-template <int KT, int NT, bool AFFINE, bool GATHER, int NP = 3>
+template <int KT, int NT, bool AFFINE, bool GATHER, int NP = 3, bool PAD = false>
 __global__ __launch_bounds__(TTHR) __attribute__((amdgpu_waves_per_eu(2, 2))) void k_gemm_tn_split(
     const float* __restrict__ A, int lda, const float* __restrict__ B, int ldb, float* __restrict__ P, int R, int Ka, int No,
     const float* __restrict__ a_scale, const float* __restrict__ a_shift, int chunk_rows, const int64_t* __restrict__ a_rowidx,
-    const float* __restrict__ A2, int lda2, int Ka2, TnAmax amax) {
+    const float* __restrict__ A2, int lda2, int Ka2, TnAmax amax, TnPad pd) {
   extern __shared__ __attribute__((aligned(16))) unsigned char smem_tn[];
   constexpr int AC = KT * 16, BC = NT * 16, A_EL = AC * TCP, B_EL = BC * TCP;
   constexpr int MT = KT / 4, REM = KT % 4, RS = (REM * NT + 3) / 4;
@@ -264,6 +264,7 @@
   constexpr int MAJ_C = A_MAJOR ? AC : BC, MIN_C = A_MAJOR ? BC : AC, MAJ_EL = A_MAJOR ? A_EL : B_EL, MIN_EL = A_MAJOR ? B_EL : A_EL;
   static_assert(MAJ_TW <= 4 && MIN_TW <= 4, "task-waves per operand");
   static_assert(NP == 3 || !GATHER, "the gathered table goes through the exact split");
+  static_assert(!PAD || GATHER, "pad-uniform tiles are a property of the gather indices");
   uint16_t* const As = reinterpret_cast<uint16_t*>(smem_tn);
   uint16_t* const Bs = As + NP * A_EL;
   uint16_t* const Maj = A_MAJOR ? As : Bs;
@@ -271,7 +272,20 @@
   const int tid = threadIdx.x, lane = tid & 63, w = __builtin_amdgcn_readfirstlane(tid >> 6);
   QAGNN_TN_BLOCK(false, TnLive{})
   const int r_beg = chunk * chunk_rows, r_end = min(R, r_beg + chunk_rows);
-  const int ntile = (r_end - r_beg + TKR - 1) / TKR;
+  int ntile = (r_end - r_beg + TKR - 1) / TKR;
+  TnPadSlot pslot = {0, chunk * (chunk_rows / TKR), ntile};
+  if constexpr (PAD) {
+    pslot = tn_pad_slot((int)gridDim.z, pd.T, __builtin_amdgcn_readfirstlane(pd.n_ord[0]), pd.chunk_tiles, chunk);
+    ntile = pslot.cnt;
+  }
+  auto tile_row = [&](int t) {
+    if constexpr (PAD) {
+      const int q = min(pslot.beg + t, pd.T - 1);
+      return (pslot.list ? min(max(pd.list[q], 0), pd.T - 1) : q) * TKR;
+    } else {
+      return r_beg + t * TKR;
+    }
+  };
 
   static_assert(!GATHER || A_MAJOR, "the gathered operand is handled as the wide one");
   const __amdgpu_buffer_rsrc_t rsA = __builtin_amdgcn_make_buffer_rsrc(const_cast<float*>(A), 0, GATHER ? 0 : R * lda * 4, 0x00020000);
@@ -306,7 +320,7 @@
   const float* const Acol = A + min(maj0 + c4j * 4, Ka - 4);
   auto gidx = [&](int t) {
     if constexpr (GATHER) {
-      const int r0 = r_beg + t * TKR + g * 8;
+      const int r0 = tile_row(t) + g * 8;
 #pragma unroll
       for (int i = 0; i < 8; ++i) {
         const int64_t v = a_rowidx[min(r0 + i, R - 1)];
@@ -330,7 +344,7 @@
     if (mk < MIN_TW) {
       const int c4 = mk * 16 + (lane >> 2);
       const bool in = c4 * 4 < MIN_C && min0 + c4 * 4 < minDim;
-      const uint32_t voff = in ? ((uint32_t)(r_beg + t * TKR + g * 8) * ldMin4 + (uint32_t)(min0 + c4 * 4) * 4u) : OOB;
+      const uint32_t voff = in ? ((uint32_t)(tile_row(t) + g * 8) * ldMin4 + (uint32_t)(min0 + c4 * 4) * 4u) : OOB;
 #pragma unroll
       for (int i = 0; i < 8; ++i) rn[i] = bload<float4>(rsMin, voff + (uint32_t)i * ldMin4);
     }
@@ -675,6 +689,11 @@
   const LiveTiles lt = live_tiles_of(p.g);
   return TnLive{lt.list, lt.n_live, lt.n_tiles, 3 * r.nchunks, r.chunk_rows / TKR};
 }
+static TnPad tn_pad_args(const TnRoute& r, const TnProduct& p) {
+  if (!r.pad) return TnPad{nullptr, nullptr, nullptr, 0, 0};
+  const PadTiles pt = pad_tiles_of(const_cast<int32_t*>(p.pad_tiles), p.R);
+  return TnPad{pt.list, pt.n_ord, pt.ord, pt.n_tiles, r.chunk_rows / TKR};
+}
 static TnAmax tn_amax(const TnRoute& r, const TnProduct& p) {
   return r.np == 3 ? TnAmax{nullptr, nullptr, nullptr} : TnAmax{p.amax[0], p.two ? p.amax[1] : nullptr, p.amax[2]};
 }
@@ -687,11 +706,11 @@
   QAGNN_LAUNCH_CHECK("k_gemm_tn_ws");
   return QAGNN_OK;
 }
-template <int KT, int NT, bool AFFINE, bool GATHER = false, int NP = 3>
+template <int KT, int NT, bool AFFINE, bool GATHER = false, int NP = 3, bool PAD = false>
 static int launch_tn_split_i(const TnRoute& r, const TnProduct& p, hipStream_t stream) {
   constexpr int lds = NP * (KT * 16 + NT * 16) * TCP * (int)sizeof(uint16_t);
-  if (int rc = raise_lds_limit<k_gemm_tn_split<KT, NT, AFFINE, GATHER, NP>>(lds, "k_gemm_tn_split")) return rc;
-  k_gemm_tn_split<KT, NT, AFFINE, GATHER, NP><<<r.grid, TTHR, lds, stream>>>(QAGNN_TN_ARGS, p.a_scale, p.a_shift, r.chunk_rows, p.a_rowidx, p.A2, p.lda2, p.Ka2, tn_amax(r, p));
+  if (int rc = raise_lds_limit<k_gemm_tn_split<KT, NT, AFFINE, GATHER, NP, PAD>>(lds, "k_gemm_tn_split")) return rc;
+  k_gemm_tn_split<KT, NT, AFFINE, GATHER, NP, PAD><<<r.grid, TTHR, lds, stream>>>(QAGNN_TN_ARGS, p.a_scale, p.a_shift, r.chunk_rows, p.a_rowidx, p.A2, p.lda2, p.Ka2, tn_amax(r, p), tn_pad_args(r, p));
   QAGNN_LAUNCH_CHECK("k_gemm_tn_split");
   return QAGNN_OK;
 }
@@ -703,6 +722,7 @@
   });
 }
 int launch_tn_split(const TnRoute& r, const TnProduct& p, hipStream_t stream) {
+  if (r.gather && r.pad) return launch_tn_split_i<13, 7, false, true, 3, true>(r, p, stream);
   if (r.gather) return launch_tn_split_i<13, 7, false, true>(r, p, stream);
   return dispatch_bool(r.kt == 7, [&](auto wide_b) {
     return dispatch_bool(r.affine, [&](auto aff) {
diff --git a/qagnn_amd/csrc/graph_prep.hip b/qagnn_amd/csrc/graph_prep.hip
--- a/qagnn_amd/csrc/graph_prep.hip
+++ b/qagnn_amd/csrc/graph_prep.hip
@@ -474,6 +474,37 @@
     list[live[t] ? r : L + (t - r)] = t;
   }
   if (threadIdx.x == 0) *n_live = L;
+}
+
+__global__ __launch_bounds__(1024) void k_pad_tiles(const int64_t* __restrict__ rowidx, int R, int64_t pad_row, int T, int* ord, int* rank,
+                                                    int* list, int* n_ord) {
+  const int lane = threadIdx.x & 63, w = threadIdx.x >> 6;
+  constexpr int U = 16;
+  for (int t0 = w * 4 * U; t0 < T; t0 += 16 * 4 * U) {
+    longlong2 v[U];
+#pragma unroll
+    for (int u = 0; u < U; ++u) {
+      const int64_t r0 = ((int64_t)(t0 + 4 * u + (lane >> 4)) << 5) + (lane & 15) * 2;
+      v[u] = *reinterpret_cast<const longlong2*>(rowidx + (r0 + 1 < R ? r0 : 0));
+    }
+#pragma unroll
+    for (int u = 0; u < U; ++u) {
+      const int t = t0 + 4 * u + (lane >> 4);
+      const int64_t r0 = ((int64_t)t << 5) + (lane & 15) * 2;
+      const bool uni = r0 + 1 < R && v[u].x == pad_row && v[u].y == pad_row;
+      const unsigned long long m = __ballot(uni);
+      if ((lane & 15) == 0 && t < T) ord[t] = ((m >> (lane & 48)) & 0xFFFFull) == 0xFFFFull ? 0 : 1;
+    }
+  }
+  __syncthreads();
+  block_exclusive_scan(ord, rank, T);
+  __syncthreads();
+  const int O = rank[T];
+  for (int t = threadIdx.x; t < T; t += 1024) {
+    const int r = rank[t];
+    list[ord[t] ? r : O + (t - r)] = t;
+  }
+  if (threadIdx.x == 0) *n_ord = O;
 }
 
 __global__ void k_tn_work_table(const int* __restrict__ n_live, int T, int S, int chunk_tiles, int* __restrict__ out) {
@@ -695,6 +726,17 @@
   return QAGNN_OK;
 }
 
+extern "C" int64_t qagnn_pad_tiles_elems(int32_t R) { return R > 0 ? pad_tiles_elems(R) : 0; }
+
+extern "C" int qagnn_pad_tiles(const int64_t* a_rowidx, int32_t R, int64_t pad_row, int32_t* tiles, qagnn_stream_t stream_) {
+  QAGNN_REQUIRE(a_rowidx && tiles && aligned16(a_rowidx) && aligned16(tiles), QAGNN_EINVAL, "pad_tiles: null or misaligned pointer (16 bytes)");
+  QAGNN_REQUIRE(R >= 2, QAGNN_EINVAL, "pad_tiles: R=%d", R);
+  const PadTiles pt = pad_tiles_of(tiles, R);
+  k_pad_tiles<<<1, 1024, 0, (hipStream_t)stream_>>>(a_rowidx, R, pad_row, pt.n_tiles, pt.ord, pt.rank, pt.list, pt.n_ord);
+  QAGNN_LAUNCH_CHECK("k_pad_tiles");
+  return QAGNN_OK;
+}
+
 static int check_store(const char* who, const qagnn_store* st) {
   QAGNN_REQUIRE(st, QAGNN_EINVAL, "%s: null store", who);
   QAGNN_REQUIRE(st->blobs && st->blob_off && st->concept_ids && st->node_type && st->node_scores && st->adj_len, QAGNN_EINVAL,
diff --git a/qagnn_amd/data_utils.py b/qagnn_amd/data_utils.py
--- a/qagnn_amd/data_utils.py
+++ b/qagnn_amd/data_utils.py
@@ -3,6 +3,18 @@
 
 import numpy as np
 import torch
+
+PAD_CONCEPT_ID = 1
+PAD_TABLE_ROW = PAD_CONCEPT_ID - 1
+
+
+def pad_uniform_tiles(row_ids, pad_row=PAD_TABLE_ROW, tile=32):
+    ids = np.asarray(row_ids).reshape(-1)
+    R = ids.size
+    T = (R + tile - 1) // tile
+    full = np.full(T * tile, pad_row + 1, dtype=np.int64)
+    full[:R] = ids
+    return (full.reshape(T, tile) == pad_row).all(1)
 
 
 def record_to_graph(rec, max_node_num):
@@ -19,7 +31,7 @@
         raise AssertionError('question/answer concepts must precede all other concepts')
 
     num_concept = min(len(concepts), n - 1) + 1
-    concept_ids = np.full(n, 1, dtype=np.int64)
+    concept_ids = np.full(n, PAD_CONCEPT_ID, dtype=np.int64)
     concept_ids[0] = 0
     concept_ids[1:num_concept] = concepts[:num_concept - 1].astype(np.int64) + 1
     node_scores = np.zeros(n, dtype=np.float32)
diff --git a/qagnn_amd/modeling_qagnn.py b/qagnn_amd/modeling_qagnn.py
--- a/qagnn_amd/modeling_qagnn.py
+++ b/qagnn_amd/modeling_qagnn.py
@@ -5,6 +5,7 @@
 import torch.nn.functional as F
 
 from . import ops
+from .data_utils import PAD_TABLE_ROW
 from .layers import GELU, MLP, CustomizedEmbedding, MultiheadAttPoolLayer, gelu
 
 
@@ -465,7 +466,7 @@
             Wc_t, Wc, bc = self._input_plan((ce.cpt_transform.weight, ce.cpt_transform.bias),
                                             lambda ids: [L.pad(ids[0].t()), L.pad(ids[0].t()).t().contiguous(), L.pad(ids[1])])
             gnn_input = ops.concept_input(ce.emb.weight, ridx, Wc_t, bc, L.pad(self.svec2nvec(sent_vecs)), n,
-                                          self.dropout_e.p, self.training, Wc=Wc)
+                                          self.dropout_e.p, self.training, Wc=Wc, pad_row=PAD_TABLE_ROW)
         else:
             gnn_input0 = self.activation(self.svec2nvec(sent_vecs)).unsqueeze(1)
             gnn_input1 = self.concept_emb(concept_ids[:, 1:] - 1, emb_data).to(dev)
diff --git a/qagnn_amd/ops.py b/qagnn_amd/ops.py
--- a/qagnn_amd/ops.py
+++ b/qagnn_amd/ops.py
@@ -959,7 +959,7 @@
 
     @staticmethod
     @_fwd
-    def forward(ctx, emb_w, rowidx, Wc_t, bc, ctx_pre, n, p, seed, Wc=None):
+    def forward(ctx, emb_w, rowidx, Wc_t, bc, ctx_pre, n, p, seed, Wc=None, pad_row=-1):
         K = kernels()
         tam = table_amax(K, emb_w) if rowidx.numel() >= pack_min_rows(K) else None
         pre = K.gemm_nn(emb_w, Wc_t, bias=bc, a_rowidx=rowidx, B1n=Wc if Wc is not None else Wc_t.t().contiguous(),
@@ -967,7 +967,7 @@
         B = ctx_pre.size(0)
         pre.view(B, n, -1)[:, 0] = ctx_pre
         ctx.save_for_backward(emb_w, rowidx, pre)
-        ctx.cfg = (n, p, seed)
+        ctx.cfg = (n, p, seed, int(pad_row))
         if _wants_amax(K, pre):
             Hp, word = K.gelu_dropout_fwd(pre, p, seed, amax=True)
             return amax_note(Hp, word)
@@ -978,17 +978,22 @@
     def backward(ctx, dHp):
         K = kernels()
         emb_w, rowidx, pre = ctx.saved_tensors
-        n, p, seed = ctx.cfg
+        n, p, seed, pad_row = ctx.cfg
         dpre = K.gelu_dropout_bwd(pre, dHp.contiguous(), p, seed)
         dctx = dpre.view(-1, n, dpre.size(1))[:, 0].contiguous()
-        dWc_t, cs = K.gemm_tn(emb_w, dpre, a_rowidx=rowidx), K.colsum(dpre)
+        if pad_row >= 0 and hasattr(K, 'gemm_tn_pad'):
+            tiles = K.pad_tiles(rowidx, pad_row)
+            cs = K.colsum_pad(dpre, tiles)
+            dWc_t = K.gemm_tn_pad(emb_w, dpre, rowidx, pad_row, tiles, cs[1])
+        else:
+            dWc_t, cs = K.gemm_tn(emb_w, dpre, a_rowidx=rowidx), K.colsum(dpre)
         dbc = cs[0] - dctx.sum(0)
-        return None, None, dWc_t, dbc, dctx, None, None, None, None
-
-
-def concept_input(emb_w, rowidx, Wc_t, bc, ctx_pre, n, p, training, Wc=None):
+        return None, None, dWc_t, dbc, dctx, None, None, None, None, None
+
+
+def concept_input(emb_w, rowidx, Wc_t, bc, ctx_pre, n, p, training, Wc=None, pad_row=-1):
     p = float(p) if training else 0.0
-    return ConceptInputFn.apply(emb_w, rowidx, Wc_t, bc, ctx_pre, n, p, next_seed() if p > 0 else 0, Wc)
+    return ConceptInputFn.apply(emb_w, rowidx, Wc_t, bc, ctx_pre, n, p, next_seed() if p > 0 else 0, Wc, pad_row)
 
 
 QSCALE = lambda dh: 1.0 / math.sqrt(dh)
```

Measured after the change: 45170 QA-subgraphs/s, median of 2. About the same (+0.1%).
